# wyhuai/DDNM

Measured on NVIDIA H100. Metric: restored 256x256 images/sec @100 DDIM steps, higher is better.
Workload: dtype fp32

## Files before the change

ddnm_b200/_lib.py:

```python
import ctypes as C
import os

_HERE = os.path.dirname(os.path.abspath(__file__))
LIB_PATH = os.path.join(_HERE, "libddnm_b200.so")


class DDNMError(RuntimeError):
    pass


class SimpleCfg(C.Structure):
    _fields_ = [("ch", C.c_int), ("out_ch", C.c_int), ("n_levels", C.c_int), ("ch_mult", C.c_int * 8),
                ("num_res_blocks", C.c_int), ("n_attn_res", C.c_int), ("attn_res", C.c_int * 4),
                ("in_channels", C.c_int), ("resolution", C.c_int), ("groups", C.c_int), ("eps", C.c_float)]


class OpenAICfg(C.Structure):
    _fields_ = [("image_size", C.c_int), ("model_channels", C.c_int), ("num_res_blocks", C.c_int), ("n_levels", C.c_int),
                ("channel_mult", C.c_int * 8), ("n_attn_ds", C.c_int), ("attn_ds", C.c_int * 4),
                ("num_head_channels", C.c_int), ("out_channels", C.c_int), ("in_channels", C.c_int), ("groups", C.c_int),
                ("eps", C.c_float), ("num_classes", C.c_int), ("low_res", C.c_int), ("num_heads", C.c_int),
                ("num_heads_upsample", C.c_int), ("new_attention_order", C.c_int)]


class ClassifierCfg(C.Structure):
    _fields_ = [("image_size", C.c_int), ("model_channels", C.c_int), ("num_res_blocks", C.c_int), ("n_levels", C.c_int),
                ("channel_mult", C.c_int * 8), ("n_attn_ds", C.c_int), ("attn_ds", C.c_int * 4),
                ("num_head_channels", C.c_int), ("out_channels", C.c_int), ("in_channels", C.c_int), ("groups", C.c_int),
                ("eps", C.c_float), ("pool", C.c_int)]


class ClassifierGuidance(C.Structure):
    _fields_ = [("classifier", C.c_void_p), ("x", C.c_void_p), ("labels", C.c_void_p), ("scale", C.c_float),
                ("grad_buf", C.c_void_p), ("batch", C.c_int), ("labels_checked", C.c_int)]


class OperatorDesc(C.Structure):
    _fields_ = [("kind", C.c_int), ("channels", C.c_int), ("img_dim", C.c_int), ("ratio", C.c_int),
                ("v_small", C.c_void_p), ("u_small", C.c_void_p), ("singulars", C.c_void_p),
                ("singulars_orig", C.c_void_p), ("perm", C.c_void_p), ("mask", C.c_void_p), ("v_small2", C.c_void_p),
                ("u_small2", C.c_void_p)]


class SimpleDeg(C.Structure):
    _fields_ = [("use_mask", C.c_int), ("use_gray", C.c_int), ("scale", C.c_int), ("img_dim", C.c_int), ("channels", C.c_int),
                ("mask", C.c_void_p), ("image_mask", C.c_void_p)]


class HqScalars(C.Structure):
    _fields_ = [("c_recip", C.c_float), ("c_recipm1", C.c_float), ("coef1", C.c_float), ("coef2", C.c_float), ("lambda_t", C.c_float),
                ("gamma_t", C.c_float), ("nonzero", C.c_float), ("clip", C.c_int)]


class Schedule(C.Structure):
    _fields_ = [("n_pairs", C.c_int), ("t_i", C.c_void_p), ("t_j", C.c_void_p), ("abar", C.c_void_p),
                ("num_timesteps", C.c_int), ("eta", C.c_float), ("sigma_y", C.c_float), ("plus", C.c_int)]


class NoiseSeed(C.Structure):
    _fields_ = [("seed", C.c_ulonglong), ("row_offset", C.c_longlong)]


_lib = None

_P, _I, _LL, _F, _D = C.c_void_p, C.c_int, C.c_longlong, C.c_float, C.c_double
GuidanceFn = C.CFUNCTYPE(C.c_int, C.c_void_p, C.c_int, C.c_int, C.c_void_p)

_SIGS = {
    "ddnm_version": (C.c_int, []),
    "ddnm_unet_simple_create": (C.c_int, [C.POINTER(SimpleCfg), _I, C.POINTER(_P)]),
    "ddnm_unet_openai_create": (C.c_int, [C.POINTER(OpenAICfg), _I, C.POINTER(_P)]),
    "ddnm_classifier_create": (C.c_int, [C.POINTER(ClassifierCfg), _I, C.POINTER(_P)]),
    "ddnm_classifier_forward": (C.c_int, [_P, _P, _P, _P, _P]),
    "ddnm_classifier_grad": (C.c_int, [_P, _P, _P, _P, _F, _P, _P, _P]),
    "ddnm_classifier_guidance_fn": (C.c_int, [_P, _I, _I, _P]),
    "ddnm_unet_set_param": (C.c_int, [_P, C.c_char_p, _P, _LL]),
    "ddnm_unet_set_precision": (C.c_int, [_P, _I]),
    "ddnm_unet_finalize": (C.c_int, [_P]),
    "ddnm_unet_forward": (C.c_int, [_P, _P, _P, _P, _P]),
    "ddnm_unet_forward_cond": (C.c_int, [_P, _P, _P, _P, _P, _P]),
    "ddnm_unet_set_graph": (C.c_int, [_P, _I]),
    "ddnm_unet_set_low_res": (C.c_int, [_P, _P, _P]),
    "ddnm_unet_read_tap": (C.c_int, [_P, C.c_char_p, _P, _LL, _P]),
    "ddnm_unet_info": (C.c_int, [_P, C.POINTER(_LL), C.POINTER(_I), C.POINTER(_D)]),
    "ddnm_unet_profile": (C.c_int, [_P, _P, _P, _P, _P, C.c_char_p, _LL]),
    "ddnm_unet_destroy": (C.c_int, [_P]),
    "ddnm_operator_create": (C.c_int, [C.POINTER(OperatorDesc), C.POINTER(_P)]),
    "ddnm_operator_y_dim": (_LL, [_P]),
    "ddnm_operator_A": (C.c_int, [_P, _P, _I, _P, _P]),
    "ddnm_operator_A_pinv": (C.c_int, [_P, _P, _I, _P, _P]),
    "ddnm_operator_project": (C.c_int, [_P, _P, _P, _I, _P, _P]),
    "ddnm_operator_lambda": (C.c_int, [_P, _P, _I, _F, _F, _F, _F, _P, _P]),
    "ddnm_operator_lambda_noise": (C.c_int, [_P, _P, _P, _I, _F, _F, _F, _F, _P, _P]),
    "ddnm_operator_destroy": (C.c_int, [_P]),
    "ddnm_sample": (C.c_int, [_P, _P, C.POINTER(Schedule), _P, _P, _P, _I, _P, _P, _P]),
    "ddnm_sample_guided": (C.c_int, [_P, _P, C.POINTER(Schedule), _P, _P, _P, _I, _P, _P, GuidanceFn, _P, _P, _P, _P]),
    "ddnm_sample_range": (C.c_int, [_P, _P, C.POINTER(Schedule), _I, _I, _P, _P, C.POINTER(C.c_int), _P, _P, _I, _P, _P, _P, _P, _P]),
    "ddnm_noise_fill": (C.c_int, [C.POINTER(NoiseSeed), C.c_uint, C.c_uint, _P, _I, _LL, _P]),
    "ddnm_sample_range_seeded": (C.c_int, [_P, _P, C.POINTER(Schedule), _I, _I, _P, _P, C.POINTER(C.c_int), _P, C.POINTER(NoiseSeed), _I,
                                           _P, _P, _P, _P, _P]),
    "ddnm_sample_seeded": (C.c_int, [_P, _P, C.POINTER(Schedule), _P, _P, C.POINTER(NoiseSeed), _I, _P, _P, _P]),
    "ddnm_sample_simplified_range_seeded": (C.c_int, [_P, C.POINTER(SimpleDeg), C.POINTER(Schedule), _I, _I, _P, _P, C.POINTER(C.c_int),
                                                      _P, C.POINTER(NoiseSeed), _I, _P]),
    "ddnm_hq_step_seeded": (C.c_int, [C.POINTER(SimpleDeg), _P, _P, _I, _P, _P, _I, _I, _P, _P, C.POINTER(NoiseSeed), C.c_uint,
                                      C.POINTER(HqScalars), _I, _P, _P, _P, _P]),
    "ddnm_hq_undo_seeded": (C.c_int, [_P, C.POINTER(NoiseSeed), C.c_uint, _F, _F, _I, _LL, _P]),
    "ddnm_sample_simplified_range": (C.c_int, [_P, C.POINTER(SimpleDeg), C.POINTER(Schedule), _I, _I, _P, _P, C.POINTER(C.c_int), _P, _P,
                                               _I, _P]),
    "ddnm_simplified_A": (C.c_int, [C.POINTER(SimpleDeg), _P, _I, _P, _P]),
    "ddnm_simplified_Ap": (C.c_int, [C.POINTER(SimpleDeg), _P, _I, _P, _P]),
    "ddnm_sample_simplified": (C.c_int, [_P, C.POINTER(SimpleDeg), C.POINTER(Schedule), _P, _P, _P, _I, _P, _P, _P]),
    "ddnm_hq_canvas": (C.c_int, [_P, _I, _I, _I, _I, _I, _P, _P]),
    "ddnm_hq_step": (C.c_int, [C.POINTER(SimpleDeg), _P, _P, _I, _P, _P, _I, _I, _P, _P, _P, C.POINTER(HqScalars), _I, _P, _P, _P, _P]),
    "ddnm_hq_undo": (C.c_int, [_P, _P, _F, _F, _LL, _P]),
    "ddnm_hq_canvas_masked": (C.c_int, [C.POINTER(SimpleDeg), _P, _I, _P, _P, _P]),
    "ddnm_data_transform": (C.c_int, [_P, _LL, _P, _P, _I, _I, _P, _P]),
    "ddnm_inverse_data_transform": (C.c_int, [_P, _LL, _I, _I, _P, _P]),
    "ddnm_finish_images": (C.c_int, [_P, _P, _I, _I, _I, _I, _I, _I, _P, _P, _P, _P]),
    "ddnm_conv_tc": (C.c_int, [_P, _I, _I, _I, _I, _P, _P, _I, _I, _I, _P, _I, _P, _P, _P, _P]),
    "ddnm_conv_tc_ex": (C.c_int, [_P, _I, _I, _I, _I, _P, _P, _I, _I, _I, _I, _P, _I, _P, _P, _I, _P, _I, _I, _I, _I, C.POINTER(_D),
                                  C.POINTER(_I), _P]),
    "ddnm_gemm_tc": (C.c_int, [_P, _LL, _LL, _LL, _LL, _LL, _P, _LL, _LL, _LL, _LL, _LL, _I, _I, _I, _I, _I, _F, _P, _LL, _LL, _LL,
                               _I, _P]),
    "ddnm_conv_direct": (C.c_int, [_P, _I, _I, _I, _I, _P, _P, _I, _I, _I, _P, _P]),
    "ddnm_conv_stem_sr": (C.c_int, [_P, _P, _I, _I, _I, _I, _I, _I, _P, _P, _I, _P, _I, C.POINTER(_F), _P]),
    "ddnm_conv_tc_bench": (C.c_int, [_I, _I, _I, _I, _I, _I, _I, C.POINTER(_F), C.POINTER(_D)]),
    "ddnm_gnconv_chunk_bench": (C.c_int, [_I, _I, _I, _I, _I, _I, _I, C.POINTER(_F)]),
    "ddnm_groupnorm": (C.c_int, [_P, _I, _I, _I, _I, _I, _P, _P, _F, _I, _P, _P]),
    "ddnm_tc_debug_force_bn": (C.c_int, [_I]),
    "ddnm_tc_debug_deal": (C.c_int, [_I]),
    "ddnm_tc_debug_dual_mode": (C.c_int, [_I]),
    "ddnm_tc_debug_halo": (C.c_int, [_I]),
    "ddnm_tc_debug_pingpong": (C.c_int, [_I]),
    "ddnm_tc_debug_pp_pair": (C.c_int, [_I]),
    "ddnm_unet_set_batch_invariant": (C.c_int, [_P, _I]),
    "ddnm_tc_debug_sm_count": (C.c_int, [_I]),
}
EXPORTS = ["ddnm_last_error"] + list(_SIGS)


def lib():
    global _lib
    if _lib is None:
        if not os.path.exists(LIB_PATH):
            raise DDNMError(f"{LIB_PATH} not found: run `python -c 'import __graft_entry__ as g; g.build()'` first")
        L = C.CDLL(LIB_PATH)
        L.ddnm_last_error.restype = C.c_char_p
        L.ddnm_last_error.argtypes = []
        missing = [n for n in _SIGS if not hasattr(L, n)]
        if missing:
            raise DDNMError(f"{LIB_PATH} lacks symbols {missing}: stale build?")
        for name, (res, args) in _SIGS.items():
            fn = getattr(L, name)
            fn.restype, fn.argtypes = res, args
        _lib = L
    return _lib


def check(rc):
    if rc != 0:
        raise DDNMError(lib().ddnm_last_error().decode("utf-8", "replace"))


def noise_seed(seed, row_offset=0):
    seed, row_offset = int(seed), int(row_offset)
    if not 0 <= seed < 1 << 64:
        raise ValueError("seed must fit 64 unsigned bits")
    if row_offset < 0:
        raise ValueError("row_offset must not be negative")
    return NoiseSeed(seed, row_offset)


def ptr(t):
    return None if t is None else C.c_void_p(t.data_ptr())


def cur_stream():
    import torch
    return C.c_void_p(torch.cuda.current_stream().cuda_stream)
```

ddnm_b200/csrc/api.cu:

```cuda
#include "../../include/ddnm_b200.h"

#include <cstring>
#include <vector>

#include "api_util.cuh"
#include "engine.cuh"
#include "kernels.cuh"
#include "tc_gemm.cuh"

using namespace ddnm;

namespace ddnm {
thread_local std::string g_last_error;
}

extern "C" {

const char* ddnm_last_error(void) { return g_last_error.c_str(); }
int ddnm_version(void) { return 100; }

int ddnm_unet_simple_create(const ddnm_simple_cfg* c, int batch, void** handle) {
  DDNM_API_BEGIN
  DDNM_CHECK(c && handle, "null argument");
  SimpleCfg cfg;
  cfg.ch = c->ch; cfg.out_ch = c->out_ch; cfg.n_levels = c->n_levels;
  DDNM_CHECK(c->n_levels >= 1 && c->n_levels <= 8 && c->n_attn_res >= 0 && c->n_attn_res <= 4, "bad config");
  for (int i = 0; i < 8; ++i) cfg.ch_mult[i] = c->ch_mult[i];
  cfg.num_res_blocks = c->num_res_blocks;
  cfg.n_attn_res = c->n_attn_res;
  for (int i = 0; i < 4; ++i) cfg.attn_res[i] = c->attn_res[i];
  cfg.in_channels = c->in_channels; cfg.resolution = c->resolution; cfg.groups = c->groups; cfg.eps = c->eps;
  *handle = static_cast<UNetEngine*>(new UNetSimple(cfg, batch));
  DDNM_API_END
}

int ddnm_unet_openai_create(const ddnm_openai_cfg* c, int batch, void** handle) {
  DDNM_API_BEGIN
  DDNM_CHECK(c && handle, "null argument");
  DDNM_CHECK(c->n_levels >= 1 && c->n_levels <= 8 && c->n_attn_ds >= 0 && c->n_attn_ds <= 4, "bad config");
  OpenAICfg cfg;
  cfg.image_size = c->image_size; cfg.model_channels = c->model_channels; cfg.num_res_blocks = c->num_res_blocks;
  cfg.n_levels = c->n_levels;
  for (int i = 0; i < 8; ++i) cfg.channel_mult[i] = c->channel_mult[i];
  cfg.n_attn_ds = c->n_attn_ds;
  for (int i = 0; i < 4; ++i) cfg.attn_ds[i] = c->attn_ds[i];
  cfg.num_head_channels = c->num_head_channels; cfg.out_channels = c->out_channels; cfg.in_channels = c->in_channels;
  cfg.groups = c->groups; cfg.eps = c->eps; cfg.num_classes = c->num_classes; cfg.low_res = c->low_res;
  cfg.num_heads = c->num_heads; cfg.num_heads_upsample = c->num_heads_upsample; cfg.new_attention_order = c->new_attention_order;
  DDNM_CHECK(c->num_classes >= 0, "bad num_classes");
  DDNM_CHECK(c->new_attention_order == 0 || c->new_attention_order == 1, "new_attention_order must be 0 or 1");
  DDNM_CHECK(c->num_head_channels > 0 || c->num_heads >= 1, "num_head_channels <= 0 needs num_heads >= 1");
  *handle = static_cast<UNetEngine*>(new UNetOpenAI(cfg, batch));
  DDNM_API_END
}

int ddnm_classifier_create(const ddnm_classifier_cfg* c, int batch, void** handle) {
  DDNM_API_BEGIN
  DDNM_CHECK(c && handle, "null argument");
  DDNM_CHECK(c->n_levels >= 1 && c->n_levels <= 8 && c->n_attn_ds >= 0 && c->n_attn_ds <= 4, "bad config");
  EncoderCfg cfg;
  cfg.image_size = c->image_size; cfg.model_channels = c->model_channels; cfg.num_res_blocks = c->num_res_blocks;
  cfg.n_levels = c->n_levels;
  for (int i = 0; i < 8; ++i) cfg.channel_mult[i] = c->channel_mult[i];
  cfg.n_attn_ds = c->n_attn_ds;
  for (int i = 0; i < 4; ++i) cfg.attn_ds[i] = c->attn_ds[i];
  cfg.num_head_channels = c->num_head_channels; cfg.out_channels = c->out_channels; cfg.in_channels = c->in_channels;
  cfg.groups = c->groups; cfg.eps = c->eps; cfg.pool = c->pool;
  *handle = static_cast<UNetEngine*>(new UNetEncoder(cfg, batch));
  DDNM_API_END
}

static UNetEncoder* as_classifier(void* h) {
  UNetEncoder* e = dynamic_cast<UNetEncoder*>(static_cast<UNetEngine*>(h));
  DDNM_CHECK(e != nullptr, "handle is not a classifier");
  return e;
}

int ddnm_classifier_forward(void* h, const float* x, const float* t, float* logits, void* stream) {
  DDNM_API_BEGIN
  DDNM_CHECK(x && t && logits, "null argument");
  as_classifier(h)->forward(x, t, logits, (cudaStream_t)stream);
  DDNM_API_END
}

int ddnm_classifier_grad(void* h, const float* x, const float* t, const int* labels, float scale, float* grad_out, float* logits_out,
                         void* stream) {
  DDNM_API_BEGIN
  as_classifier(h)->grad(x, t, labels, scale, grad_out, logits_out, (cudaStream_t)stream);
  DDNM_API_END
}

int ddnm_classifier_guidance_fn(void* user, int, int t, void* stream) {
  DDNM_API_BEGIN
  ddnm_classifier_guidance* g = static_cast<ddnm_classifier_guidance*>(user);
  DDNM_CHECK(g && g->classifier && g->x && g->labels && g->grad_buf, "incomplete guidance context");
  UNetEncoder* e = as_classifier(g->classifier);
  DDNM_CHECK(g->batch == e->batch(), "classifier was built for batch " + std::to_string(e->batch()) + ", the guided loop runs " +
                                         std::to_string(g->batch));
  cudaStream_t st = (cudaStream_t)stream;
  if (!g->labels_checked) {
    e->check_labels(g->labels, st);
    g->labels_checked = 1;
  }
  e->fill_t((float)t, st);
  e->grad(g->x, e->t_in(), g->labels, g->scale, g->grad_buf, nullptr, st, true);
  DDNM_API_END
}

int ddnm_unet_set_param(void* h, const char* name, const float* data, long long numel) {
  DDNM_API_BEGIN
  static_cast<UNetEngine*>(h)->set_param(name, data, numel);
  DDNM_API_END
}
int ddnm_unet_finalize(void* h) {
  DDNM_API_BEGIN
  static_cast<UNetEngine*>(h)->finalize();
  DDNM_API_END
}
int ddnm_unet_forward(void* h, const float* x, const float* t, float* out, void* stream) {
  DDNM_API_BEGIN
  static_cast<UNetEngine*>(h)->forward(x, t, out, (cudaStream_t)stream);
  DDNM_API_END
}
int ddnm_unet_forward_cond(void* h, const float* x, const float* t, const int* labels, float* out, void* stream) {
  DDNM_API_BEGIN
  UNetEngine* u = static_cast<UNetEngine*>(h);
  u->set_labels(labels, (cudaStream_t)stream);
  u->forward(x, t, out, (cudaStream_t)stream);
  DDNM_API_END
}
int ddnm_unet_set_low_res(void* h, const float* low_res, void* stream) {
  DDNM_API_BEGIN
  static_cast<UNetEngine*>(h)->set_low_res(low_res, (cudaStream_t)stream);
  DDNM_API_END
}
int ddnm_unet_set_precision(void* h, int fp16_terms) {
  DDNM_API_BEGIN
  static_cast<UNetEngine*>(h)->set_terms(fp16_terms);
  DDNM_API_END
}
int ddnm_unet_set_batch_invariant(void* h, int on) {
  DDNM_API_BEGIN
  static_cast<UNetEngine*>(h)->set_batch_invariant(on != 0);
  DDNM_API_END
}
int ddnm_unet_set_graph(void* h, int on) {
  DDNM_API_BEGIN
  static_cast<UNetEngine*>(h)->set_use_graph(on != 0);
  DDNM_API_END
}
int ddnm_unet_read_tap(void* h, const char* name, float* dst, long long cap, void* stream) {
  DDNM_API_BEGIN
  DDNM_CHECK(static_cast<UNetEngine*>(h)->read_tap(name, dst, cap, (cudaStream_t)stream), std::string("unknown tap ") + name);
  DDNM_API_END
}
int ddnm_unet_info(void* h, long long* ws, int* launches, double* flops) {
  DDNM_API_BEGIN
  UNetEngine* u = static_cast<UNetEngine*>(h);
  if (ws) *ws = (long long)u->workspace_bytes();
  if (launches) *launches = u->num_launches();
  if (flops) *flops = u->flops_per_forward();
  DDNM_API_END
}
int ddnm_unet_profile(void* h, const float* x, const float* t, float* out, void* stream, char* json, long long cap) {
  DDNM_API_BEGIN
  std::string s = static_cast<UNetEngine*>(h)->profile(x, t, out, (cudaStream_t)stream);
  DDNM_CHECK((long long)s.size() + 1 <= cap, "json buffer too small");
  std::memcpy(json, s.c_str(), s.size() + 1);
  DDNM_API_END
}
int ddnm_unet_destroy(void* h) {
  DDNM_API_BEGIN
  delete static_cast<UNetEngine*>(h);
  DDNM_API_END
}

}

namespace {
struct Tmp {
  std::vector<void*> ptrs;
  ~Tmp() {
    for (void* p : ptrs) cudaFree(p);
  }
  template <class T>
  T* get(size_t n) {
    void* p = nullptr;
    CUDA_CHECK(cudaMalloc(&p, std::max<size_t>(n, 1) * sizeof(T)));
    ptrs.push_back(p);
    return (T*)p;
  }
};
int sm_count() {
  int dev = 0, n = 0;
  CUDA_CHECK(cudaGetDevice(&dev));
  CUDA_CHECK(cudaDeviceGetAttribute(&n, cudaDevAttrMultiProcessorCount, dev));
  return n;
}
View mkview(float* p, int N, int H, int W, int C) {
  View v;
  v.p = p; v.N = N; v.H = H; v.W = W; v.C = C; v.ld = C;
  return v;
}
int planned_sm_count() {
  int dev = 0;
  CUDA_CHECK(cudaGetDevice(&dev));
  cudaDeviceProp prop;
  CUDA_CHECK(cudaGetDeviceProperties(&prop, dev));
  return engine_sm_count(prop);
}
struct TermsScope {
  int prev;
  explicit TermsScope(int t) : prev(tc_get_terms()) { tc_set_terms(t); }
  ~TermsScope() { tc_set_terms(prev); }
};
}

extern "C" {

int ddnm_conv_tc(const float* x, int N, int H, int W, int Cin, const float* w, const float* bias, int Cout, int mode, int up2,
                 const float* side_x, int CinSide, const float* side_w, const float* residual, float* out, void* stream) {
  DDNM_API_BEGIN
  cudaStream_t s = (cudaStream_t)stream;
  Tmp tmp;
  const int taps = mode == TAPS_1X1 ? 1 : 9;
  int oH = H, oW = W;
  int smode = SPLIT_SAME;
  if (mode == TAPS_3X3_S2) { oH = H / 2; oW = W / 2; smode = SPLIT_S2D; DDNM_CHECK(!up2, "stride 2 with upsample"); }
  if (up2) { oH = 2 * H; oW = 2 * W; DDNM_CHECK(mode == TAPS_3X3 && !side_x && !residual, "upsample path: plain 3x3 only"); }
  const size_t pe = (size_t)N * H * W * Cin;
  SplitView A;
  A.hi = tmp.get<__half>(pe); A.lo = tmp.get<__half>(pe); A.C = Cin;
  if (smode == SPLIT_S2D) { A.N = 4 * N; A.H = oH; A.W = oW; } else { A.N = N; A.H = H; A.W = W; }
  View xv = mkview(const_cast<float*>(x), N, H, W, Cin);
  gn_apply_split(xv, 1, false, nullptr, nullptr, 0.f, false, smode, A.hi, A.lo, s);
  View ov = mkview(out, N, oH, oW, Cout);
  if (up2) {
    const size_t per_phase = (size_t)Cout * 4 * Cin;
    __half* wh = tmp.get<__half>(4 * per_phase);
    __half* wl = tmp.get<__half>(4 * per_phase);
    presum_up2_weights(w, Cout, Cin, wh, wl, s);
    for (int ph = 0; ph < 4; ++ph) {
      TcLaunch L = tc_make_up2_launch(A, wh + ph * per_phase, wl + ph * per_phase, Cout, ov, bias, 0, ph >> 1, ph & 1, sm_count());
      tc_run(L, s);
    }
    CUDA_CHECK(cudaStreamSynchronize(s));
    return 0;
  }
  SplitView S;
  if (side_x) {
    const size_t se = (size_t)N * oH * oW * CinSide;
    S.hi = tmp.get<__half>(se); S.lo = tmp.get<__half>(se); S.N = N; S.H = oH; S.W = oW; S.C = CinSide;
    gn_apply_split(mkview(const_cast<float*>(side_x), N, oH, oW, CinSide), 1, false, nullptr, nullptr, 0.f, false, SPLIT_SAME,
                   S.hi, S.lo, s);
  }
  const int ktot = taps * Cin + (side_x ? CinSide : 0);
  __half* wh = tmp.get<__half>((size_t)Cout * ktot);
  __half* wl = tmp.get<__half>((size_t)Cout * ktot);
  split_conv_weight(w, Cout, Cin, taps, wh, wl, ktot, 0, s);
  if (side_x) split_conv_weight(side_w, Cout, CinSide, 1, wh, wl, ktot, taps * Cin, s);
  TcLaunch L = tc_make_launch(A, mode, side_x ? &S : nullptr, wh, wl, 1, Cout, ov, bias, 0, residual, Cout, 1.0f, sm_count());
  tc_run(L, s);
  CUDA_CHECK(cudaStreamSynchronize(s));
  DDNM_API_END
}

int ddnm_conv_tc_ex(const float* x, int N, int H, int W, int Cin, const float* w, const float* chanadd, int ca_ld, int Cout, int mode,
                    int up2, const float* side_x, int CinSide, const float* side_w, const float* residual, int res_mode, float* out,
                    int out_ld, int split_k, int invariant, int terms, double* stats_out, int* split_used, void* stream) {
  DDNM_API_BEGIN
  DDNM_CHECK(x && w && out, "null argument");
  DDNM_CHECK(mode >= TAPS_3X3 && mode <= TAPS_3X3_S2 && res_mode >= 0 && res_mode <= 2 && out_ld >= Cout && ca_ld >= 0,
             "bad mode, res_mode, out_ld or ca_ld");
  DDNM_CHECK(split_k == -1 || split_k == 1 || split_k == 2 || split_k == 4, "split_k must be -1 (the engine's rule), 1, 2 or 4");
  cudaStream_t s = (cudaStream_t)stream;
  Tmp tmp;
  const TermsScope terms_scope(terms);
  const int sms = planned_sm_count();
  const int taps = mode == TAPS_1X1 ? 1 : 9;
  int oH = H, oW = W;
  int smode = SPLIT_SAME;
  if (mode == TAPS_3X3_S2) { oH = H / 2; oW = W / 2; smode = SPLIT_S2D; DDNM_CHECK(!up2, "stride 2 with upsample"); }
  if (up2) {
    oH = 2 * H; oW = 2 * W;
    DDNM_CHECK(mode == TAPS_3X3 && !side_x && !residual && split_k <= 1, "upsample path: plain unsplit 3x3 only");
  }
  const size_t pe = (size_t)N * H * W * Cin;
  SplitView A;
  A.hi = tmp.get<__half>(pe); A.lo = tmp.get<__half>(pe); A.C = Cin;
  if (smode == SPLIT_S2D) { A.N = 4 * N; A.H = oH; A.W = oW; } else { A.N = N; A.H = H; A.W = W; }
  gn_apply_split(mkview(const_cast<float*>(x), N, H, W, Cin), 1, false, nullptr, nullptr, 0.f, false, smode, A.hi, A.lo, s);
  View ov = mkview(out, N, oH, oW, Cout);
  ov.ld = out_ld;
  if (stats_out) {
    ov.st = tmp.get<StatAcc>((size_t)N * Cout * 2);
    ov.st_ld = Cout;
    CUDA_CHECK(cudaMemsetAsync(ov.st, 0, (size_t)N * Cout * 2 * sizeof(StatAcc), s));
  }
  int S = 1;
  if (up2) {
    const size_t per_phase = (size_t)Cout * 4 * Cin;
    __half* wh = tmp.get<__half>(4 * per_phase);
    __half* wl = tmp.get<__half>(4 * per_phase);
    presum_up2_weights(w, Cout, Cin, wh, wl, s);
    for (int ph = 0; ph < 4; ++ph)
      tc_run(tc_make_up2_launch(A, wh + ph * per_phase, wl + ph * per_phase, Cout, ov, chanadd, ca_ld, ph >> 1, ph & 1, sms, invariant != 0), s);
  } else {
    SplitView Sv;
    if (side_x) {
      const size_t se = (size_t)N * oH * oW * CinSide;
      Sv.hi = tmp.get<__half>(se); Sv.lo = tmp.get<__half>(se); Sv.N = N; Sv.H = oH; Sv.W = oW; Sv.C = CinSide;
      gn_apply_split(mkview(const_cast<float*>(side_x), N, oH, oW, CinSide), 1, false, nullptr, nullptr, 0.f, false, SPLIT_SAME,
                     Sv.hi, Sv.lo, s);
    }
    const int ktot = taps * Cin + (side_x ? CinSide : 0);
    __half* wh = tmp.get<__half>((size_t)Cout * ktot);
    __half* wl = tmp.get<__half>((size_t)Cout * ktot);
    split_conv_weight(w, Cout, Cin, taps, wh, wl, ktot, 0, s);
    if (side_x) split_conv_weight(side_w, Cout, CinSide, 1, wh, wl, ktot, taps * Cin, s);
    TcConvPlan P = tc_plan_conv(A, mode, side_x ? &Sv : nullptr, wh, wl, Cout, ov, chanadd, ca_ld, residual, Cout, res_mode, sms,
                                invariant != 0, split_k);
    if (P.S > 1) tc_set_partials(P, tmp.get<float>((size_t)P.part_elems));
    tc_run_conv(P, s);
    S = P.S;
  }
  CUDA_CHECK(cudaStreamSynchronize(s));
  if (split_used) *split_used = S;
  if (stats_out) {
    std::vector<StatAcc> h((size_t)N * Cout * 2);
    CUDA_CHECK(cudaMemcpy(h.data(), ov.st, h.size() * sizeof(StatAcc), cudaMemcpyDeviceToHost));
    for (size_t i = 0; i < h.size(); ++i) stats_out[i] = stat_value(h[i]);
  }
  DDNM_API_END
}

int ddnm_gemm_tc(const float* a, long long a_numel, long long a_off, long long a_s_row, long long a_s_head, long long a_s_img,
                 const float* b, long long b_numel, long long b_off, long long b_s_row, long long b_s_head, long long b_s_img, int M,
                 int N, int K, int heads, int images, float alpha, float* out, long long out_sn, long long out_sy, long long out_sx,
                 int invariant, void* stream) {
  DDNM_API_BEGIN
  DDNM_CHECK(a && b && out && M > 0 && N > 0 && K > 0 && heads > 0 && images > 0, "null or empty argument");
  cudaStream_t s = (cudaStream_t)stream;
  Tmp tmp;
  auto operand = [&](const float* src, long long numel, long long off, long long rows, long long s_row, long long s_head,
                     long long s_img) {
    DDNM_CHECK(numel % 8 == 0 && off >= 0 && s_row > 0 && s_head > 0 && s_img > 0, "GEMM operand: bad size or strides");
    DDNM_CHECK(off + (K - 1) + (rows - 1) * s_row + (heads - 1) * s_head + (images - 1) * s_img < numel,
               "GEMM operand reaches past its buffer");
    __half* hi = tmp.get<__half>((size_t)numel);
    __half* lo = tmp.get<__half>((size_t)numel);
    gn_apply_split(mkview(const_cast<float*>(src), 1, 1, (int)(numel / 8), 8), 1, false, nullptr, nullptr, 0.f, false, SPLIT_SAME,
                   hi, lo, s);
    return GemmOperand{hi + off, lo + off, s_row, s_head, s_img};
  };
  const GemmOperand A = operand(a, a_numel, a_off, M, a_s_row, a_s_head, a_s_img);
  const GemmOperand B = operand(b, b_numel, b_off, N, b_s_row, b_s_head, b_s_img);
  tc_run(tc_make_gemm_launch(A, B, M, N, K, heads, images, out, out_sn, out_sy, out_sx, alpha, planned_sm_count(), invariant != 0), s);
  CUDA_CHECK(cudaStreamSynchronize(s));
  DDNM_API_END
}

int ddnm_conv_stem_sr(const float* x, const float* low_res, int N, int C, int H, int W, int h, int w, const float* weight,
                      const float* bias, int Cout, float* out, int iters, float* ms_per_iter, void* stream) {
  DDNM_API_BEGIN
  DDNM_CHECK(x && weight && bias && out, "null argument");
  cudaStream_t s = (cudaStream_t)stream;
  View ov = mkview(out, N, H, W, Cout);
  conv3x3_stem_sr(x, low_res, C, h, w, weight, bias, ov, s);
  if (iters > 0 && ms_per_iter) {
    cudaEvent_t e0, e1;
    CUDA_CHECK(cudaEventCreate(&e0));
    CUDA_CHECK(cudaEventCreate(&e1));
    CUDA_CHECK(cudaEventRecord(e0, s));
    for (int i = 0; i < iters; ++i) conv3x3_stem_sr(x, low_res, C, h, w, weight, bias, ov, s);
    CUDA_CHECK(cudaEventRecord(e1, s));
    CUDA_CHECK(cudaEventSynchronize(e1));
    float ms = 0;
    CUDA_CHECK(cudaEventElapsedTime(&ms, e0, e1));
    cudaEventDestroy(e0);
    cudaEventDestroy(e1);
    *ms_per_iter = ms / iters;
  }
  CUDA_CHECK(cudaStreamSynchronize(s));
  DDNM_API_END
}

int ddnm_conv_direct(const float* x, int N, int H, int W, int Cin, const float* w, const float* bias, int Cout, int mode, int up2,
                     float* out, void* stream) {
  DDNM_API_BEGIN
  int oH = H, oW = W;
  if (mode == TAPS_3X3_S2) { oH = H / 2; oW = W / 2; }
  if (up2) { oH = 2 * H; oW = 2 * W; }
  conv_direct_ref(mkview(const_cast<float*>(x), N, H, W, Cin), w, bias, mode, up2 != 0, mkview(out, N, oH, oW, Cout),
                  (cudaStream_t)stream);
  DDNM_API_END
}

namespace {
__device__ __forceinline__ float bench_hash(unsigned long long i, unsigned seed) {
  unsigned x = (unsigned)(i * 2654435761ull) ^ seed;
  x ^= x >> 16; x *= 0x7feb352du; x ^= x >> 15; x *= 0x846ca68bu; x ^= x >> 16;
  return (float)(int)x * (1.0f / 2147483648.0f);
}
__global__ void bench_fill_f32(float* p, long long n, unsigned seed) {
  const long long i = (long long)blockIdx.x * blockDim.x + threadIdx.x;
  if (i < n) p[i] = bench_hash(i, seed);
}
__global__ void bench_fill_split(__half* hi, __half* lo, long long n, unsigned seed, float scale) {
  const long long i = (long long)blockIdx.x * blockDim.x + threadIdx.x;
  if (i < n) split_f16(bench_hash(i, seed) * scale, hi[i], lo[i]);
}
}

int ddnm_conv_tc_bench(int N, int H, int W, int Cin, int Cout, int mode, int iters, float* ms_per_iter, double* flops) {
  DDNM_API_BEGIN
  const bool random = iters < 0;
  if (random) iters = -iters;
  const int feat = mode >> 4;
  mode &= 15;
  const bool up2 = (feat & 8) != 0;
  Tmp tmp;
  const int taps = up2 ? 4 : (mode == TAPS_1X1 ? 1 : 9);
  const size_t pe = (size_t)N * H * W * Cin;
  SplitView A;
  A.hi = tmp.get<__half>(pe); A.lo = tmp.get<__half>(pe); A.N = N; A.H = H; A.W = W; A.C = Cin;
  float* xf = tmp.get<float>(pe);
  CUDA_CHECK(cudaMemset(xf, 0, pe * 4));
  if (random) bench_fill_f32<<<(unsigned)cdivll((long long)pe, 256), 256>>>(xf, (long long)pe, 0x1234u);
  gn_apply_split(mkview(xf, N, H, W, Cin), 1, false, nullptr, nullptr, 0.f, false, SPLIT_SAME, A.hi, A.lo, 0);
  const int ktot = taps * Cin;
  __half* wh = tmp.get<__half>((size_t)Cout * ktot);
  __half* wl = tmp.get<__half>((size_t)Cout * ktot);
  CUDA_CHECK(cudaMemset(wh, 0, (size_t)Cout * ktot * 2));
  CUDA_CHECK(cudaMemset(wl, 0, (size_t)Cout * ktot * 2));
  if (random) {
    const long long wn = (long long)Cout * ktot;
    bench_fill_split<<<(unsigned)cdivll(wn, 256), 256>>>(wh, wl, wn, 0x9876u, 1.0f / sqrtf((float)ktot));
  }
  const int oH = up2 ? 2 * H : H, oW = up2 ? 2 * W : W;
  const size_t oe = (size_t)N * oH * oW * Cout;
  float* o = tmp.get<float>(oe);
  View ov = mkview(o, N, oH, oW, Cout);
  if (feat & 1) {
    ov.st = tmp.get<StatAcc>((size_t)N * Cout * 2);
    ov.st_ld = Cout;
    CUDA_CHECK(cudaMemset(ov.st, 0, (size_t)N * Cout * 2 * sizeof(StatAcc)));
  }
  float* res = nullptr;
  if (feat & 2) {
    res = tmp.get<float>(oe);
    CUDA_CHECK(cudaMemset(res, 0, oe * 4));
    if (random) bench_fill_f32<<<(unsigned)cdivll((long long)oe, 256), 256>>>(res, (long long)oe, 0x777u);
  }
  float* ca = nullptr;
  if (feat & 4) {
    ca = tmp.get<float>((size_t)N * Cout);
    CUDA_CHECK(cudaMemset(ca, 0, (size_t)N * Cout * 4));
  }
  TcLaunch L = up2 ? tc_make_up2_launch(A, wh, wl, Cout, ov, ca, Cout, 0, 0, sm_count())
                   : tc_make_launch(A, mode, nullptr, wh, wl, 1, Cout, ov, ca, Cout, res, Cout, 1.0f, sm_count());
  for (int i = 0; i < 3; ++i) tc_run(L, 0);
  cudaEvent_t e0, e1;
  CUDA_CHECK(cudaEventCreate(&e0));
  CUDA_CHECK(cudaEventCreate(&e1));
  CUDA_CHECK(cudaEventRecord(e0, 0));
  for (int i = 0; i < iters; ++i) tc_run(L, 0);
  CUDA_CHECK(cudaEventRecord(e1, 0));
  CUDA_CHECK(cudaEventSynchronize(e1));
  float ms = 0;
  CUDA_CHECK(cudaEventElapsedTime(&ms, e0, e1));
  cudaEventDestroy(e0);
  cudaEventDestroy(e1);
  *ms_per_iter = ms / iters;
  *flops = L.flops;
  DDNM_API_END
}

int ddnm_gnconv_chunk_bench(int N, int chunk, int H, int W, int Cin, int Cout, int iters, float* ms_per_pass) {
  DDNM_API_BEGIN
  DDNM_CHECK(chunk >= 1 && N % chunk == 0, "chunk must divide N");
  Tmp tmp;
  const size_t pe = (size_t)N * H * W * Cin, ce = (size_t)chunk * H * W * Cin, oe = (size_t)N * H * W * Cout;
  float* x = tmp.get<float>(pe);
  bench_fill_f32<<<(unsigned)cdivll((long long)pe, 256), 256>>>(x, (long long)pe, 0x4321u);
  StatAcc* st = tmp.get<StatAcc>((size_t)N * Cin * 2);
  CUDA_CHECK(cudaMemset(st, 0, (size_t)N * Cin * 2 * sizeof(StatAcc)));
  View xv = mkview(x, N, H, W, Cin);
  xv.st = st; xv.st_ld = Cin;
  gn_stats(xv, 0);
  float* gamma = tmp.get<float>(Cin);
  float* beta = tmp.get<float>(Cin);
  bench_fill_f32<<<cdiv(Cin, 256), 256>>>(gamma, Cin, 0x11u);
  bench_fill_f32<<<cdiv(Cin, 256), 256>>>(beta, Cin, 0x22u);
  SplitView A;
  A.hi = tmp.get<__half>(ce); A.lo = tmp.get<__half>(ce); A.N = chunk; A.H = H; A.W = W; A.C = Cin;
  const int ktot = 9 * Cin;
  __half* wh = tmp.get<__half>((size_t)Cout * ktot);
  __half* wl = tmp.get<__half>((size_t)Cout * ktot);
  bench_fill_split<<<(unsigned)cdivll((long long)Cout * ktot, 256), 256>>>(wh, wl, (long long)Cout * ktot, 0x9876u, 1.0f / sqrtf((float)ktot));
  float* o = tmp.get<float>(oe);
  StatAcc* ost = tmp.get<StatAcc>((size_t)N * Cout * 2);
  CUDA_CHECK(cudaMemset(ost, 0, (size_t)N * Cout * 2 * sizeof(StatAcc)));
  float* ca = tmp.get<float>((size_t)N * Cout);
  CUDA_CHECK(cudaMemset(ca, 0, (size_t)N * Cout * 4));
  const int nch = N / chunk;
  std::vector<View> xs;
  std::vector<TcLaunch> Ls;
  for (int c = 0; c < nch; ++c) {
    View xc = xv;
    xc.p = x + (size_t)c * chunk * H * W * Cin; xc.N = chunk; xc.st = st + (size_t)c * chunk * Cin * 2;
    View oc = mkview(o + (size_t)c * chunk * H * W * Cout, chunk, H, W, Cout);
    oc.st = ost + (size_t)c * chunk * Cout * 2; oc.st_ld = Cout;
    xs.push_back(xc);
    Ls.push_back(tc_make_launch(A, TAPS_3X3, nullptr, wh, wl, 1, Cout, oc, ca + (size_t)c * chunk * Cout, Cout, nullptr, 0, 1.0f, sm_count()));
  }
  auto pass = [&]() {
    for (int c = 0; c < nch; ++c) {
      gn_apply_split(xs[c], 32, true, gamma, beta, 1e-6f, true, SPLIT_SAME, A.hi, A.lo, 0);
      tc_run(Ls[c], 0);
    }
  };
  for (int i = 0; i < 2; ++i) pass();
  cudaEvent_t e0, e1;
  CUDA_CHECK(cudaEventCreate(&e0));
  CUDA_CHECK(cudaEventCreate(&e1));
  CUDA_CHECK(cudaEventRecord(e0, 0));
  for (int i = 0; i < iters; ++i) pass();
  CUDA_CHECK(cudaEventRecord(e1, 0));
  CUDA_CHECK(cudaEventSynchronize(e1));
  float ms = 0;
  CUDA_CHECK(cudaEventElapsedTime(&ms, e0, e1));
  cudaEventDestroy(e0);
  cudaEventDestroy(e1);
  *ms_per_pass = ms / iters;
  DDNM_API_END
}

int ddnm_groupnorm(const float* x, int N, int H, int W, int C, int groups, const float* gamma, const float* beta, float eps,
                   int silu, float* out, void* stream) {
  DDNM_API_BEGIN
  cudaStream_t s = (cudaStream_t)stream;
  Tmp tmp;
  StatAcc* st = tmp.get<StatAcc>((size_t)N * C * 2);
  CUDA_CHECK(cudaMemsetAsync(st, 0, (size_t)N * C * 2 * sizeof(StatAcc), s));
  View xv = mkview(const_cast<float*>(x), N, H, W, C);
  xv.st = st;
  xv.st_ld = C;
  gn_stats(xv, s);
  gn_apply_f32(xv, groups, gamma, beta, eps, silu != 0, out, s);
  CUDA_CHECK(cudaStreamSynchronize(s));
  DDNM_API_END
}

int ddnm_tc_debug_deal(int mode) {
  DDNM_API_BEGIN
  tc_debug_deal(mode);
  DDNM_API_END
}
int ddnm_tc_debug_dual_mode(int mode) {
  DDNM_API_BEGIN
  tc_debug_dual_mode(mode);
  DDNM_API_END
}
int ddnm_tc_debug_halo(int on) {
  DDNM_API_BEGIN
  tc_debug_halo(on);
  DDNM_API_END
}
int ddnm_tc_debug_pingpong(int on) {
  DDNM_API_BEGIN
  tc_debug_pingpong(on);
  DDNM_API_END
}
int ddnm_tc_debug_pp_pair(int on) {
  DDNM_API_BEGIN
  tc_debug_pp_pair(on);
  DDNM_API_END
}
int ddnm_tc_debug_force_bn(int bn) {
  DDNM_API_BEGIN
  tc_debug_force_bn(bn);
  DDNM_API_END
}
int ddnm_tc_debug_sm_count(int n) {
  DDNM_API_BEGIN
  engine_debug_sm_count(n);
  DDNM_API_END
}
}
```

ddnm_b200/csrc/common.cuh:

```cuda
#pragma once
#include <cuda_runtime.h>
#include <cuda_fp16.h>
#include <cuda.h>
#include <cstdint>
#include <cstdio>
#include <stdexcept>
#include <string>

namespace ddnm {

struct Error : std::runtime_error {
  using std::runtime_error::runtime_error;
};

#define DDNM_CHECK(cond, msg)                                                                     \
  do {                                                                                            \
    if (!(cond)) throw ::ddnm::Error(std::string(msg) + " [" #cond "] at " __FILE__ ":" + std::to_string(__LINE__)); \
  } while (0)

#define CUDA_CHECK(expr)                                                                          \
  do {                                                                                            \
    cudaError_t _e = (expr);                                                                      \
    if (_e != cudaSuccess)                                                                        \
      throw ::ddnm::Error(std::string("CUDA error: ") + cudaGetErrorString(_e) + " in " #expr " at " __FILE__ ":" + \
                          std::to_string(__LINE__));                                              \
  } while (0)

inline int cdiv(int a, int b) { return (a + b - 1) / b; }
inline bool first_use_on_device(bool (&flags)[64]) {
  int dev = 0;
  cudaGetDevice(&dev);
  dev &= 63;
  if (flags[dev]) return false;
  flags[dev] = true;
  return true;
}
inline long long cdivll(long long a, long long b) { return (a + b - 1) / b; }

struct StreamBuf {
  float* p = nullptr;
  cudaStream_t st = nullptr;
  StreamBuf(size_t elems, cudaStream_t s) : st(s) {
    cudaError_t e = cudaMallocAsync((void**)&p, elems * sizeof(float), s);
    if (e != cudaSuccess) throw Error(std::string("CUDA error: ") + cudaGetErrorString(e) + " in cudaMallocAsync (sampler scratch)");
  }
  ~StreamBuf() {
    if (p) cudaFreeAsync(p, st);
  }
  StreamBuf(const StreamBuf&) = delete;
  StreamBuf& operator=(const StreamBuf&) = delete;
};

struct StatAcc {
  unsigned long long lo;
  long long hi;
};

bool pdl_enabled();
template <typename... KArgs, typename... Args>
inline void launch_pdl(void (*kernel)(KArgs...), dim3 grid, dim3 block, size_t smem, cudaStream_t st, int cluster, Args... args) {
  cudaLaunchConfig_t cfg = {};
  cfg.gridDim = grid;
  cfg.blockDim = block;
  cfg.dynamicSmemBytes = smem;
  cfg.stream = st;
  cudaLaunchAttribute at[2];
  int na = 0;
  if (pdl_enabled()) {
    at[na].id = cudaLaunchAttributeProgrammaticStreamSerialization;
    at[na].val.programmaticStreamSerializationAllowed = 1;
    ++na;
  }
  if (cluster > 1) {
    at[na].id = cudaLaunchAttributeClusterDimension;
    at[na].val.clusterDim.x = cluster;
    at[na].val.clusterDim.y = 1;
    at[na].val.clusterDim.z = 1;
    ++na;
  }
  cfg.attrs = at;
  cfg.numAttrs = na;
  cudaError_t e = cudaLaunchKernelEx(&cfg, kernel, KArgs(args)...);
  if (e != cudaSuccess) throw Error(std::string("CUDA error: ") + cudaGetErrorString(e) + " in cudaLaunchKernelEx");
}

struct View {
  float* p = nullptr;
  int N = 0, H = 0, W = 0, C = 0, ld = 0;
  StatAcc* st = nullptr;
  int st_ld = 0;
  long long pixels() const { return (long long)N * H * W; }
  View slice(int c0, int c) const {
    View v = *this;
    v.p = p + c0;
    v.C = c;
    if (st) v.st = st + 2 * (size_t)c0;
    return v;
  }
};

struct SplitView {
  __half* hi = nullptr;
  __half* lo = nullptr;
  int N = 0, H = 0, W = 0, C = 0;
};

#ifdef __CUDACC__
__device__ __forceinline__ void pdl_prologue() {
  asm volatile("griddepcontrol.launch_dependents;" ::: "memory");
  asm volatile("griddepcontrol.wait;" ::: "memory");
}
__device__ __forceinline__ uint32_t smem_u32(const void* p) { return (uint32_t)__cvta_generic_to_shared(p); }

__device__ __forceinline__ void mbar_init(uint32_t bar, uint32_t count) {
  asm volatile("mbarrier.init.shared::cta.b64 [%0], %1;" ::"r"(bar), "r"(count));
}
__device__ __forceinline__ void mbar_fence_init() { asm volatile("fence.mbarrier_init.release.cluster;" ::: "memory"); }
__device__ __forceinline__ void mbar_expect_tx(uint32_t bar, uint32_t bytes) {
  asm volatile("mbarrier.arrive.expect_tx.shared::cta.b64 _, [%0], %1;" ::"r"(bar), "r"(bytes) : "memory");
}
__device__ __forceinline__ void mbar_arrive(uint32_t bar) {
  asm volatile("mbarrier.arrive.shared::cta.b64 _, [%0];" ::"r"(bar) : "memory");
}
__device__ __forceinline__ bool mbar_try_wait(uint32_t bar, uint32_t parity) {
  uint32_t ok;
  asm volatile(
      "{\n\t.reg .pred p;\n\t"
      "mbarrier.try_wait.parity.shared::cta.b64 p, [%1], %2;\n\t"
      "selp.u32 %0, 1, 0, p;\n\t}"
      : "=r"(ok)
      : "r"(bar), "r"(parity)
      : "memory");
  return ok != 0;
}
__device__ __forceinline__ void mbar_wait(uint32_t bar, uint32_t parity) {
  if (mbar_try_wait(bar, parity)) return;
  long long t0 = clock64();
  while (!mbar_try_wait(bar, parity)) {
    if (clock64() - t0 > 4000000000LL) __trap();
  }
}

__device__ __forceinline__ void tma_prefetch_desc(const void* tmap) {
  asm volatile("prefetch.tensormap [%0];" ::"l"(tmap) : "memory");
}
__device__ __forceinline__ void tma_load_2d(uint32_t dst, const void* tmap, uint32_t bar, int c0, int c1) {
  asm volatile(
      "cp.async.bulk.tensor.2d.shared::cluster.global.tile.mbarrier::complete_tx::bytes [%0], [%1, {%3, %4}], [%2];" ::"r"(dst),
      "l"(tmap), "r"(bar), "r"(c0), "r"(c1)
      : "memory");
}
__device__ __forceinline__ void tma_load_3d(uint32_t dst, const void* tmap, uint32_t bar, int c0, int c1, int c2) {
  asm volatile(
      "cp.async.bulk.tensor.3d.shared::cluster.global.tile.mbarrier::complete_tx::bytes [%0], [%1, {%3, %4, %5}], [%2];" ::"r"(dst),
      "l"(tmap), "r"(bar), "r"(c0), "r"(c1), "r"(c2)
      : "memory");
}
__device__ __forceinline__ void tma_load_4d(uint32_t dst, const void* tmap, uint32_t bar, int c0, int c1, int c2, int c3) {
  asm volatile(
      "cp.async.bulk.tensor.4d.shared::cluster.global.tile.mbarrier::complete_tx::bytes [%0], [%1, {%3, %4, %5, %6}], [%2];" ::"r"(dst),
      "l"(tmap), "r"(bar), "r"(c0), "r"(c1), "r"(c2), "r"(c3)
      : "memory");
}

__device__ __forceinline__ uint64_t wgmma_desc_sw128(uint32_t saddr) {
  return (uint64_t)((saddr & 0x3FFFFu) >> 4) | ((uint64_t)1 << 16) | ((uint64_t)(1024 >> 4) << 32) | ((uint64_t)1 << 62);
}
__device__ __forceinline__ void wgmma_fence() { asm volatile("wgmma.fence.sync.aligned;" ::: "memory"); }
__device__ __forceinline__ void wgmma_commit() { asm volatile("wgmma.commit_group.sync.aligned;" ::: "memory"); }
template <int N>
__device__ __forceinline__ void wgmma_wait() { asm volatile("wgmma.wait_group.sync.aligned %0;" ::"n"(N) : "memory"); }
__device__ __forceinline__ void wgmma_m64n64k16(float (&d)[32], uint64_t a_desc, uint64_t b_desc, uint32_t accumulate) {
  asm volatile(
      "{\n\t.reg .pred p;\n\t"
      "setp.ne.b32 p, %34, 0;\n\t"
      "wgmma.mma_async.sync.aligned.m64n64k16.f32.f16.f16 "
      "{%0, %1, %2, %3, %4, %5, %6, %7, %8, %9, %10, %11, %12, %13, %14, %15, %16, %17, %18, %19, %20, %21, %22, %23, %24, %25, %26, %27, %28, %29, %30, %31}, "
      "%32, %33, p, 1, 1, 0, 0;\n\t}"
      : "+f"(d[0]), "+f"(d[1]), "+f"(d[2]), "+f"(d[3]), "+f"(d[4]), "+f"(d[5]), "+f"(d[6]), "+f"(d[7]), "+f"(d[8]), "+f"(d[9]), "+f"(d[10]), "+f"(d[11]), "+f"(d[12]), "+f"(d[13]), "+f"(d[14]), "+f"(d[15]), "+f"(d[16]), "+f"(d[17]), "+f"(d[18]), "+f"(d[19]), "+f"(d[20]), "+f"(d[21]), "+f"(d[22]), "+f"(d[23]), "+f"(d[24]), "+f"(d[25]), "+f"(d[26]), "+f"(d[27]), "+f"(d[28]), "+f"(d[29]), "+f"(d[30]), "+f"(d[31])
      : "l"(a_desc), "l"(b_desc), "r"(accumulate));
}
__device__ __forceinline__ void wgmma_m64n128k16(float (&d)[64], uint64_t a_desc, uint64_t b_desc, uint32_t accumulate) {
  asm volatile(
      "{\n\t.reg .pred p;\n\t"
      "setp.ne.b32 p, %66, 0;\n\t"
      "wgmma.mma_async.sync.aligned.m64n128k16.f32.f16.f16 "
      "{%0, %1, %2, %3, %4, %5, %6, %7, %8, %9, %10, %11, %12, %13, %14, %15, %16, %17, %18, %19, %20, %21, %22, %23, %24, %25, %26, %27, %28, %29, %30, %31, %32, %33, %34, %35, %36, %37, %38, %39, %40, %41, %42, %43, %44, %45, %46, %47, %48, %49, %50, %51, %52, %53, %54, %55, %56, %57, %58, %59, %60, %61, %62, %63}, "
      "%64, %65, p, 1, 1, 0, 0;\n\t}"
      : "+f"(d[0]), "+f"(d[1]), "+f"(d[2]), "+f"(d[3]), "+f"(d[4]), "+f"(d[5]), "+f"(d[6]), "+f"(d[7]), "+f"(d[8]), "+f"(d[9]), "+f"(d[10]), "+f"(d[11]), "+f"(d[12]), "+f"(d[13]), "+f"(d[14]), "+f"(d[15]), "+f"(d[16]), "+f"(d[17]), "+f"(d[18]), "+f"(d[19]), "+f"(d[20]), "+f"(d[21]), "+f"(d[22]), "+f"(d[23]), "+f"(d[24]), "+f"(d[25]), "+f"(d[26]), "+f"(d[27]), "+f"(d[28]), "+f"(d[29]), "+f"(d[30]), "+f"(d[31]), "+f"(d[32]), "+f"(d[33]), "+f"(d[34]), "+f"(d[35]), "+f"(d[36]), "+f"(d[37]), "+f"(d[38]), "+f"(d[39]), "+f"(d[40]), "+f"(d[41]), "+f"(d[42]), "+f"(d[43]), "+f"(d[44]), "+f"(d[45]), "+f"(d[46]), "+f"(d[47]), "+f"(d[48]), "+f"(d[49]), "+f"(d[50]), "+f"(d[51]), "+f"(d[52]), "+f"(d[53]), "+f"(d[54]), "+f"(d[55]), "+f"(d[56]), "+f"(d[57]), "+f"(d[58]), "+f"(d[59]), "+f"(d[60]), "+f"(d[61]), "+f"(d[62]), "+f"(d[63])
      : "l"(a_desc), "l"(b_desc), "r"(accumulate));
}
__device__ __forceinline__ void wgmma_m64n256k16(float (&d)[128], uint64_t a_desc, uint64_t b_desc, uint32_t accumulate) {
  asm volatile(
      "{\n\t.reg .pred p;\n\t"
      "setp.ne.b32 p, %130, 0;\n\t"
      "wgmma.mma_async.sync.aligned.m64n256k16.f32.f16.f16 "
      "{%0, %1, %2, %3, %4, %5, %6, %7, %8, %9, %10, %11, %12, %13, %14, %15, %16, %17, %18, %19, %20, %21, %22, %23, %24, %25, %26, %27, %28, %29, %30, %31, %32, %33, %34, %35, %36, %37, %38, %39, %40, %41, %42, %43, %44, %45, %46, %47, %48, %49, %50, %51, %52, %53, %54, %55, %56, %57, %58, %59, %60, %61, %62, %63, %64, %65, %66, %67, %68, %69, %70, %71, %72, %73, %74, %75, %76, %77, %78, %79, %80, %81, %82, %83, %84, %85, %86, %87, %88, %89, %90, %91, %92, %93, %94, %95, %96, %97, %98, %99, %100, %101, %102, %103, %104, %105, %106, %107, %108, %109, %110, %111, %112, %113, %114, %115, %116, %117, %118, %119, %120, %121, %122, %123, %124, %125, %126, %127}, "
      "%128, %129, p, 1, 1, 0, 0;\n\t}"
      : "+f"(d[0]), "+f"(d[1]), "+f"(d[2]), "+f"(d[3]), "+f"(d[4]), "+f"(d[5]), "+f"(d[6]), "+f"(d[7]), "+f"(d[8]), "+f"(d[9]), "+f"(d[10]), "+f"(d[11]), "+f"(d[12]), "+f"(d[13]), "+f"(d[14]), "+f"(d[15]), "+f"(d[16]), "+f"(d[17]), "+f"(d[18]), "+f"(d[19]), "+f"(d[20]), "+f"(d[21]), "+f"(d[22]), "+f"(d[23]), "+f"(d[24]), "+f"(d[25]), "+f"(d[26]), "+f"(d[27]), "+f"(d[28]), "+f"(d[29]), "+f"(d[30]), "+f"(d[31]), "+f"(d[32]), "+f"(d[33]), "+f"(d[34]), "+f"(d[35]), "+f"(d[36]), "+f"(d[37]), "+f"(d[38]), "+f"(d[39]), "+f"(d[40]), "+f"(d[41]), "+f"(d[42]), "+f"(d[43]), "+f"(d[44]), "+f"(d[45]), "+f"(d[46]), "+f"(d[47]), "+f"(d[48]), "+f"(d[49]), "+f"(d[50]), "+f"(d[51]), "+f"(d[52]), "+f"(d[53]), "+f"(d[54]), "+f"(d[55]), "+f"(d[56]), "+f"(d[57]), "+f"(d[58]), "+f"(d[59]), "+f"(d[60]), "+f"(d[61]), "+f"(d[62]), "+f"(d[63]), "+f"(d[64]), "+f"(d[65]), "+f"(d[66]), "+f"(d[67]), "+f"(d[68]), "+f"(d[69]), "+f"(d[70]), "+f"(d[71]), "+f"(d[72]), "+f"(d[73]), "+f"(d[74]), "+f"(d[75]), "+f"(d[76]), "+f"(d[77]), "+f"(d[78]), "+f"(d[79]), "+f"(d[80]), "+f"(d[81]), "+f"(d[82]), "+f"(d[83]), "+f"(d[84]), "+f"(d[85]), "+f"(d[86]), "+f"(d[87]), "+f"(d[88]), "+f"(d[89]), "+f"(d[90]), "+f"(d[91]), "+f"(d[92]), "+f"(d[93]), "+f"(d[94]), "+f"(d[95]), "+f"(d[96]), "+f"(d[97]), "+f"(d[98]), "+f"(d[99]), "+f"(d[100]), "+f"(d[101]), "+f"(d[102]), "+f"(d[103]), "+f"(d[104]), "+f"(d[105]), "+f"(d[106]), "+f"(d[107]), "+f"(d[108]), "+f"(d[109]), "+f"(d[110]), "+f"(d[111]), "+f"(d[112]), "+f"(d[113]), "+f"(d[114]), "+f"(d[115]), "+f"(d[116]), "+f"(d[117]), "+f"(d[118]), "+f"(d[119]), "+f"(d[120]), "+f"(d[121]), "+f"(d[122]), "+f"(d[123]), "+f"(d[124]), "+f"(d[125]), "+f"(d[126]), "+f"(d[127])
      : "l"(a_desc), "l"(b_desc), "r"(accumulate));
}
__device__ __forceinline__ uint32_t cluster_ctarank() {
  uint32_t r;
  asm volatile("mov.u32 %0, %%cluster_ctarank;" : "=r"(r));
  return r;
}
__device__ __forceinline__ void cluster_sync_all() {
  asm volatile("barrier.cluster.arrive.release.aligned;" ::: "memory");
  asm volatile("barrier.cluster.wait.acquire.aligned;" ::: "memory");
}
__device__ __forceinline__ void mbar_arrive_cluster(uint32_t bar, uint32_t cta) {
  uint32_t remote;
  asm volatile("mapa.shared::cluster.u32 %0, %1, %2;" : "=r"(remote) : "r"(bar), "r"(cta));
  asm volatile("mbarrier.arrive.shared::cluster.b64 _, [%0];" ::"r"(remote) : "memory");
}
__device__ __forceinline__ void tma_load_3d_multicast(uint32_t dst, const void* tmap, uint32_t bar, int c0, int c1, int c2, uint16_t mask) {
  asm volatile(
      "cp.async.bulk.tensor.3d.shared::cluster.global.mbarrier::complete_tx::bytes.multicast::cluster [%0], [%1, {%3, %4, %5}], [%2], %6;" ::"r"(dst),
      "l"(tmap), "r"(bar), "r"(c0), "r"(c1), "r"(c2), "h"(mask)
      : "memory");
}
__device__ __forceinline__ void named_bar_sync(int id, int threads) { asm volatile("bar.sync %0, %1;" ::"r"(id), "r"(threads) : "memory"); }
template <int R>
__device__ __forceinline__ void setmaxnreg_dec() { asm volatile("setmaxnreg.dec.sync.aligned.u32 %0;" ::"n"(R)); }
template <int R>
__device__ __forceinline__ void setmaxnreg_inc() { asm volatile("setmaxnreg.inc.sync.aligned.u32 %0;" ::"n"(R)); }

__device__ __forceinline__ void stat_add(StatAcc* acc, float p) {
  const int bits = __float_as_int(p);
  int ex = (bits >> 23) & 0xff;
  unsigned long long m = (unsigned long long)(bits & 0x7fffff);
  if (ex) m |= 0x800000ull; else ex = 1;
  const int sh = ex - 150 + 48;
  unsigned long long lo = 0, hi = 0;
  if (sh >= 64) hi = m << min(sh - 64, 7);
  else if (sh > 0) { lo = m << sh; hi = sh > 40 ? m >> (64 - sh) : 0ull; }
  else if (sh > -24) lo = m >> (-sh);
  if (bits < 0) {
    lo = ~lo + 1ull;
    hi = ~hi + (lo == 0ull ? 1ull : 0ull);
  }
  const unsigned long long w0 = lo & 0xffffffffull;
  const unsigned long long w1 = (hi << 32) | (lo >> 32);
  if (w0) atomicAdd(&acc->lo, w0);
  if (w1) atomicAdd(reinterpret_cast<unsigned long long*>(&acc->hi), w1);
}
__device__ __forceinline__ void two_sum_acc(float& sum, float& comp, float v) {
  const float s = __fadd_rn(sum, v);
  const float bb = __fadd_rn(s, -sum);
  comp = __fadd_rn(comp, __fadd_rn(__fadd_rn(sum, -__fadd_rn(s, -bb)), __fadd_rn(v, -bb)));
  sum = s;
}
__host__ __device__ __forceinline__ double stat_value(const StatAcc& a) {
  return ((double)a.hi * 4294967296.0 + (double)a.lo) * (1.0 / 281474976710656.0);
}

__device__ __forceinline__ float swishf_fast(float x) {
  float e;
  asm("ex2.approx.ftz.f32 %0, %1;" : "=f"(e) : "f"(x * -1.4426950408889634f));
  return __fdividef(x, 1.0f + e);
}
__device__ __forceinline__ void split_f16(float x, __half& hi, __half& lo) {
  unsigned short h;
  asm("cvt.rn.satfinite.f16.f32 %0, %1;" : "=h"(h) : "f"(x));
  hi = __ushort_as_half(h);
  float r = x - __half2float(hi);
  asm("cvt.rn.satfinite.f16.f32 %0, %1;" : "=h"(h) : "f"(r));
  lo = __ushort_as_half(h);
}
__device__ __forceinline__ void split2_f16(float x0, float x1, uint32_t& hi, uint32_t& lo) {
  asm("cvt.rn.satfinite.f16x2.f32 %0, %1, %2;" : "=r"(hi) : "f"(x1), "f"(x0));
  const __half2 h = *reinterpret_cast<const __half2*>(&hi);
  const float2 f = __half22float2(h);
  asm("cvt.rn.satfinite.f16x2.f32 %0, %1, %2;" : "=r"(lo) : "f"(x1 - f.y), "f"(x0 - f.x));
}

#endif

}
```

ddnm_b200/csrc/engine.cu:

```cuda
#include "engine.cuh"

#include <algorithm>
#include <cmath>
#include <cstdlib>
#include <sstream>

#include "kernels.cuh"

namespace ddnm {

Arena::~Arena() {
  for (void* b : blocks_) cudaFree(b);
}
void* Arena::alloc(size_t bytes) {
  bytes = (bytes + 1023) / 1024 * 1024;
  if (bytes == 0) bytes = 1024;
  void* p = nullptr;
  CUDA_CHECK(cudaMalloc(&p, bytes));
  blocks_.push_back(p);
  total_ += bytes;
  return p;
}

static int g_sm_count = 0;
void engine_debug_sm_count(int n) {
  DDNM_CHECK(n >= 0, "SM count must be 0 (the device's) or positive");
  g_sm_count = n;
}
int engine_sm_count(const cudaDeviceProp& prop) {
  return g_sm_count > 0 ? std::min(g_sm_count, prop.multiProcessorCount) : prop.multiProcessorCount;
}

UNetEngine::UNetEngine(int batch, int in_channels, int out_ch, int resolution, int groups, float eps)
    : B_(batch), in_ch_(in_channels), out_ch_(out_ch), R_(resolution), groups_(groups), eps_(eps) {
  DDNM_CHECK(batch >= 1, "batch must be positive");
  int dev = 0;
  CUDA_CHECK(cudaGetDevice(&dev));
  cudaDeviceProp prop;
  CUDA_CHECK(cudaGetDeviceProperties(&prop, dev));
  DDNM_CHECK(prop.major == 9 && prop.minor == 0, "ddnm_b200 kernels are built for sm_90a (H100) only");
  num_sms_ = engine_sm_count(prop);
}

UNetEngine::~UNetEngine() {
  if (graph_exec_) cudaGraphExecDestroy(graph_exec_);
  if (graph_) cudaGraphDestroy(graph_);
  for (auto& kv : params_) cudaFree(kv.second.p);
}

void UNetEngine::set_param(const std::string& name, const float* data, long long numel) {
  DDNM_CHECK(!finalized_, "set_param after finalize");
  DDNM_CHECK(numel > 0 && data != nullptr, "empty parameter " + name);
  float* d = nullptr;
  CUDA_CHECK(cudaMalloc(&d, (size_t)numel * sizeof(float)));
  CUDA_CHECK(cudaMemcpy(d, data, (size_t)numel * sizeof(float), cudaMemcpyDefault));
  auto it = params_.find(name);
  if (it != params_.end()) cudaFree(it->second.p);
  params_[name] = Param{d, numel};
}

const float* UNetEngine::P(const std::string& name, long long expect) const {
  auto it = params_.find(name);
  DDNM_CHECK(it != params_.end(), "missing parameter '" + name + "'");
  if (expect >= 0)
    DDNM_CHECK(it->second.n == expect, "parameter '" + name + "' has " + std::to_string(it->second.n) + " elements, expected " +
                                           std::to_string(expect));
  return it->second.p;
}

View UNetEngine::new_view(int H, int W, int C) {
  View v = view_of((float*)arena_.alloc((size_t)B_ * H * W * C * sizeof(float)), H, W, C);
  v.st = new_stats(C);
  v.st_ld = C;
  return v;
}

View UNetEngine::view_of(float* p, int H, int W, int C) const {
  View v;
  v.p = p; v.N = B_; v.H = H; v.W = W; v.C = C; v.ld = C;
  return v;
}

StatAcc* UNetEngine::new_stats(int C) {
  const size_t need = (size_t)B_ * C * 2;
  if (stats_chunks_.empty() || stats_chunks_.back().used + need > stats_chunks_.back().cap) {
    StatsChunk c;
    c.cap = std::max<size_t>(need, (size_t)1 << 20);
    c.used = 0;
    c.p = (StatAcc*)arena_.alloc(c.cap * sizeof(StatAcc));
    stats_chunks_.push_back(c);
  }
  StatsChunk& c = stats_chunks_.back();
  StatAcc* p = c.p + c.used;
  c.used += need;
  return p;
}

UNetEngine::TcWeights UNetEngine::prep_weights(const std::string& main, int Cout, int Cin, int taps, const std::string& side,
                                               int CinSide) {
  TcWeights w;
  w.ktot = taps * Cin + CinSide;
  const size_t n = (size_t)Cout * w.ktot;
  w.hi = (__half*)arena_.alloc(n * sizeof(__half));
  w.lo = (__half*)arena_.alloc(n * sizeof(__half));
  split_conv_weight(P(main, (long long)Cout * Cin * taps), Cout, Cin, taps, w.hi, w.lo, w.ktot, 0, 0);
  if (CinSide) split_conv_weight(P(side, (long long)Cout * CinSide), Cout, CinSide, 1, w.hi, w.lo, w.ktot, taps * Cin, 0);
  return w;
}

const float* UNetEngine::bias_sum(const std::string& a, const std::string& b, int C) {
  std::vector<float> ha(C), hb(C, 0.f);
  CUDA_CHECK(cudaMemcpy(ha.data(), P(a, C), C * sizeof(float), cudaMemcpyDeviceToHost));
  if (!b.empty()) CUDA_CHECK(cudaMemcpy(hb.data(), P(b, C), C * sizeof(float), cudaMemcpyDeviceToHost));
  for (int i = 0; i < C; ++i) ha[i] += hb[i];
  float* d = (float*)arena_.alloc(C * sizeof(float));
  CUDA_CHECK(cudaMemcpy(d, ha.data(), C * sizeof(float), cudaMemcpyHostToDevice));
  return d;
}

float* UNetEngine::dev_copy(const std::vector<float>& v) {
  float* d = (float*)arena_.alloc(v.size() * sizeof(float));
  CUDA_CHECK(cudaMemcpy(d, v.data(), v.size() * sizeof(float), cudaMemcpyHostToDevice));
  return d;
}

void UNetEngine::add_op(const std::string& name, const std::string& kind, double flops, double bytes,
                        std::function<void(cudaStream_t)> f) {
  ops_.push_back(OpRecord{name, kind, flops, bytes, std::move(f)});
}

void UNetEngine::emit_gn_split(const std::string& name, const View& x, const std::string& norm, bool silu, int mode,
                               SplitView& dst, const float* ss, int ss_ld, SplitView* raw) {
  const long long out_elems = mode == SPLIT_AVG2 ? x.pixels() * x.C / 4 : x.pixels() * x.C;
  DDNM_CHECK((size_t)out_elems <= split_elems_, "split scratch too small");
  dst.C = x.C;
  if (mode == SPLIT_SAME) { dst.N = x.N; dst.H = x.H; dst.W = x.W; }
  else if (mode == SPLIT_AVG2) { dst.N = x.N; dst.H = x.H / 2; dst.W = x.W / 2; }
  else { dst.N = 4 * x.N; dst.H = x.H / 2; dst.W = x.W / 2; }
  const double in_bytes = (double)x.pixels() * x.C * 4;
  if (!norm.empty()) {
    DDNM_CHECK(x.st != nullptr, "GroupNorm input without producer-side statistics: " + name);
    const float* g = P(norm + ".weight", x.C);
    const float* b = P(norm + ".bias", x.C);
    const int groups = groups_;
    const float eps = eps_;
    __half *hi = dst.hi, *lo = dst.lo, *rhi = nullptr, *rlo = nullptr;
    if (raw) {
      DDNM_CHECK(mode == SPLIT_SAME, "raw side output only with the plain split");
      raw->N = x.N; raw->H = x.H; raw->W = x.W; raw->C = x.C;
      rhi = raw->hi; rlo = raw->lo;
    }
    add_op(name + ".gn_split", "gn_split", 0, in_bytes + out_elems * 4.0 * (raw ? 2 : 1),
           [=](cudaStream_t s) { gn_apply_split(x, groups, true, g, b, eps, silu, mode, hi, lo, s, ss, ss_ld, rhi, rlo); });
  } else {
    __half *hi = dst.hi, *lo = dst.lo;
    add_op(name + ".split", "gn_split", 0, in_bytes + out_elems * 4.0,
           [=](cudaStream_t s) { gn_apply_split(x, 1, false, nullptr, nullptr, 0.f, silu, mode, hi, lo, s); });
  }
}

void UNetEngine::emit_tc(const std::string& name, const SplitView& a, int mode, const SplitView* side, const TcWeights& w,
                         int Cout, const View& out, const float* chanadd, int ca_ld, const float* residual, int ldr, int res_mode) {
  TcConvPlan P = tc_plan_conv(a, mode, side, w.hi, w.lo, Cout, out, chanadd, ca_ld, residual, ldr, res_mode, num_sms_, invariant_);
  const TcLaunch& L = P.L;
  const double bytes = (double)a.N * a.H * a.W * a.C * 4 + (side ? (double)side->N * side->H * side->W * side->C * 4 : 0) +
                       (double)Cout * w.ktot * 4 + (double)out.pixels() * Cout * 4 * (residual ? 2 : 1);
  if (P.S > 1) {
    tc_set_partials(P, (float*)arena_.alloc((size_t)P.part_elems * sizeof(float)));
    add_op(name, "tc", L.flops, bytes, [L](cudaStream_t s) { tc_run(L, s); });
    add_op(name + ".splitk_reduce", "reduce", 0, (double)(P.S + 1 + (residual ? 1 : 0)) * (P.part_elems / P.S) * 4,
           [P](cudaStream_t s) { tc_run_split_reduce(P, s); });
    return;
  }
  add_op(name, "tc", L.flops, bytes, [L](cudaStream_t s) { tc_run(L, s); });
}

void UNetEngine::alloc_common(size_t split_elems, size_t hbuf_elems) {
  split_elems_ = split_elems;
  hbuf_elems_ = hbuf_elems;
  splitA_hi_ = (__half*)arena_.alloc(split_elems * 2);
  splitA_lo_ = (__half*)arena_.alloc(split_elems * 2);
  splitB_hi_ = (__half*)arena_.alloc(split_elems * 2);
  splitB_lo_ = (__half*)arena_.alloc(split_elems * 2);
  if (hbuf_elems) hbuf_ = (float*)arena_.alloc(hbuf_elems * 4);
  x_in_ = (float*)arena_.alloc((size_t)B_ * in_ch_ * R_ * R_ * 4);
  t_in_ = (float*)arena_.alloc((size_t)B_ * 4);
  labels_in_ = (int*)arena_.alloc((size_t)B_ * 4);
  CUDA_CHECK(cudaMemset(labels_in_, 0, (size_t)B_ * 4));
  out_ = (float*)arena_.alloc(out_elems() * 4);
  if (lowres_ > 0) lowres_in_ = (float*)arena_.alloc((size_t)B_ * in_ch_ * lowres_ * lowres_ * 4);
}

void UNetEngine::emit_up2_conv(const std::string& name, const SplitView& a, const std::string& wname, int Cout, const View& out,
                               const float* chanadd, int ca_ld) {
  const int Cin = a.C;
  const size_t per_phase = (size_t)Cout * 4 * Cin;
  __half* wh = (__half*)arena_.alloc(4 * per_phase * sizeof(__half));
  __half* wl = (__half*)arena_.alloc(4 * per_phase * sizeof(__half));
  presum_up2_weights(P(wname, (long long)Cout * Cin * 9), Cout, Cin, wh, wl, 0);
  for (int ph = 0; ph < 4; ++ph) {
    TcLaunch L = tc_make_up2_launch(a, wh + ph * per_phase, wl + ph * per_phase, Cout, out, chanadd, ca_ld, ph >> 1, ph & 1, num_sms_,
                                     invariant_);
    const double bytes = (double)a.N * a.H * a.W * Cin * 4 + (double)per_phase * 4 + (double)a.N * a.H * a.W * Cout * 4;
    add_op(name + ".ph" + std::to_string(ph), "tc", L.flops, bytes, [L](cudaStream_t s) { tc_run(L, s); });
  }
}

void UNetEngine::alloc_attention(size_t qkv_elems, size_t s_elems, size_t o_elems) {
  qkv_ = (float*)arena_.alloc(qkv_elems * 4);
  attS_ = (float*)arena_.alloc(s_elems * 4);
  attO_ = (float*)arena_.alloc(o_elems * 4);
  qkvh_ = (__half*)arena_.alloc(qkv_elems * 2);
  qkvl_ = (__half*)arena_.alloc(qkv_elems * 2);
  ph_ = (__half*)arena_.alloc(s_elems * 2);
  pl_ = (__half*)arena_.alloc(s_elems * 2);
  vth_ = (__half*)arena_.alloc(o_elems * 2);
  vtl_ = (__half*)arena_.alloc(o_elems * 2);
}

void UNetEngine::emit_attention_core(const std::string& name, float* qkv, int T, int heads, int ch, int qkv_ld, int head_stride,
                                     int q_off, int k_off, int v_off, float alpha) {
  float *q = qkv, *S = attS_, *O = attO_;
  const int Bn = B_, C = heads * ch;
  const long long img = (long long)T * qkv_ld;
  const double fl = 2.0 * Bn * heads * (double)T * T * ch;
  const double sbytes = (double)Bn * heads * T * T * 4;
  if (T % 128 == 0 && ch % 8 == 0) {
    __half *qh = qkvh_, *ql = qkvl_, *ph = ph_, *pl = pl_, *vh = vth_, *vl = vtl_;
    DDNM_CHECK(qkv_ld % C == 0, "qkv row is not a multiple of the attention width");
    const View qv = view_of(qkv, 1, T * (qkv_ld / C), C);
    add_op(name + ".qkv_split", "gn_split", 0, (double)Bn * T * qkv_ld * 8,
           [=](cudaStream_t s) { gn_apply_split(qv, 1, false, nullptr, nullptr, 0.f, false, SPLIT_SAME, qh, ql, s); });
    const long long hs = head_stride ? head_stride : qkv_ld;
    GemmOperand A{qh + q_off, ql + q_off, qkv_ld, hs, img};
    GemmOperand Bk{qh + k_off, ql + k_off, qkv_ld, hs, img};
    TcLaunch L1 = tc_make_gemm_launch(A, Bk, T, T, ch, heads, Bn, S, (long long)heads * T * T, (long long)T * T, T, alpha, num_sms_, invariant_);
    add_op(name + ".qk", "tc", L1.flops, (double)Bn * T * qkv_ld * 4 + sbytes, [L1](cudaStream_t s) { tc_run(L1, s); });
    add_op(name + ".softmax", "softmax", 0, sbytes * 2, [=](cudaStream_t s) { softmax_split(S, (long long)Bn * heads * T, T, ph, pl, s); });
    add_op(name + ".v_transpose", "gn_split", 0, (double)Bn * T * C * 8,
           [=](cudaStream_t s) { transpose_split(q, qkv_ld, head_stride, v_off, Bn, T, heads, ch, vh, vl, s); });
    GemmOperand P{ph, pl, T, (long long)T * T, (long long)heads * T * T};
    GemmOperand Vt{vh, vl, T, (long long)ch * T, (long long)heads * ch * T};
    TcLaunch L2 = tc_make_gemm_launch(P, Vt, T, ch, T, heads, Bn, O, (long long)T * C, ch, C, 1.0f, num_sms_, invariant_);
    add_op(name + ".pv", "tc", L2.flops, sbytes + (double)Bn * T * C * 8, [L2](cudaStream_t s) { tc_run(L2, s); });
  } else {
    add_op(name + ".qk", "sgemm", fl, (double)Bn * heads * T * (2.0 * ch + T) * 4, [=](cudaStream_t s) {
      sgemm_batched(true, Bn, heads, T, T, ch, alpha, q + q_off, qkv_ld, img, head_stride, q + k_off, qkv_ld, img, head_stride, S, T,
                    (long long)heads * T * T, (long long)T * T, s);
    });
    add_op(name + ".softmax", "softmax", 0, sbytes * 2, [=](cudaStream_t s) { softmax_rows(S, (long long)Bn * heads * T, T, s); });
    add_op(name + ".pv", "sgemm", fl, (double)Bn * heads * T * (2.0 * ch + T) * 4, [=](cudaStream_t s) {
      sgemm_batched(false, Bn, heads, T, ch, T, 1.0f, S, T, (long long)heads * T * T, (long long)T * T, q + v_off, qkv_ld, img, head_stride, O,
                    C, (long long)T * C, ch, s);
    });
  }
}

void UNetEngine::emit_stem(const std::string& wname, const View& out) {
  const float* xin = x_in_;
  if (lowres_ > 0) {
    const float *w = P(wname + ".weight", (long long)out.C * 2 * in_ch_ * 9), *b = P(wname + ".bias", out.C);
    const float* lr = lowres_in_;
    const int cin = in_ch_, s = lowres_;
    add_op("stem.sr", "stem", 2.0 * B_ * R_ * R_ * (double)out.C * 2 * cin * 9,
           (double)B_ * (R_ * R_ * (cin + out.C) + (double)s * s * cin) * 4,
           [=](cudaStream_t st) { conv3x3_stem_sr(xin, lr, cin, s, s, w, b, out, st); });
    return;
  }
  const float *w = P(wname + ".weight", (long long)out.C * in_ch_ * 9), *b = P(wname + ".bias", out.C);
  const int cin = in_ch_;
  add_op("stem", "stem", 2.0 * B_ * R_ * R_ * (double)out.C * cin * 9, (double)B_ * R_ * R_ * (cin + out.C) * 4,
         [=](cudaStream_t s) { conv3x3_small_cin(xin, cin, w, b, out, s); });
}

void UNetEngine::emit_head(const std::string& norm, const std::string& conv, const View& fh) {
  DDNM_CHECK(fh.st != nullptr, "head input without statistics");
  DDNM_CHECK(out_ch_ <= 64, "head convolution: out_ch <= 64");
  if (head_conv_supported(fh, out_ch_) && std::getenv("DDNM_HEAD_TC") == nullptr) {
    const float *g = P(norm + ".weight", fh.C), *b = P(norm + ".bias", fh.C);
    const float *w = P(conv + ".weight", (long long)out_ch_ * fh.C * 9), *cb = P(conv + ".bias", out_ch_);
    const int groups = groups_, oc = out_ch_;
    const float eps = eps_;
    float* o = out_;
    add_op("head.conv", "head", 2.0 * fh.pixels() * (double)oc * fh.C * 9, (double)fh.pixels() * (fh.C + oc) * 4,
           [=](cudaStream_t s) { head_conv(fh, groups, g, b, eps, w, cb, oc, o, s); });
    return;
  }
  SplitView A{splitA_hi_, splitA_lo_};
  emit_gn_split("head", fh, norm, true, SPLIT_SAME, A);
  const int ktot = 9 * fh.C;
  TcWeights w;
  w.ktot = ktot;
  w.hi = (__half*)arena_.alloc((size_t)64 * ktot * sizeof(__half));
  w.lo = (__half*)arena_.alloc((size_t)64 * ktot * sizeof(__half));
  CUDA_CHECK(cudaMemset(w.hi, 0, (size_t)64 * ktot * sizeof(__half)));
  CUDA_CHECK(cudaMemset(w.lo, 0, (size_t)64 * ktot * sizeof(__half)));
  split_conv_weight(P(conv + ".weight", (long long)out_ch_ * fh.C * 9), out_ch_, fh.C, 9, w.hi, w.lo, ktot, 0, 0);
  std::vector<float> hb(64, 0.f);
  CUDA_CHECK(cudaMemcpy(hb.data(), P(conv + ".bias", out_ch_), out_ch_ * sizeof(float), cudaMemcpyDeviceToHost));
  float* bias64 = dev_copy(hb);
  const View o64 = view_of((float*)arena_.alloc((size_t)B_ * fh.H * fh.W * 64 * sizeof(float)), fh.H, fh.W, 64);
  emit_tc("head.conv", A, TAPS_3X3, nullptr, w, 64, o64, bias64, 0, nullptr, 0);
  float* o = out_;
  const View real = o64.slice(0, out_ch_);
  add_op("head.to_nchw", "head", 0, (double)fh.pixels() * (64 + out_ch_) * 4, [=](cudaStream_t s) { nhwc_to_nchw(real, o, s); });
}

void UNetEngine::emit_time_embed(const std::string& name, const std::string& layer0, const std::string& layer1, int ch,
                                 bool sin_first, const float* label_emb, int num_classes, const std::vector<EmbProj>& projs) {
  const int tdim = ch * 4;
  float* emb = (float*)arena_.alloc((size_t)B_ * ch * 4);
  float* t0 = (float*)arena_.alloc((size_t)B_ * tdim * 4);
  float* t1 = (float*)arena_.alloc((size_t)B_ * tdim * 4);
  float* fr = (float*)arena_.alloc((size_t)(ch / 2) * 4);
  CUDA_CHECK(cudaMemcpy(fr, P("__freq", ch / 2), (ch / 2) * 4, cudaMemcpyDeviceToDevice));
  emb_ld_ = 0;
  for (const EmbProj& pr : projs) {
    emb_off_[pr.block] = emb_ld_;
    emb_ld_ += pr.rows;
  }
  float* W = (float*)arena_.alloc((size_t)emb_ld_ * tdim * 4);
  float* Bv = (float*)arena_.alloc((size_t)emb_ld_ * 4);
  emb_all_ = (float*)arena_.alloc((size_t)B_ * emb_ld_ * 4);
  for (const EmbProj& pr : projs) {
    const int off = emb_off_[pr.block];
    CUDA_CHECK(cudaMemcpy(W + (size_t)off * tdim, P(pr.weight, (long long)pr.rows * tdim), (size_t)pr.rows * tdim * 4,
                          cudaMemcpyDeviceToDevice));
    CUDA_CHECK(cudaMemcpy(Bv + off, pr.bias, (size_t)pr.rows * 4, cudaMemcpyDeviceToDevice));
  }
  const float *w0 = P(layer0 + ".weight", (long long)tdim * ch), *b0 = P(layer0 + ".bias", tdim);
  const float *w1 = P(layer1 + ".weight", (long long)tdim * tdim), *b1 = P(layer1 + ".bias", tdim);
  const float* t = t_in_;
  const int* labels = labels_in_;
  float* rows = emb_all_;
  const int Bn = B_, tot = emb_ld_;
  add_op(name, "temb", 0, 0, [=](cudaStream_t s) {
    sinusoid(t, Bn, fr, ch, sin_first, emb, s);
    linear(emb, Bn, ch, w0, b0, tdim, t0, tdim, 0, 1, s);
    if (label_emb) {
      linear(t0, Bn, tdim, w1, b1, tdim, t1, tdim, 0, 0, s);
      add_label_swish(t1, label_emb, labels, Bn, tdim, num_classes, s);
    } else {
      linear(t0, Bn, tdim, w1, b1, tdim, t1, tdim, 0, 1, s);
    }
    linear(t1, Bn, tdim, W, Bv, tot, rows, tot, 0, 0, s);
  });
}

UNetEngine::Torso UNetEngine::plan_torso(int image_size, int in_channels, int model_channels, const int* channel_mult, int n_levels,
                                         int num_res_blocks, const int* attn_ds, int n_attn_ds) {
  auto attn_at = [&](int ds) { return std::find(attn_ds, attn_ds + n_attn_ds, ds) != attn_ds + n_attn_ds; };
  Torso t;
  int ch = channel_mult[0] * model_channels, ds = 1, res = image_size;
  t.input.push_back({{{LAYER_CONV, in_channels, ch}}, res, res, ch});
  for (int lv = 0; lv < n_levels; ++lv) {
    const int co = channel_mult[lv] * model_channels;
    for (int i = 0; i < num_res_blocks; ++i) {
      Block b{{{LAYER_RES, ch, co}}, res, res, co};
      ch = co;
      if (attn_at(ds)) b.layers.push_back({LAYER_ATTN, ch, ch});
      t.input.push_back(b);
    }
    if (lv != n_levels - 1) {
      t.input.push_back({{{LAYER_RES_DOWN, ch, ch}}, res, res / 2, ch});
      res /= 2;
      ds *= 2;
    }
  }
  t.middle = {{{LAYER_RES, ch, ch}, {LAYER_ATTN, ch, ch}, {LAYER_RES, ch, ch}}, res, res, ch};
  return t;
}

void UNetEngine::emit_res_block(const std::string& p, const View& x, const View& h, const View& out, int kind) {
  const int Cin = x.C, Cout = out.C;
  if (kind != LAYER_RES) DDNM_CHECK(Cin == Cout, "up/down ResBlocks keep the channel count");
  SplitView A{splitA_hi_, splitA_lo_}, Bs{splitB_hi_, splitB_lo_};
  const int mode1 = kind == LAYER_RES_DOWN ? SPLIT_AVG2 : SPLIT_SAME;
  const bool has_skip_conv = has_param(p + ".skip_connection.weight");
  emit_gn_split(p + ".in", x, p + ".in_layers.0", true, mode1, A, nullptr, 0, has_skip_conv ? &Bs : nullptr);
  if (kind == LAYER_RES_UP) {
    emit_up2_conv(p + ".conv1", A, p + ".in_layers.2.weight", Cout, h, P(p + ".in_layers.2.bias", Cout), 0);
  } else {
    TcWeights w1 = prep_weights(p + ".in_layers.2.weight", Cout, Cin, 9, "", 0);
    emit_tc(p + ".conv1", A, TAPS_3X3, nullptr, w1, Cout, h, P(p + ".in_layers.2.bias", Cout), 0, nullptr, 0);
  }
  emit_gn_split(p + ".out", h, p + ".out_layers.0", true, SPLIT_SAME, A, emb_rows(p), emb_ld_);
  if (has_skip_conv) {
    DDNM_CHECK(kind == LAYER_RES, "skip convolution on an up/down block");
    TcWeights w2 = prep_weights(p + ".out_layers.3.weight", Cout, Cout, 9, p + ".skip_connection.weight", Cin);
    emit_tc(p + ".conv2+skip", A, TAPS_3X3, &Bs, w2, Cout, out, bias_sum(p + ".out_layers.3.bias", p + ".skip_connection.bias", Cout), 0,
            nullptr, 0);
  } else {
    DDNM_CHECK(Cin == Cout, "identity skip needs equal channels");
    TcWeights w2 = prep_weights(p + ".out_layers.3.weight", Cout, Cout, 9, "", 0);
    emit_tc(p + ".conv2", A, TAPS_3X3, nullptr, w2, Cout, out, P(p + ".out_layers.3.bias", Cout), 0, x.p, x.ld,
            kind == LAYER_RES_UP ? 1 : (kind == LAYER_RES_DOWN ? 2 : 0));
  }
}

void UNetEngine::emit_attention_block(const std::string& p, const View& x, const View& out, int heads, bool new_order, float* qkv) {
  const int C = x.C, T = x.H * x.W, ch = C / heads;
  SplitView A{splitA_hi_, splitA_lo_};
  emit_gn_split(p + ".norm", x, p + ".norm", false, SPLIT_SAME, A);
  TcWeights wqkv = prep_weights(p + ".qkv.weight", 3 * C, C, 1, "", 0);
  emit_tc(p + ".qkv", A, TAPS_1X1, nullptr, wqkv, 3 * C, view_of(qkv, x.H, x.W, 3 * C), P(p + ".qkv.bias", 3 * C), 0, nullptr, 0);
  const float alpha = 1.0f / std::sqrt((float)ch);
  if (new_order) emit_attention_core(p, qkv, T, heads, ch, 3 * C, ch, 0, C, 2 * C, alpha);
  else emit_attention_core(p, qkv, T, heads, ch, 3 * C, 3 * ch, 0, ch, 2 * ch, alpha);
  emit_gn_split(p + ".proj_in", view_of(attO_, x.H, x.W, C), "", false, SPLIT_SAME, A);
  TcWeights wp = prep_weights(p + ".proj_out.weight", C, C, 1, "", 0);
  emit_tc(p + ".proj_out", A, TAPS_1X1, nullptr, wp, C, out, P(p + ".proj_out.bias", C), 0, x.p, x.ld);
}

void UNetEngine::set_terms(int t) {
  DDNM_CHECK(!finalized_, "precision must be chosen before finalize");
  DDNM_CHECK(t == 1 || t == 3, "terms must be 1 (fast fp16) or 3 (fp32-grade)");
  terms_ = t;
}

void UNetEngine::set_batch_invariant(bool on) {
  DDNM_CHECK(!finalized_, "batch-invariant mode must be chosen before finalize");
  invariant_ = on;
}

void UNetEngine::finalize() {
  DDNM_CHECK(!finalized_, "finalize called twice");
  const int prev = tc_get_terms();
  tc_set_terms(terms_);
  try {
    build_program();
  } catch (...) {
    tc_set_terms(prev);
    throw;
  }
  tc_set_terms(prev);
  std::vector<OpRecord> zero;
  for (const StatsChunk& c : stats_chunks_) {
    StatAcc* sb = c.p;
    const size_t sbytes = c.used * sizeof(StatAcc);
    zero.push_back(OpRecord{"stats.zero", "memset", 0, (double)sbytes,
                            [=](cudaStream_t s) { CUDA_CHECK(cudaMemsetAsync(sb, 0, sbytes, s)); }});
  }
  ops_.insert(ops_.begin(), zero.begin(), zero.end());
  CUDA_CHECK(cudaDeviceSynchronize());
  finalized_ = true;
}

void UNetEngine::run_ops(cudaStream_t s, size_t n) {
  for (size_t i = 0; i < n && i < ops_.size(); ++i) ops_[i].run(s);
}

void UNetEngine::fill_t(float t, cudaStream_t stream) { fill(t_in_, B_, t, stream); }

void UNetEngine::set_labels(const int* labels_dev, cudaStream_t stream) {
  DDNM_CHECK(class_cond_, "set_labels on a network without a label embedding");
  DDNM_CHECK(labels_dev != nullptr, "null labels");
  if (labels_dev != labels_in_) CUDA_CHECK(cudaMemcpyAsync(labels_in_, labels_dev, (size_t)B_ * sizeof(int), cudaMemcpyDeviceToDevice, stream));
}

void UNetEngine::set_low_res(const float* low_res_dev, cudaStream_t stream) {
  DDNM_CHECK(lowres_ > 0, "set_low_res on a network without a low-resolution input");
  DDNM_CHECK(low_res_dev != nullptr, "null low_res");
  if (low_res_dev != lowres_in_)
    CUDA_CHECK(cudaMemcpyAsync(lowres_in_, low_res_dev, (size_t)B_ * in_ch_ * lowres_ * lowres_ * 4, cudaMemcpyDeviceToDevice, stream));
  lowres_set_ = true;
}

void UNetEngine::forward(const float* x, const float* t, float* out, cudaStream_t stream) {
  DDNM_CHECK(finalized_, "forward before finalize");
  DDNM_CHECK(lowres_ == 0 || lowres_set_, "super-resolution network: no low_res conditioning image was given");
  const size_t xin = (size_t)B_ * in_ch_ * R_ * R_ * 4;
  if (x != x_in_) CUDA_CHECK(cudaMemcpyAsync(x_in_, x, xin, cudaMemcpyDeviceToDevice, stream));
  if (t != t_in_) CUDA_CHECK(cudaMemcpyAsync(t_in_, t, (size_t)B_ * 4, cudaMemcpyDeviceToDevice, stream));
  replay(stream, ops_.size() - n_tail_ops_, graph_, graph_exec_);
  if (out != out_) CUDA_CHECK(cudaMemcpyAsync(out, out_, out_elems() * 4, cudaMemcpyDeviceToDevice, stream));
}

void UNetEngine::replay(cudaStream_t stream, size_t n, cudaGraph_t& g, cudaGraphExec_t& exec) {
  if (!use_graph_) {
    run_ops(stream, n);
    return;
  }
  if (!exec) {
    cudaStream_t cs = nullptr;
    CUDA_CHECK(cudaStreamCreateWithFlags(&cs, cudaStreamNonBlocking));
    CUDA_CHECK(cudaStreamSynchronize(stream));
    run_ops(cs, n);
    CUDA_CHECK(cudaStreamSynchronize(cs));
    CUDA_CHECK(cudaStreamBeginCapture(cs, cudaStreamCaptureModeThreadLocal));
    try {
      run_ops(cs, n);
    } catch (...) {
      cudaGraph_t gg = nullptr;
      cudaStreamEndCapture(cs, &gg);
      if (gg) cudaGraphDestroy(gg);
      cudaStreamDestroy(cs);
      throw;
    }
    CUDA_CHECK(cudaStreamEndCapture(cs, &g));
    CUDA_CHECK(cudaGraphInstantiate(&exec, g, 0));
    CUDA_CHECK(cudaStreamDestroy(cs));
  }
  CUDA_CHECK(cudaGraphLaunch(exec, stream));
}

bool UNetEngine::read_tap(const std::string& name, float* dst, long long capacity, cudaStream_t stream) {
  auto it = taps_.find(name);
  if (it == taps_.end()) return false;
  const View& v = it->second;
  DDNM_CHECK(capacity >= v.pixels() * v.C, "tap buffer too small");
  nhwc_to_nchw(v, dst, stream);
  return true;
}

double UNetEngine::flops_per_forward() const {
  double f = 0;
  for (auto& op : ops_) f += op.flops;
  return f;
}

std::string UNetEngine::profile(const float* x, const float* t, float* out, cudaStream_t stream) {
  const bool g = use_graph_;
  use_graph_ = false;
  forward(x, t, out, stream);
  CUDA_CHECK(cudaStreamSynchronize(stream));
  std::vector<cudaEvent_t> ev(ops_.size() + 1);
  for (auto& e : ev) CUDA_CHECK(cudaEventCreate(&e));
  CUDA_CHECK(cudaEventRecord(ev[0], stream));
  for (size_t i = 0; i < ops_.size(); ++i) {
    ops_[i].run(stream);
    CUDA_CHECK(cudaEventRecord(ev[i + 1], stream));
  }
  CUDA_CHECK(cudaStreamSynchronize(stream));
  std::ostringstream js;
  js << "[";
  for (size_t i = 0; i < ops_.size(); ++i) {
    float ms = 0;
    CUDA_CHECK(cudaEventElapsedTime(&ms, ev[i], ev[i + 1]));
    if (i) js << ",";
    js << "{\"name\":\"" << ops_[i].name << "\",\"kind\":\"" << ops_[i].kind << "\",\"ms\":" << ms << ",\"flops\":" << ops_[i].flops
       << ",\"bytes\":" << ops_[i].bytes << "}";
  }
  js << "]";
  for (auto& e : ev) cudaEventDestroy(e);
  use_graph_ = g;
  return js.str();
}

}
```

ddnm_b200/csrc/engine.cuh:

```cuda
#pragma once
#include <functional>
#include <map>
#include <memory>
#include <string>
#include <vector>

#include "common.cuh"
#include "tc_gemm.cuh"

namespace ddnm {

struct SimpleCfg {
  int ch = 128, out_ch = 3, n_levels = 6;
  int ch_mult[8] = {1, 1, 2, 2, 4, 4, 0, 0};
  int num_res_blocks = 2;
  int n_attn_res = 1;
  int attn_res[4] = {16, 0, 0, 0};
  int in_channels = 3, resolution = 256, groups = 32;
  float eps = 1e-6f;
};

class Arena {
 public:
  ~Arena();
  void* alloc(size_t bytes);
  size_t used() const { return total_; }

 private:
  std::vector<void*> blocks_;
  size_t total_ = 0;
};

struct OpRecord {
  std::string name;
  std::string kind;
  double flops = 0;
  double bytes = 0;
  std::function<void(cudaStream_t)> run;
};

struct OpenAICfg {
  int image_size = 256, model_channels = 256, num_res_blocks = 2, n_levels = 6;
  int channel_mult[8] = {1, 1, 2, 2, 4, 4, 0, 0};
  int n_attn_ds = 3;
  int attn_ds[4] = {8, 16, 32, 0};
  int num_head_channels = 64;
  int out_channels = 6, in_channels = 3, groups = 32;
  float eps = 1e-5f;
  int num_classes = 0;
  int low_res = 0;
  int num_heads = 1, num_heads_upsample = -1;
  int new_attention_order = 0;
};

void engine_debug_sm_count(int n);
int engine_sm_count(const cudaDeviceProp& prop);

class UNetEngine {
 public:
  UNetEngine(int batch, int in_channels, int out_ch, int resolution, int groups, float eps);
  virtual ~UNetEngine();
  void set_param(const std::string& name, const float* data, long long numel);
  void finalize();
  void forward(const float* x, const float* t, float* out, cudaStream_t stream);
  bool read_tap(const std::string& name, float* dst_nchw, long long capacity, cudaStream_t stream);
  std::string profile(const float* x, const float* t, float* out, cudaStream_t stream);
  int batch() const { return B_; }
  int out_ch() const { return out_ch_; }
  int in_channels() const { return in_ch_; }
  int resolution() const { return R_; }
  float* x_in() const { return x_in_; }
  float* t_in() const { return t_in_; }
  void fill_t(float t, cudaStream_t stream);
  int* labels_in() const { return labels_in_; }
  bool class_conditional() const { return class_cond_; }
  void set_labels(const int* labels_dev, cudaStream_t stream);
  int low_res_size() const { return lowres_; }
  void set_low_res(const float* low_res_dev, cudaStream_t stream);
  float* out_buf() const { return out_; }
  void set_use_graph(bool on) { use_graph_ = on; }
  void set_terms(int t);
  void set_batch_invariant(bool on);
  size_t workspace_bytes() const { return arena_.used(); }
  int num_launches() const { return (int)ops_.size(); }
  double flops_per_forward() const;

 protected:
  struct Param { float* p; long long n; };
  const float* P(const std::string& name, long long expect = -1) const;
  View new_view(int H, int W, int C);
  View view_of(float* p, int H, int W, int C) const;
  StatAcc* new_stats(int C);
  struct TcWeights { __half *hi, *lo; int ktot; };
  TcWeights prep_weights(const std::string& main, int Cout, int Cin, int taps, const std::string& side, int CinSide);
  const float* bias_sum(const std::string& a, const std::string& b, int C);
  float* dev_copy(const std::vector<float>& v);
  bool has_param(const std::string& name) const { return params_.count(name) != 0; }

  void add_op(const std::string& name, const std::string& kind, double flops, double bytes, std::function<void(cudaStream_t)> f);
  void emit_gn_split(const std::string& name, const View& x, const std::string& norm, bool silu, int mode, SplitView& dst,
                     const float* ss = nullptr, int ss_ld = 0, SplitView* raw = nullptr);
  void emit_tc(const std::string& name, const SplitView& a, int mode, const SplitView* side, const TcWeights& w, int Cout,
               const View& out, const float* chanadd, int ca_ld, const float* residual, int ldr, int res_mode = 0);
  void emit_attention_core(const std::string& name, float* qkv, int T, int heads, int ch, int qkv_ld, int head_stride, int q_off,
                           int k_off, int v_off, float alpha);
  void alloc_attention(size_t qkv_elems, size_t s_elems, size_t o_elems);
  void emit_up2_conv(const std::string& name, const SplitView& a, const std::string& wname, int Cout, const View& out,
                     const float* chanadd, int ca_ld);
  void emit_stem(const std::string& wname, const View& out);
  void emit_head(const std::string& norm, const std::string& conv, const View& h);

  struct EmbProj { std::string block, weight; const float* bias; int rows; };
  void emit_time_embed(const std::string& name, const std::string& layer0, const std::string& layer1, int ch, bool sin_first,
                       const float* label_emb, int num_classes, const std::vector<EmbProj>& projs);
  const float* emb_rows(const std::string& block) const { return emb_all_ + emb_off_.at(block); }

  enum LayerKind { LAYER_CONV, LAYER_RES, LAYER_RES_DOWN, LAYER_RES_UP, LAYER_ATTN };
  struct Block {
    struct Layer { int kind, cin, cout; };
    std::vector<Layer> layers;
    int res_in, res_out, cout;
  };
  struct Torso { std::vector<Block> input; Block middle; };
  static Torso plan_torso(int image_size, int in_channels, int model_channels, const int* channel_mult, int n_levels,
                          int num_res_blocks, const int* attn_ds, int n_attn_ds);
  void emit_res_block(const std::string& p, const View& x, const View& h, const View& out, int kind);
  void emit_attention_block(const std::string& p, const View& x, const View& out, int heads, bool new_order, float* qkv);

  void alloc_common(size_t split_elems, size_t hbuf_elems);
  virtual void build_program() = 0;
  virtual size_t out_elems() const { return (size_t)B_ * out_ch_ * R_ * R_; }
  void run_ops(cudaStream_t s, size_t n = (size_t)-1);
  void replay(cudaStream_t stream, size_t n, cudaGraph_t& g, cudaGraphExec_t& exec);

  int B_, in_ch_, out_ch_, R_, groups_;
  float eps_;
  int num_sms_ = 132;
  bool finalized_ = false, use_graph_ = true;
  int terms_ = 3;
  bool invariant_ = false;
  Arena arena_;
  std::map<std::string, Param> params_;
  std::vector<OpRecord> ops_;
  size_t n_tail_ops_ = 0;
  std::map<std::string, View> taps_;
  float *x_in_ = nullptr, *t_in_ = nullptr, *out_ = nullptr;
  int* labels_in_ = nullptr;
  bool class_cond_ = false;
  float* lowres_in_ = nullptr;
  int lowres_ = 0;
  bool lowres_set_ = false;
  __half *splitA_hi_ = nullptr, *splitA_lo_ = nullptr, *splitB_hi_ = nullptr, *splitB_lo_ = nullptr;
  size_t split_elems_ = 0;
  float* hbuf_ = nullptr;
  size_t hbuf_elems_ = 0;
  float *qkv_ = nullptr, *attS_ = nullptr, *attO_ = nullptr;
  __half *qkvh_ = nullptr, *qkvl_ = nullptr, *ph_ = nullptr, *pl_ = nullptr, *vth_ = nullptr, *vtl_ = nullptr;
  struct StatsChunk { StatAcc* p; size_t cap, used; };
  std::vector<StatsChunk> stats_chunks_;
  float* emb_all_ = nullptr;
  int emb_ld_ = 0;
  std::map<std::string, int> emb_off_;
  cudaGraph_t graph_ = nullptr;
  cudaGraphExec_t graph_exec_ = nullptr;
};

class UNetSimple : public UNetEngine {
 public:
  UNetSimple(const SimpleCfg& cfg, int batch);

 private:
  void build_program() override;
  void emit_resblock(const std::string& p, const View& x, const View& out);
  void emit_attn(const std::string& p, const View& x, const View& out);
  void emit_downsample(const std::string& p, const View& x, const View& out);
  void emit_upsample(const std::string& p, const View& x, const View& out);
  SimpleCfg cfg_;
};

class UNetOpenAI : public UNetEngine {
 public:
  UNetOpenAI(const OpenAICfg& cfg, int batch);

 private:
  void build_program() override;
  int attn_heads(int C, bool upsample) const;
  OpenAICfg cfg_;
};

struct EncoderCfg {
  int image_size = 256, model_channels = 128, num_res_blocks = 2, n_levels = 6;
  int channel_mult[8] = {1, 1, 2, 2, 4, 4, 0, 0};
  int n_attn_ds = 3;
  int attn_ds[4] = {8, 16, 32, 0};
  int num_head_channels = 64;
  int out_channels = 1000, in_channels = 3, groups = 32;
  float eps = 1e-5f;
  int pool = 1;
};

class UNetEncoder : public UNetEngine {
 public:
  UNetEncoder(const EncoderCfg& cfg, int batch);
  ~UNetEncoder() override;
  void grad(const float* x, const float* t, const int* labels, float scale, float* grad_out, float* logits, cudaStream_t stream,
            bool labels_checked = false);
  void check_labels(const int* labels, cudaStream_t stream) const;
  int num_classes() const { return cfg_.out_channels; }

 private:
  void build_program() override;
  size_t out_elems() const override { return (size_t)B_ * cfg_.out_channels; }
  struct Res { std::string p; View x, h, out; bool down, skip_conv; };
  struct Attn { std::string p; View x, out; float* qkv; };
  struct Layer { int kind; Res r; Attn a; };
  void emit_head(const View& h);
  void emit_backward(const View& stem_out, const std::vector<Layer>& layers, const View& top);
  void emit_gn_backward(const std::string& name, const float* g, const View& x, const std::string& norm, const float* ss, int ss_ld,
                        bool silu, bool pool, const float* add, bool add_pool, float* dx32, const SplitView& dst);
  TcWeights prep_weights_t(const std::string& w, int Cout, int Cin, int taps);
  EncoderCfg cfg_;
  int headT_ = 0;
  float *hf_ = nullptr, *tok_ = nullptr, *hqkv_ = nullptr, *hp_ = nullptr, *ha0_ = nullptr;
  float *scale_in_ = nullptr, *grad_ = nullptr, *gx_[2] = {nullptr, nullptr}, *g1_ = nullptr, *g2_ = nullptr, *gqkv_ = nullptr;
  float *sP_ = nullptr, *sdP_ = nullptr, *gnb_part_ = nullptr;
  size_t gnb_part_elems_ = 0;
  cudaGraph_t ggraph_ = nullptr;
  cudaGraphExec_t ggraph_exec_ = nullptr;
};

}
```

ddnm_b200/csrc/tc_gemm.cu:

```cuda
#include "tc_gemm.cuh"

#include <cstdlib>

#include "kernels.cuh"

namespace ddnm {

static constexpr int BM = 128;
static constexpr int kConsumerThreads = 256;
static constexpr int kTcThreads = kConsumerThreads + 32;
static constexpr int BK = 64;
static constexpr int A_PLANE_BYTES = BM * BK * 2;

static constexpr int HALO_PLANE_BYTES = 17 * 1024;
static constexpr int HALO_UNITS = 2;

template <int BN, bool DUAL, bool HALO = false>
struct TcCfg {
  static constexpr int B_PLANE_BYTES = BN * BK * 2;
  static constexpr int A_UNIT_BYTES = 2 * HALO_PLANE_BYTES;
  static constexpr int A_RING_BYTES = HALO ? HALO_UNITS * A_UNIT_BYTES : 0;
  static constexpr int STAGE_BYTES = (HALO ? 0 : 2 * A_PLANE_BYTES) + 2 * B_PLANE_BYTES;
  static constexpr int STAGES = (HALO || BN == 64) ? 4 : 3;
  static constexpr int RING_BYTES = A_RING_BYTES + STAGES * STAGE_BYTES;
  static constexpr int PART_BYTES = 8 * BN * 8;
  static constexpr int RUN_BYTES = 4 * 2 * BN * 8;
  static constexpr int SMEM_BYTES = RING_BYTES + 1024  + 256  + PART_BYTES + RUN_BYTES;
  static constexpr int ACC = DUAL ? BN : BN / 2;
  static_assert(SMEM_BYTES <= 227 * 1024, "shared memory capacity");
};

template <int N, int R>
__device__ __forceinline__ void wgmma_tile(float (&d)[R], uint64_t a, uint64_t b, uint32_t accumulate) {
  static_assert(N / 2 <= R, "accumulator too small");
  if constexpr (N == 64) wgmma_m64n64k16(*reinterpret_cast<float(*)[32]>(&d[0]), a, b, accumulate);
  else if constexpr (N == 128) wgmma_m64n128k16(*reinterpret_cast<float(*)[64]>(&d[0]), a, b, accumulate);
  else wgmma_m64n256k16(*reinterpret_cast<float(*)[128]>(&d[0]), a, b, accumulate);
}

__device__ __forceinline__ void tc_decode(const TcParams& p, int tile, int& n_idx, int& x0, int& y0, int& n0) {
  n_idx = tile % p.n_tiles;
  const int m = tile / p.n_tiles;
  const int tx = m % p.tiles_x;
  const int t2 = m / p.tiles_x;
  const int ty = t2 % p.tiles_y;
  const int tn = t2 / p.tiles_y;
  x0 = tx * p.bw;
  y0 = ty * p.bh;
  n0 = tn * p.bn;
}

template <int STAGES>
struct TcBars {
  uint32_t base;
  __device__ uint32_t full(int s) const { return base + 8u * s; }
  __device__ uint32_t empty(int s) const { return base + 8u * (STAGES + s); }
  __device__ uint32_t a_full(int u) const { return base + 8u * (2 * STAGES + u); }
  __device__ uint32_t a_empty(int u) const { return base + 8u * (2 * STAGES + HALO_UNITS + u); }
  __device__ uint32_t turn(int w) const { return base + 8u * (2 * STAGES + 2 * HALO_UNITS + w); }
};

struct TcRing {
  uint32_t stage = 0, phase = 0;
  uint32_t aunit = 0, aphase = 0;
};

template <class Cfg, bool PAIR, bool HALO>
__device__ __forceinline__ void tc_produce_tile(const CUtensorMap* tm_a0h, const CUtensorMap* tm_a0l, const CUtensorMap* tm_a1h,
                                                const CUtensorMap* tm_a1l, const CUtensorMap* tm_bh, const CUtensorMap* tm_bl,
                                                const TcParams& p, uint32_t smem_base, TcBars<Cfg::STAGES> bars, int tile, int kb_lo,
                                                int kb_hi, uint32_t rank, TcRing& r, bool load_a = true) {
  const int halo_r = p.mode0 == TAPS_UP2X2 ? 2 : 3;
  const int halo_w = p.bw + halo_r - 1;
  const bool lo = p.terms != 1;
  const uint32_t planes = lo ? 2u : 1u;
  const uint32_t stage_tx = (HALO || !load_a) ? planes * Cfg::B_PLANE_BYTES : (uint32_t)(lo ? Cfg::STAGE_BYTES : Cfg::STAGE_BYTES / 2);
  int n_idx, x0, y0, n0;
  tc_decode(p, tile, n_idx, x0, y0, n0);
  const int bz = p.b_batched == 1 ? n0 : 0;
  for (int kb = kb_lo; kb < kb_hi; ++kb) {
    int bkb = kb;
    if constexpr (HALO) {
      const int ua = kb / halo_r, dx = kb - ua * halo_r, dy = ua / p.cb0, cs = ua - dy * p.cb0;
      bkb = (dy * halo_r + dx) * p.cb0 + cs;
      if (dx == 0 && load_a) {
        mbar_wait(bars.a_empty(r.aunit), r.aphase ^ 1u);
        const uint32_t ua_s = smem_base + r.aunit * Cfg::A_UNIT_BYTES;
        const uint32_t fa = bars.a_full(r.aunit);
        const int cy = y0 + dy - 1 + p.up_py, cx = x0 - 1 + p.up_px;
        mbar_expect_tx(fa, planes * (uint32_t)(halo_w * p.bh * 128));
        tma_load_4d(ua_s, tm_a0h, fa, cs * BK, cx, cy, n0);
        if (lo) tma_load_4d(ua_s + HALO_PLANE_BYTES, tm_a0l, fa, cs * BK, cx, cy, n0);
      }
      if (dx == halo_r - 1) {
        if (++r.aunit == HALO_UNITS) {
          r.aunit = 0;
          r.aphase ^= 1u;
        }
      }
    }
    mbar_wait(bars.empty(r.stage), r.phase ^ 1u);
    const uint32_t sa = smem_base + Cfg::A_RING_BYTES + r.stage * Cfg::STAGE_BYTES;
    const uint32_t sb = HALO ? sa : sa + 2 * A_PLANE_BYTES;
    const uint32_t fb = bars.full(r.stage);
    mbar_expect_tx(fb, stage_tx);
    if (HALO || !load_a) {
    } else if (kb < p.kb0) {
      const int tap = kb / p.cb0;
      const int c = (kb - tap * p.cb0) * BK;
      int cx = x0, cy = y0, cn = n0;
      if (p.mode0 == TAPS_3X3) {
        cy += tap / 3 - 1;
        cx += tap % 3 - 1;
      } else if (p.mode0 == TAPS_UP2X2) {
        cy += tap / 2 + p.up_py - 1;
        cx += tap % 2 + p.up_px - 1;
      } else if (p.mode0 == TAPS_3X3_S2) {
        const int dy = tap / 3, dx = tap % 3;
        cy += dy >> 1;
        cx += dx >> 1;
        cn += ((dy & 1) * 2 + (dx & 1)) * p.phase_stride;
      }
      tma_load_4d(sa, tm_a0h, fb, c, cx, cy, cn);
      if (lo) tma_load_4d(sa + A_PLANE_BYTES, tm_a0l, fb, c, cx, cy, cn);
    } else {
      const int c = (kb - p.kb0) * BK;
      tma_load_4d(sa, tm_a1h, fb, c, x0, y0, n0);
      if (lo) tma_load_4d(sa + A_PLANE_BYTES, tm_a1l, fb, c, x0, y0, n0);
    }
    if (PAIR) {
      constexpr int BN = Cfg::B_PLANE_BYTES / (BK * 2);
      const uint32_t half = rank * (BN / 2) * 128u;
      const int brow = n_idx * BN + (int)rank * (BN / 2);
      tma_load_3d_multicast(sb + half, tm_bh, fb, bkb * BK, brow, 0, (uint16_t)3);
      if (lo) tma_load_3d_multicast(sb + Cfg::B_PLANE_BYTES + half, tm_bl, fb, bkb * BK, brow, 0, (uint16_t)3);
    } else if (p.b_batched == 2) {
      constexpr int BN = Cfg::B_PLANE_BYTES / (BK * 2);
      tma_load_4d(sb, tm_bh, fb, kb * BK, n_idx * BN, y0, n0);
      if (lo) tma_load_4d(sb + Cfg::B_PLANE_BYTES, tm_bl, fb, kb * BK, n_idx * BN, y0, n0);
    } else {
      constexpr int BN = Cfg::B_PLANE_BYTES / (BK * 2);
      tma_load_3d(sb, tm_bh, fb, bkb * BK, n_idx * BN, bz);
      if (lo) tma_load_3d(sb + Cfg::B_PLANE_BYTES, tm_bl, fb, bkb * BK, n_idx * BN, bz);
    }
    if (++r.stage == Cfg::STAGES) {
      r.stage = 0;
      r.phase ^= 1u;
    }
  }
}

template <int BN, bool DUAL, bool NTAIL, int R>
__device__ __forceinline__ void tc_epilogue_rows(const TcParams& p, float (&d)[R], bool dual, int r0, int cq, int n_idx, int x0,
                                                 int y0, int n0, int split_off) {
  const int ppi = p.bw * p.bh;
  float* orow[2];
  const float* rrow[2];
  const float* crow[2];
  bool valid[2];
#pragma unroll
  for (int h = 0; h < 2; ++h) {
    const int r = r0 + 8 * h;
    const int xi = r % p.bw, yi = (r / p.bw) % p.bh, ni = r / ppi;
    const int n = n0 + ni;
    valid[h] = n < p.N;
    orow[h] = p.out + (long long)n * p.out_sn + (long long)(y0 + yi) * p.out_sy + (long long)(x0 + xi) * p.out_sx + n_idx * BN +
              (long long)split_off * p.split_stride;
    rrow[h] = nullptr;
    if (p.residual) {
      long long rp;
      if (p.res_mode == 0) rp = ((long long)n * p.H + (y0 + yi)) * p.W + (x0 + xi);
      else if (p.res_mode == 1) rp = ((long long)n * (p.H >> 1) + ((y0 + yi) >> 1)) * (p.W >> 1) + ((x0 + xi) >> 1);
      else rp = ((long long)n * (2 * p.H) + 2 * (y0 + yi)) * (2 * p.W) + 2 * (x0 + xi);
      rrow[h] = p.residual + rp * p.ldr + n_idx * BN;
    }
    crow[h] = p.chanadd ? p.chanadd + (long long)n * p.ca_ld + n_idx * BN : nullptr;
  }
#pragma unroll
  for (int j = 0; j < BN / 8; ++j) {
    const int c = 8 * j + cq;
#pragma unroll
    for (int h = 0; h < 2; ++h) {
      float a0 = d[4 * j + 2 * h], a1 = d[4 * j + 2 * h + 1];
      if constexpr (DUAL) {
        if (dual) {
          a0 += d[4 * (j + BN / 8) + 2 * h];
          a1 += d[4 * (j + BN / 8) + 2 * h + 1];
        }
      }
      float v0 = p.alpha * a0, v1 = p.alpha * a1;
      if (crow[h] && valid[h]) {
        const float2 cv = __ldg(reinterpret_cast<const float2*>(crow[h] + c));
        v0 += cv.x;
        v1 += cv.y;
      }
      if (rrow[h] && valid[h]) {
        float2 rv = __ldg(reinterpret_cast<const float2*>(rrow[h] + c));
        if (p.res_mode == 2) {
          const long long r_dx = p.ldr, r_dy = (long long)2 * p.W * p.ldr;
          const float2 q1 = __ldg(reinterpret_cast<const float2*>(rrow[h] + r_dx + c));
          const float2 q2 = __ldg(reinterpret_cast<const float2*>(rrow[h] + r_dy + c));
          const float2 q3 = __ldg(reinterpret_cast<const float2*>(rrow[h] + r_dy + r_dx + c));
          rv.x = ((rv.x + q1.x) + (q2.x + q3.x)) * 0.25f;
          rv.y = ((rv.y + q1.y) + (q2.y + q3.y)) * 0.25f;
        }
        v0 += rv.x;
        v1 += rv.y;
      }
      if (!valid[h]) v0 = v1 = 0.f;
      d[4 * j + 2 * h] = v0;
      d[4 * j + 2 * h + 1] = v1;
      if (valid[h] && (!NTAIL || n_idx * BN + c < p.Cout)) *reinterpret_cast<float2*>(orow[h] + c) = make_float2(v0, v1);
    }
  }
}

template <int BN, int R>
__device__ __forceinline__ void tc_stats_rows(const float (&d)[R], float2* part, int lane, int cq) {
#pragma unroll
  for (int j = 0; j < BN / 8; ++j) {
#pragma unroll
    for (int e = 0; e < 2; ++e) {
      const float a = d[4 * j + e], b = d[4 * j + 2 + e];
      float s = a + b, q = a * a + b * b;
#pragma unroll
      for (int k = 4; k <= 16; k <<= 1) {
        s += __shfl_xor_sync(0xffffffffu, s, k);
        q += __shfl_xor_sync(0xffffffffu, q, k);
      }
      if (lane < 4) part[8 * j + cq + e] = make_float2(s, q);
    }
  }
}

template <int BN, bool DUAL, bool HALO, bool NTAIL>
__global__ void __launch_bounds__(kTcThreads, 1)
conv_tc_kernel(const __grid_constant__ CUtensorMap tm_a0h, const __grid_constant__ CUtensorMap tm_a0l,
               const __grid_constant__ CUtensorMap tm_a1h, const __grid_constant__ CUtensorMap tm_a1l,
               const __grid_constant__ CUtensorMap tm_bh, const __grid_constant__ CUtensorMap tm_bl, const TcParams p) {
  using Cfg = TcCfg<BN, DUAL, HALO>;
  constexpr int STAGES = Cfg::STAGES;
  extern __shared__ uint8_t smem_raw[];
  const uint32_t smem_base = (smem_u32(smem_raw) + 1023u) & ~1023u;
  const uint32_t bar_base = smem_base + Cfg::RING_BYTES;
  const TcBars<STAGES> bars{bar_base};
  auto full_bar = [&](int s) { return bars.full(s); };
  auto empty_bar = [&](int s) { return bars.empty(s); };
  auto a_full_bar = [&](int u) { return bars.a_full(u); };
  auto a_empty_bar = [&](int u) { return bars.a_empty(u); };
  const int halo_r = p.mode0 == TAPS_UP2X2 ? 2 : 3;
  const int halo_w = p.bw + halo_r - 1;
  uint8_t* stat_smem = smem_raw + (bar_base + 256u - smem_u32(smem_raw));
  float2* part = reinterpret_cast<float2*>(stat_smem);
  float2* run = reinterpret_cast<float2*>(stat_smem + Cfg::PART_BYTES);

  pdl_prologue();
  const int warp = threadIdx.x >> 5;
  const int lane = threadIdx.x & 31;
  const int KB = p.kb0 + p.kb1;
  const int m_tiles = p.tiles_x * p.tiles_y * p.tiles_n;
  const int total_tiles = m_tiles * p.n_tiles;
  const int n_units = total_tiles * p.split_k;
  const int n_workers = (int)gridDim.x;
  const int worker = (int)blockIdx.x;
  const int unit_begin = p.deal ? (int)((long long)worker * n_units / n_workers) : worker;
  const int unit_end = p.deal ? (int)((long long)(worker + 1) * n_units / n_workers) : n_units;
  const int unit_step = p.deal ? 1 : n_workers;
  auto k_lo = [&](int u) { return (int)((long long)(u % p.split_k) * KB / p.split_k); };
  auto k_hi = [&](int u) { return (int)((long long)(u % p.split_k + 1) * KB / p.split_k); };

  if (warp == 8 && lane == 0) {
    tma_prefetch_desc(&tm_a0h);
    tma_prefetch_desc(&tm_a0l);
    tma_prefetch_desc(&tm_bh);
    tma_prefetch_desc(&tm_bl);
    if (p.kb1) {
      tma_prefetch_desc(&tm_a1h);
      tma_prefetch_desc(&tm_a1l);
    }
    for (int s = 0; s < STAGES; ++s) {
      mbar_init(full_bar(s), 1);
      mbar_init(empty_bar(s), 8);
    }
    if (HALO) {
      for (int u = 0; u < HALO_UNITS; ++u) {
        mbar_init(a_full_bar(u), 1);
        mbar_init(a_empty_bar(u), 8);
      }
    }
    mbar_fence_init();
  }
  __syncthreads();

  auto decode = [&](int tile, int& n_idx, int& x0, int& y0, int& n0) { tc_decode(p, tile, n_idx, x0, y0, n0); };

  if (warp == 8) {
    if (lane == 0) {
      TcRing ring;
      for (int u = unit_begin; u < unit_end; u += unit_step)
        tc_produce_tile<Cfg, false, HALO>(&tm_a0h, &tm_a0l, &tm_a1h, &tm_a1l, &tm_bh, &tm_bl, p, smem_base, bars, u / p.split_k, k_lo(u),
                                          k_hi(u), 0u, ring);
    }
  } else {
  const int wg = warp >> 2;
  const uint32_t a_row_off = (uint32_t)wg * 64u * 128u;
  const uint32_t halo_row_off = (uint32_t)(((wg * 64) / p.bw) * halo_w + (wg * 64) % p.bw) * 128u;
  const int r0 = warp * 16 + (lane >> 2);
  const int cq = (lane & 3) * 2;
  const int tid = threadIdx.x;
  const int ppi = p.bw * p.bh;
  const int wpi = ppi >= 128 ? 8 : ppi / 16;
  uint32_t stage = 0, phase = 0;
  uint32_t a_done = 0;
  if (p.stats) {
    for (int i = tid; i < 4 * 2 * BN; i += kConsumerThreads) run[i] = make_float2(0.f, 0.f);
  }
  float d[Cfg::ACC];
  const bool dual = DUAL && p.terms != 1;
  auto release = [&](int s) {
    if (lane == 0) mbar_arrive(empty_bar(s));
  };
  auto release_a = [&](int a) {
    if (lane == 0) mbar_arrive(a_empty_bar(a));
  };
  for (int u = unit_begin; u < unit_end; u += unit_step) {
    const int kb_lo = k_lo(u), kb_hi = k_hi(u);
    int prev = -1;
    for (int kb = kb_lo; kb < kb_hi; ++kb) {
      uint32_t a_base = smem_base + stage * Cfg::STAGE_BYTES + a_row_off;
      uint32_t a_plane = A_PLANE_BYTES;
      uint32_t a_unit = 0;
      bool a_first = false;
      if constexpr (HALO) {
        int ua = 0, dx = 0;
        if (kb < p.kb0) {
          ua = halo_r == 3 ? (int)(__umulhi((uint32_t)kb, 0xAAAAAAABu) >> 1) : kb >> 1;
          dx = kb - ua * halo_r;
        }
        a_unit = a_done + (uint32_t)ua;
        a_first = dx == 0;
        if (a_first) mbar_wait(a_full_bar(a_unit % HALO_UNITS), (a_unit / HALO_UNITS) & 1u);
        a_base = smem_base + (a_unit % HALO_UNITS) * Cfg::A_UNIT_BYTES + (kb < p.kb0 ? halo_row_off + 128u * dx : a_row_off);
        a_plane = HALO_PLANE_BYTES;
      }
      mbar_wait(full_bar(stage), phase);
      const uint32_t sa = smem_base + Cfg::A_RING_BYTES + stage * Cfg::STAGE_BYTES;
      const uint32_t sb = HALO ? sa : sa + 2 * A_PLANE_BYTES;
      const uint64_t ah = wgmma_desc_sw128(a_base);
      const uint64_t al = wgmma_desc_sw128(a_base + a_plane);
      const uint64_t bh = wgmma_desc_sw128(sb);
      const uint64_t bl = wgmma_desc_sw128(sb + Cfg::B_PLANE_BYTES);
      wgmma_fence();
#pragma unroll
      for (int k = 0; k < BK / 16; ++k) {
        const uint64_t adv = 2u * k;
        const uint32_t acc = (uint32_t)(kb != kb_lo || k != 0);
        if (dual) {
          wgmma_tile<DUAL ? 2 * BN : BN>(d, ah + adv, bh + adv, acc);
          wgmma_tile<BN>(d, al + adv, bh + adv, 1u);
        } else {
          wgmma_tile<BN>(d, ah + adv, bh + adv, acc);
          if (p.terms != 1) {
            wgmma_tile<BN>(d, ah + adv, bl + adv, 1u);
            wgmma_tile<BN>(d, al + adv, bh + adv, 1u);
          }
        }
      }
      wgmma_commit();
      wgmma_wait<1>();
      if (prev >= 0) release(prev);
      prev = (int)stage;
      if (++stage == STAGES) {
        stage = 0;
        phase ^= 1u;
      }
      if (HALO && a_first && kb != kb_lo) release_a((a_unit - 1) % HALO_UNITS);
    }
    wgmma_wait<0>();
    if (prev >= 0) release(prev);
    if constexpr (HALO) {
      a_done += p.cb0 * halo_r;
      release_a((a_done - 1) % HALO_UNITS);
    }

    int n_idx, x0, y0, n0;
    decode(u / p.split_k, n_idx, x0, y0, n0);
    tc_epilogue_rows<BN, DUAL, NTAIL>(p, d, dual, r0, cq, n_idx, x0, y0, n0, u % p.split_k);
    if (p.stats) {
      tc_stats_rows<BN>(d, part + warp * BN, lane, cq);
      named_bar_sync(1, kConsumerThreads);
      const int nslots = 8 / wpi;
      bool flush = true;
      if (u + unit_step < unit_end) {
        int nn_idx, nx0, ny0, nn0;
        decode((u + unit_step) / p.split_k, nn_idx, nx0, ny0, nn0);
        flush = p.stat_per_tile || nslots > 1 || nn0 != n0 || nn_idx != n_idx;
      }
      for (int i = tid; i < 2 * BN; i += kConsumerThreads) {
        const int which = i / BN, col = i - which * BN;
        for (int g = 0; g < nslots; ++g) {
          float2& acc = run[(g * 2 + which) * BN + col];
          for (int w = g * wpi; w < (g + 1) * wpi; ++w) {
            const float2 pv = part[w * BN + col];
            two_sum_acc(acc.x, acc.y, which ? pv.y : pv.x);
          }
          if (flush) {
            const int n = n0 + g;
            if (n < p.N) {
              StatAcc* dst = p.stats + ((size_t)n * p.st_ld + n_idx * BN + col) * 2 + which;
              stat_add(dst, acc.x);
              stat_add(dst, acc.y);
            }
            acc = make_float2(0.f, 0.f);
          }
        }
      }
      named_bar_sync(1, kConsumerThreads);
    }
  }
  }
}

static constexpr int kPpThreads = 384;

__device__ __forceinline__ int pp_worker(int cta, int T) {
  const int k = cta >> 1;
  return (k / T) * 2 * T + k % T + (cta & 1) * T;
}

template <int BN, bool HALO>
struct PpCfg {
  using Ring = TcCfg<BN, false, HALO>;
  static constexpr int PART_BYTES = 8 * BN * 8;
  static constexpr int RUN_BYTES = 2 * BN * 8;
  static constexpr int STAT_BYTES = PART_BYTES + RUN_BYTES;
  static constexpr int SMEM_BYTES = Ring::RING_BYTES + 1024  + 256  + 2 * STAT_BYTES;
  static_assert(SMEM_BYTES <= 227 * 1024, "shared memory capacity");
};

template <int BN, int TERMS, bool HALO, bool NTAIL, bool PAIR>
__global__ void __launch_bounds__(kPpThreads, 1)
conv_tc_pingpong_kernel(const __grid_constant__ CUtensorMap tm_a0h, const __grid_constant__ CUtensorMap tm_a0l,
                        const __grid_constant__ CUtensorMap tm_a1h, const __grid_constant__ CUtensorMap tm_a1l,
                        const __grid_constant__ CUtensorMap tm_bh, const __grid_constant__ CUtensorMap tm_bl, const TcParams p) {
  static_assert(TERMS == 1 || TERMS == 3, "1 or 3 fp16 products per MAC");
  static_assert(!PAIR || !NTAIL, "CTA pairs share one weight matrix (no batched GEMMs)");
  using Cfg = PpCfg<BN, HALO>;
  using Ring = typename Cfg::Ring;
  constexpr int STAGES = Ring::STAGES;
  extern __shared__ uint8_t smem_raw[];
  const uint32_t smem_base = (smem_u32(smem_raw) + 1023u) & ~1023u;
  const TcBars<STAGES> bars{smem_base + Ring::RING_BYTES};

  pdl_prologue();
  const int warp = threadIdx.x >> 5;
  const int lane = threadIdx.x & 31;
  const int KB = p.kb0 + p.kb1;
  const int n_units = p.tiles_x * p.tiles_y * p.tiles_n * p.n_tiles * p.split_k;
  const int n_workers = (int)gridDim.x, worker = PAIR ? pp_worker((int)blockIdx.x, p.n_tiles) : (int)blockIdx.x;
  const int unit_begin = p.deal ? (int)((long long)worker * n_units / n_workers) : worker;
  const int unit_end = p.deal ? (int)((long long)(worker + 1) * n_units / n_workers) : n_units;
  const int unit_step = p.deal ? 1 : n_workers;
  auto k_lo = [&](int u) { return (int)((long long)(u % p.split_k) * KB / p.split_k); };
  auto k_hi = [&](int u) { return (int)((long long)(u % p.split_k + 1) * KB / p.split_k); };
  auto units_of = [&](int w) {
    return p.deal ? (int)((long long)(w + 1) * n_units / n_workers) - (int)((long long)w * n_units / n_workers)
                  : (n_units - w + n_workers - 1) / n_workers;
  };
  const int peer = worker + ((blockIdx.x & 1) ? -p.n_tiles : p.n_tiles);

  if (threadIdx.x == 0) {
    tma_prefetch_desc(&tm_a0h);
    tma_prefetch_desc(&tm_a0l);
    tma_prefetch_desc(&tm_bh);
    tma_prefetch_desc(&tm_bl);
    if (p.kb1) {
      tma_prefetch_desc(&tm_a1h);
      tma_prefetch_desc(&tm_a1l);
    }
    for (int s = 0; s < STAGES; ++s) {
      mbar_init(bars.full(s), 1);
      mbar_init(bars.empty(s), PAIR ? 8 : 4);
    }
    if (HALO) {
      for (int u = 0; u < HALO_UNITS; ++u) {
        mbar_init(bars.a_full(u), 1);
        mbar_init(bars.a_empty(u), 4);
      }
    }
    mbar_init(bars.turn(0), 4);
    mbar_init(bars.turn(1), 4);
    mbar_fence_init();
  }
  if (PAIR) cluster_sync_all();
  else __syncthreads();

  if (warp < 4) {
    setmaxnreg_dec<40>();
    if (threadIdx.x == 0) {
      TcRing ring;
      for (int u = unit_begin; u < unit_end; u += unit_step)
        tc_produce_tile<Ring, PAIR, HALO>(&tm_a0h, &tm_a0l, &tm_a1h, &tm_a1l, &tm_bh, &tm_bl, p, smem_base, bars, u / p.split_k,
                                          k_lo(u), k_hi(u), PAIR ? cluster_ctarank() : 0u, ring);
      if constexpr (PAIR) {
        const int peer_begin = p.deal ? (int)((long long)peer * n_units / n_workers) : peer;
        const uint32_t g0 = (uint32_t)(units_of(worker) * KB);
        uint32_t q = g0;
        auto ghost_release = [&](uint32_t g) {
          mbar_wait(bars.full(g % STAGES), (g / STAGES) & 1u);
          for (int w = 0; w < 4; ++w) {
            mbar_arrive(bars.empty(g % STAGES));
            mbar_arrive_cluster(bars.empty(g % STAGES), cluster_ctarank() ^ 1u);
          }
        };
        for (int j = units_of(worker); j < units_of(peer); ++j) {
          for (int kb = 0; kb < KB; ++kb, ++q) {
            if (q >= g0 + STAGES) ghost_release(q - STAGES);
            tc_produce_tile<Ring, true, HALO>(&tm_a0h, &tm_a0l, &tm_a1h, &tm_a1l, &tm_bh, &tm_bl, p, smem_base, bars,
                                              peer_begin + j * unit_step, kb, kb + 1, cluster_ctarank(), ring, false);
          }
        }
        for (uint32_t g = q >= g0 + STAGES ? q - STAGES : g0; g < q; ++g) ghost_release(g);
        for (int s = 0; s < STAGES; ++s) {
          mbar_wait(bars.empty(ring.stage), ring.phase ^ 1u);
          if (++ring.stage == STAGES) {
            ring.stage = 0;
            ring.phase ^= 1u;
          }
        }
      }
    }
    return;
  }
  setmaxnreg_inc<232>();
  const int c = (warp >> 2) - 1;
  const int wq = warp & 3;
  const int tid = threadIdx.x - 128 * (c + 1);
  const int r0 = wq * 16 + (lane >> 2);
  const int cq = (lane & 3) * 2;
  const int halo_r = p.mode0 == TAPS_UP2X2 ? 2 : 3;
  const int halo_w = p.bw + halo_r - 1;
  const int units_per_tile = p.cb0 * halo_r;
  uint32_t halo_row_off[2];
#pragma unroll
  for (int f = 0; f < 2; ++f) halo_row_off[f] = (uint32_t)(((f * 64) / p.bw) * halo_w + (f * 64) % p.bw) * 128u;
  const int wpi = p.bw * p.bh >= 128 ? 8 : p.bw * p.bh / 16;
  uint8_t* stat_smem = smem_raw + (bars.base + 256u - smem_u32(smem_raw)) + c * Cfg::STAT_BYTES;
  float2* part = reinterpret_cast<float2*>(stat_smem);
  float2* run = reinterpret_cast<float2*>(stat_smem + Cfg::PART_BYTES);
  if (p.stats) {
    for (int i = tid; i < 2 * BN; i += 128) run[i] = make_float2(0.f, 0.f);
  }
  auto release = [&](int s) {
    if (lane == 0) {
      mbar_arrive(bars.empty(s));
      if (PAIR) mbar_arrive_cluster(bars.empty(s), cluster_ctarank() ^ 1u);
    }
  };
  auto release_a = [&](uint32_t a) {
    if (lane == 0) mbar_arrive(bars.a_empty(a % HALO_UNITS));
  };
  uint32_t kpos = c ? (uint32_t)(k_hi(unit_begin) - k_lo(unit_begin)) : 0u;
  float d[2][BN / 2];
  int turn = 0;
  for (int u = unit_begin + c * unit_step; u < unit_end; u += 2 * unit_step, ++turn) {
    const int kb_lo = k_lo(u), kb_hi = k_hi(u);
    if (c == 1 || turn > 0) mbar_wait(bars.turn(c), (uint32_t)(c ? turn : turn - 1) & 1u);
    uint32_t stage = kpos % STAGES, phase = (kpos / STAGES) & 1u;
    const uint32_t a_done = (uint32_t)((2 * turn + c) * units_per_tile);
    int prev = -1;
    for (int kb = kb_lo; kb < kb_hi; ++kb) {
      const uint32_t sb = smem_base + Ring::A_RING_BYTES + stage * Ring::STAGE_BYTES;
      uint32_t a_base = sb;
      uint32_t a_frag1 = 64u * 128u;
      uint32_t a_plane = A_PLANE_BYTES;
      uint32_t a_unit = 0;
      bool a_first = false;
      if constexpr (HALO) {
        const int ua = halo_r == 3 ? (int)(__umulhi((uint32_t)kb, 0xAAAAAAABu) >> 1) : kb >> 1;
        const int dx = kb - ua * halo_r;
        a_unit = a_done + (uint32_t)ua;
        a_first = dx == 0;
        if (a_first) mbar_wait(bars.a_full(a_unit % HALO_UNITS), (a_unit / HALO_UNITS) & 1u);
        a_base = smem_base + (a_unit % HALO_UNITS) * Ring::A_UNIT_BYTES + halo_row_off[0] + 128u * dx;
        a_frag1 = halo_row_off[1] - halo_row_off[0];
        a_plane = HALO_PLANE_BYTES;
      }
      mbar_wait(bars.full(stage), phase);
      const uint32_t sbb = HALO ? sb : sb + 2 * A_PLANE_BYTES;
      const uint64_t ah0 = wgmma_desc_sw128(a_base), ah1 = wgmma_desc_sw128(a_base + a_frag1);
      const uint64_t al0 = wgmma_desc_sw128(a_base + a_plane), al1 = wgmma_desc_sw128(a_base + a_frag1 + a_plane);
      const uint64_t bh = wgmma_desc_sw128(sbb);
      const uint64_t bl = wgmma_desc_sw128(sbb + Ring::B_PLANE_BYTES);
      wgmma_fence();
#pragma unroll
      for (int k = 0; k < BK / 16; ++k) {
        const uint64_t adv = 2u * k;
        const uint32_t acc = (uint32_t)(kb != kb_lo || k != 0);
        wgmma_tile<BN>(d[0], ah0 + adv, bh + adv, acc);
        wgmma_tile<BN>(d[1], ah1 + adv, bh + adv, acc);
        if constexpr (TERMS == 3) {
          wgmma_tile<BN>(d[0], ah0 + adv, bl + adv, 1u);
          wgmma_tile<BN>(d[1], ah1 + adv, bl + adv, 1u);
          wgmma_tile<BN>(d[0], al0 + adv, bh + adv, 1u);
          wgmma_tile<BN>(d[1], al1 + adv, bh + adv, 1u);
        }
      }
      wgmma_commit();
      wgmma_wait<1>();
      if (prev >= 0) release(prev);
      prev = (int)stage;
      if (++stage == STAGES) {
        stage = 0;
        phase ^= 1u;
      }
      if (HALO && a_first && kb != kb_lo) release_a(a_unit - 1);
    }
    __syncwarp();
    if (lane == 0) mbar_arrive(bars.turn(c ^ 1));
    wgmma_wait<0>();
    if (prev >= 0) release(prev);
    if (HALO) release_a(a_done + units_per_tile - 1);
    kpos += (uint32_t)(kb_hi - kb_lo) + (uint32_t)(k_hi(u + unit_step) - k_lo(u + unit_step));

    int n_idx, x0, y0, n0;
    tc_decode(p, u / p.split_k, n_idx, x0, y0, n0);
#pragma unroll
    for (int f = 0; f < 2; ++f) tc_epilogue_rows<BN, false, NTAIL>(p, d[f], false, 64 * f + r0, cq, n_idx, x0, y0, n0, u % p.split_k);
    if (p.stats) {
#pragma unroll
      for (int f = 0; f < 2; ++f) tc_stats_rows<BN>(d[f], part + (4 * f + wq) * BN, lane, cq);
      named_bar_sync(1 + c, 128);
      const int nslots = 8 / wpi;
      bool flush = true;
      const int un = u + 2 * unit_step;
      if (!p.stat_per_tile && un < unit_end) {
        int nn_idx, nx0, ny0, nn0;
        tc_decode(p, un / p.split_k, nn_idx, nx0, ny0, nn0);
        flush = nslots > 1 || nn0 != n0 || nn_idx != n_idx;
      }
      for (int i = tid; i < 2 * BN; i += 128) {
        const int which = i / BN, col = i - which * BN;
        for (int g = 0; g < nslots; ++g) {
          float2 acc = nslots == 1 ? run[i] : make_float2(0.f, 0.f);
          for (int w = g * wpi; w < (g + 1) * wpi; ++w) {
            const float2 pv = part[w * BN + col];
            two_sum_acc(acc.x, acc.y, which ? pv.y : pv.x);
          }
          if (flush) {
            const int n = n0 + g;
            if (n < p.N) {
              StatAcc* dst = p.stats + ((size_t)n * p.st_ld + n_idx * BN + col) * 2 + which;
              stat_add(dst, acc.x);
              stat_add(dst, acc.y);
            }
            acc = make_float2(0.f, 0.f);
          }
          if (nslots == 1) run[i] = acc;
        }
      }
      named_bar_sync(1 + c, 128);
    }
  }
}

typedef CUresult (*EncodeTiledFn)(CUtensorMap*, CUtensorMapDataType, cuuint32_t, void*, const cuuint64_t*, const cuuint64_t*,
                                  const cuuint32_t*, const cuuint32_t*, CUtensorMapInterleave, CUtensorMapSwizzle,
                                  CUtensorMapL2promotion, CUtensorMapFloatOOBfill);

static EncodeTiledFn encode_fn() {
  static EncodeTiledFn fn = nullptr;
  if (!fn) {
    void* f = nullptr;
    cudaDriverEntryPointQueryResult q;
    CUDA_CHECK(cudaGetDriverEntryPoint("cuTensorMapEncodeTiled", &f, cudaEnableDefault, &q));
    DDNM_CHECK(f != nullptr && q == cudaDriverEntryPointSuccess, "cuTensorMapEncodeTiled not available");
    fn = reinterpret_cast<EncodeTiledFn>(f);
  }
  return fn;
}

static CUtensorMap make_map_f16(const void* base, int rank, const uint64_t* dims, const uint32_t* box,
                                const uint64_t* strides_elems = nullptr) {
  CUtensorMap m;
  cuuint64_t gdim[5], gstr[4];
  cuuint32_t b[5], es[5];
  uint64_t stride = 2;
  for (int i = 0; i < rank; ++i) {
    gdim[i] = dims[i];
    b[i] = box[i];
    es[i] = 1;
    stride *= dims[i];
    if (i < rank - 1) gstr[i] = strides_elems ? strides_elems[i] * 2 : stride;
  }
  CUresult r = encode_fn()(&m, CU_TENSOR_MAP_DATA_TYPE_FLOAT16, rank, const_cast<void*>(base), gdim, gstr, b, es,
                           CU_TENSOR_MAP_INTERLEAVE_NONE, CU_TENSOR_MAP_SWIZZLE_128B, CU_TENSOR_MAP_L2_PROMOTION_L2_256B,
                           CU_TENSOR_MAP_FLOAT_OOB_FILL_NONE);
  DDNM_CHECK(r == CUDA_SUCCESS, "cuTensorMapEncodeTiled failed (" + std::to_string((int)r) + ")");
  return m;
}

static int g_terms = 3;
void tc_set_terms(int terms) {
  DDNM_CHECK(terms == 1 || terms == 3, "terms must be 1 or 3");
  g_terms = terms;
}
int tc_get_terms() { return g_terms; }
static int g_force_bn = 0;
void tc_debug_force_bn(int bn) {
  DDNM_CHECK(bn == 0 || bn == 64 || bn == 128, "BN must be 0 (heuristic), 64 or 128");
  g_force_bn = bn;
}
static int g_dual_mode = 1;
void tc_debug_dual_mode(int mode) { g_dual_mode = mode; }
static int g_halo_enable = [] { const char* v = std::getenv("DDNM_HALO"); return v && *v ? std::atoi(v) : 1; }();
void tc_debug_halo(int on) { g_halo_enable = on; }
static int g_pingpong_enable = [] { const char* v = std::getenv("DDNM_PINGPONG"); return v && *v ? std::atoi(v) : 1; }();
void tc_debug_pingpong(int on) { g_pingpong_enable = on; }
static int g_pp_pair_enable = [] { const char* v = std::getenv("DDNM_PP_PAIR"); return v && *v ? std::atoi(v) : 1; }();
void tc_debug_pp_pair(int on) { g_pp_pair_enable = on; }
static int g_deal = -1;
void tc_debug_deal(int mode) {
  DDNM_CHECK(mode >= -1 && mode <= 1, "deal mode must be -1 (default rule), 0 (round-robin) or 1 (contiguous ranges)");
  g_deal = mode;
}

TcLaunch tc_make_launch(const SplitView& src0, int mode0, const SplitView* src1, const __half* w_hi, const __half* w_lo,
                        int w_batches, int Cout, const View& out, const float* chanadd, int ca_ld, const float* residual,
                        int ldr, float alpha, int num_sms, int res_mode, bool invariant) {
  TcLaunch L;
  TcParams& p = L.p;
  const int taps = (mode0 == TAPS_1X1) ? 1 : (mode0 == TAPS_UP2X2 ? 4 : 9);
  DDNM_CHECK(src0.C % BK == 0, "tensor-core conv needs Cin % 64 == 0");
  DDNM_CHECK(Cout % 64 == 0, "tensor-core conv needs Cout % 64 == 0");
  p.H = out.H; p.W = out.W; p.N = out.N;
  p.bw = out.W >= 128 ? 128 : out.W;
  DDNM_CHECK(128 % p.bw == 0 && out.W % p.bw == 0, "unsupported width for the 128-pixel tile");
  p.bh = std::min(out.H, 128 / p.bw);
  DDNM_CHECK(out.H % p.bh == 0 && 128 % (p.bw * p.bh) == 0, "unsupported height for the 128-pixel tile");
  p.bn = 128 / (p.bw * p.bh);
  p.tiles_x = out.W / p.bw;
  p.tiles_y = out.H / p.bh;
  p.tiles_n = cdiv(out.N, p.bn);
  {
    const int m_tiles = p.tiles_x * p.tiles_y * p.tiles_n;
    L.BN = 64;
    if (Cout % 128 == 0 && (long long)m_tiles * (Cout / 128) >= num_sms / 2) L.BN = 128;
    if (g_force_bn && Cout % g_force_bn == 0) L.BN = g_force_bn;
  }
  p.n_tiles = Cout / L.BN;
  L.dual = !invariant && g_dual_mode != 0;
  L.pingpong = g_pingpong_enable != 0;
  p.mode0 = mode0;
  p.cb0 = src0.C / BK;
  p.kb0 = taps * p.cb0;
  p.kb1 = src1 ? src1->C / BK : 0;
  if (src1) DDNM_CHECK(src1->C % BK == 0 && src1->H == out.H && src1->W == out.W && src1->N == out.N, "bad 1x1 side input");
  p.phase_stride = 0;
  p.up_py = p.up_px = 0;
  p.b_batched = w_batches > 1 ? 1 : 0;
  if (p.b_batched) DDNM_CHECK(p.bn == 1 && w_batches == out.N, "batched B operand needs one image per tile");
  if (mode0 == TAPS_3X3_S2) {
    DDNM_CHECK(src0.H == out.H && src0.W == out.W && src0.N == 4 * out.N, "stride-2 source must be 4 parity phases");
    p.phase_stride = out.N;
  } else {
    DDNM_CHECK(src0.H == out.H && src0.W == out.W && src0.N == out.N, "source/output shape mismatch");
  }
  p.Cout = Cout; p.ldc = out.ld; p.out = out.p;
  p.out_sx = out.ld; p.out_sy = (long long)out.W * out.ld; p.out_sn = (long long)out.H * out.W * out.ld;
  DDNM_CHECK(out.C == Cout && out.ld % 2 == 0 && ((uintptr_t)out.p & 7) == 0, "output view misaligned (rows move as float2)");
  p.chanadd = chanadd; p.ca_ld = ca_ld; p.residual = residual; p.ldr = ldr; p.alpha = alpha; p.res_mode = res_mode;
  p.stats = out.st; p.st_ld = out.st_ld;
  p.terms = g_terms;
  p.stat_per_tile = invariant ? 1 : 0;
  if (out.st) DDNM_CHECK(p.bw * p.bh >= 32, "GroupNorm statistics need >= 32 pixels per image");
  if (residual) DDNM_CHECK(ldr % 2 == 0 && ((uintptr_t)residual & 7) == 0, "residual misaligned (rows move as float2)");
  if (chanadd) DDNM_CHECK(ca_ld % 2 == 0 && ((uintptr_t)chanadd & 7) == 0, "channel-add rows misaligned");

  const uint64_t ad[4] = {(uint64_t)src0.C, (uint64_t)src0.W, (uint64_t)src0.H, (uint64_t)src0.N};
  const uint32_t abox[4] = {(uint32_t)BK, (uint32_t)p.bw, (uint32_t)p.bh, (uint32_t)p.bn};
  L.a0h = make_map_f16(src0.hi, 4, ad, abox);
  L.a0l = make_map_f16(src0.lo, 4, ad, abox);
  L.halo = g_halo_enable != 0 && (mode0 == TAPS_3X3 || mode0 == TAPS_UP2X2) && p.bw % 64 == 0 && p.bn == 1 && !src1;
  if (L.halo) {
    const uint32_t hbox[4] = {(uint32_t)BK, (uint32_t)(p.bw + (mode0 == TAPS_UP2X2 ? 1 : 2)), (uint32_t)p.bh, 1u};
    L.hh = make_map_f16(src0.hi, 4, ad, hbox);
    L.hl = make_map_f16(src0.lo, 4, ad, hbox);
  }
  if (src1) {
    const uint64_t ad1[4] = {(uint64_t)src1->C, (uint64_t)src1->W, (uint64_t)src1->H, (uint64_t)src1->N};
    L.a1h = make_map_f16(src1->hi, 4, ad1, abox);
    L.a1l = make_map_f16(src1->lo, 4, ad1, abox);
  } else {
    L.a1h = L.a0h;
    L.a1l = L.a0l;
  }
  const int Ktot = (p.kb0 + p.kb1) * BK;
  const uint64_t bd[3] = {(uint64_t)Ktot, (uint64_t)Cout, (uint64_t)w_batches};
  const uint32_t bbox[3] = {(uint32_t)BK, (uint32_t)L.BN, 1u};
  L.bh = make_map_f16(w_hi, 3, bd, bbox);
  L.bl = make_map_f16(w_lo, 3, bd, bbox);
  L.pp_pair = g_pp_pair_enable != 0 && w_batches == 1 && mode0 != TAPS_UP2X2;
  if (L.pp_pair) {
    const uint32_t hbox[3] = {(uint32_t)BK, (uint32_t)(L.BN / 2), 1u};
    L.bh2 = make_map_f16(w_hi, 3, bd, hbox);
    L.bl2 = make_map_f16(w_lo, 3, bd, hbox);
  }
  const int total = p.tiles_x * p.tiles_y * p.tiles_n * p.n_tiles;
  L.grid = std::min(total, num_sms);
  p.deal = g_deal >= 0 ? g_deal : (out.st != nullptr && p.n_tiles == 1 && total >= 2 * L.grid ? 1 : 0);
  if (p.n_tiles != 1) p.deal = 0;
  L.flops = 2.0 * (double)out.pixels() * Cout * Ktot;
  return L;
}

TcLaunch tc_make_up2_launch(const SplitView& src, const __half* w_hi, const __half* w_lo, int Cout, const View& out, const float* chanadd,
                            int ca_ld, int py, int px, int num_sms, bool invariant) {
  DDNM_CHECK(out.H == 2 * src.H && out.W == 2 * src.W && out.N == src.N, "upsample phase: output must be twice the source size");
  View lr = out;
  lr.H = src.H;
  lr.W = src.W;
  TcLaunch L = tc_make_launch(src, TAPS_UP2X2, nullptr, w_hi, w_lo, 1, Cout, lr, chanadd, ca_ld, nullptr, 0, 1.0f, num_sms, 0, invariant);
  TcParams& p = L.p;
  p.up_py = py;
  p.up_px = px;
  p.out = out.p + ((size_t)py * out.W + px) * out.ld;
  p.out_sx = 2LL * out.ld;
  p.out_sy = 2LL * out.W * out.ld;
  p.out_sn = (long long)out.H * out.W * out.ld;
  return L;
}

TcConvPlan tc_plan_conv(const SplitView& src0, int mode0, const SplitView* src1, const __half* w_hi, const __half* w_lo, int Cout,
                        const View& out, const float* chanadd, int ca_ld, const float* residual, int ldr, int res_mode, int num_sms,
                        bool invariant, int split_k) {
  TcConvPlan P;
  P.out = out; P.chanadd = chanadd; P.ca_ld = ca_ld; P.residual = residual; P.ldr = ldr;
  P.L = tc_make_launch(src0, mode0, src1, w_hi, w_lo, 1, Cout, out, chanadd, ca_ld, residual, ldr, 1.0f, num_sms, res_mode, invariant);
  const TcParams& p = P.L.p;
  const int tiles = p.tiles_x * p.tiles_y * p.tiles_n * p.n_tiles, kblocks = p.kb0 + p.kb1;
  static const bool split_on = std::getenv("DDNM_SPLITK") == nullptr || std::atoi(std::getenv("DDNM_SPLITK")) != 0;
  int S = 1;
  if (split_k > 0) {
    DDNM_CHECK(split_k == 1 || split_k == 2 || split_k == 4, "split_k must be 1, 2 or 4");
    DDNM_CHECK(split_k == 1 || (res_mode == 0 && kblocks >= split_k), "split-K needs res_mode 0 and a k-block per split");
    S = split_k;
  } else if (split_on && res_mode == 0 && kblocks >= 32) {
    if (invariant) S = out.H * out.W <= 64 ? 2 : 1;
    else if (2 * tiles <= num_sms) S = 4 * tiles <= num_sms ? 4 : 2;
  }
  if (S == 1) return P;
  P.S = S;
  const long long stride = out.pixels() * Cout;
  P.part_elems = S * stride;
  View pv = out;
  pv.p = nullptr; pv.ld = Cout; pv.st = nullptr; pv.st_ld = 0;
  TcLaunch Ls = tc_make_launch(src0, mode0, src1, w_hi, w_lo, 1, Cout, pv, nullptr, 0, nullptr, 0, 1.0f, num_sms, 0, invariant);
  DDNM_CHECK(Ls.BN == P.L.BN, "split-K: tile shape changed");
  Ls.p.split_k = S;
  Ls.p.split_stride = stride;
  Ls.halo = false;
  Ls.grid = std::min(tiles * S, num_sms);
  P.L = Ls;
  return P;
}

void tc_set_partials(TcConvPlan& P, float* part) {
  DDNM_CHECK(P.S > 1 && part != nullptr, "partial buffer for an unsplit plan");
  P.part = part;
  P.L.p.out = part;
}

void tc_run_split_reduce(const TcConvPlan& P, cudaStream_t stream) {
  DDNM_CHECK(P.S > 1 && P.part != nullptr, "split-K reduce without partial buffers");
  splitk_reduce(P.part, P.S, P.part_elems / P.S, P.out, P.chanadd, P.ca_ld, P.residual, P.ldr, stream);
}

void tc_run_conv(const TcConvPlan& P, cudaStream_t stream) {
  tc_run(P.L, stream);
  if (P.S > 1) tc_run_split_reduce(P, stream);
}

TcLaunch tc_make_gemm_launch(const GemmOperand& A, const GemmOperand& B, int M, int N, int K, int heads, int images, float* out,
                             long long out_sn, long long out_sy, long long out_sx, float alpha, int num_sms, bool invariant) {
  TcLaunch L;
  TcParams& p = L.p;
  DDNM_CHECK(M % 128 == 0 && N % 8 == 0 && K % 8 == 0, "attention GEMM: M % 128, N % 8, K % 8");
  p.H = heads; p.W = M; p.N = images;
  p.bw = 128; p.bh = 1; p.bn = 1;
  p.tiles_x = M / 128; p.tiles_y = heads; p.tiles_n = images;
  const int m_tiles = p.tiles_x * p.tiles_y * p.tiles_n;
  L.BN = 64;
  if (N % 128 == 0 && (long long)m_tiles * (N / 128) >= num_sms / 2) L.BN = 128;
  if (g_force_bn && N % g_force_bn == 0) L.BN = g_force_bn;
  L.dual = !invariant && g_dual_mode != 0;
  L.pingpong = g_pingpong_enable != 0;
  p.n_tiles = cdiv(N, L.BN);
  L.ntail = N % L.BN != 0;
  p.mode0 = TAPS_1X1;
  p.cb0 = cdiv(K, BK); p.kb0 = p.cb0; p.kb1 = 0;
  p.phase_stride = 0;
  p.up_py = p.up_px = 0;
  p.b_batched = 2;
  p.Cout = N; p.ldc = (int)out_sx; p.out = out;
  p.out_sn = out_sn; p.out_sy = out_sy; p.out_sx = out_sx;
  DDNM_CHECK(out_sx % 2 == 0 && out_sy % 2 == 0 && out_sn % 2 == 0 && ((uintptr_t)out & 7) == 0, "attention GEMM output misaligned");
  p.chanadd = nullptr; p.ca_ld = 0; p.residual = nullptr; p.ldr = 0; p.res_mode = 0; p.alpha = alpha;
  p.stats = nullptr; p.st_ld = 0;
  p.terms = g_terms;
  const uint64_t ad[4] = {(uint64_t)K, (uint64_t)M, (uint64_t)heads, (uint64_t)images};
  const uint64_t as[3] = {(uint64_t)A.s_row, (uint64_t)A.s_head, (uint64_t)A.s_img};
  const uint32_t abox[4] = {(uint32_t)BK, 128u, 1u, 1u};
  L.a0h = make_map_f16(A.hi, 4, ad, abox, as);
  L.a0l = make_map_f16(A.lo, 4, ad, abox, as);
  L.a1h = L.a0h;
  L.a1l = L.a0l;
  const uint64_t bd[4] = {(uint64_t)K, (uint64_t)N, (uint64_t)heads, (uint64_t)images};
  const uint64_t bs[3] = {(uint64_t)B.s_row, (uint64_t)B.s_head, (uint64_t)B.s_img};
  const uint32_t bbox[4] = {(uint32_t)BK, (uint32_t)L.BN, 1u, 1u};
  L.bh = make_map_f16(B.hi, 4, bd, bbox, bs);
  L.bl = make_map_f16(B.lo, 4, bd, bbox, bs);
  L.grid = std::min(m_tiles * p.n_tiles, num_sms);
  L.flops = 2.0 * (double)images * heads * M * (double)N * K;
  return L;
}

template <int BN, bool DUAL, bool HALO = false, bool NTAIL = false>
static void launch_bn(const TcLaunch& L, cudaStream_t stream) {
  using Cfg = TcCfg<BN, DUAL, HALO>;
  static bool attr_set[64] = {};
  if (first_use_on_device(attr_set))
    CUDA_CHECK(cudaFuncSetAttribute(conv_tc_kernel<BN, DUAL, HALO, NTAIL>, cudaFuncAttributeMaxDynamicSharedMemorySize, Cfg::SMEM_BYTES));
  launch_pdl(conv_tc_kernel<BN, DUAL, HALO, NTAIL>, dim3(L.grid), dim3(kTcThreads), (size_t)Cfg::SMEM_BYTES, stream, 1,
             HALO ? L.hh : L.a0h, HALO ? L.hl : L.a0l, L.a1h, L.a1l, L.bh, L.bl, L.p);
  CUDA_CHECK(cudaGetLastError());
}

template <int BN>
static void launch_forms(const TcLaunch& L, cudaStream_t stream) {
  if (L.ntail) {
    if constexpr (BN == 64) {
      if (L.dual) launch_bn<BN, true, false, true>(L, stream);
      else launch_bn<BN, false, false, true>(L, stream);
      return;
    }
    throw Error("partial N tiles need BN = 64");
  }
  if (L.halo && L.dual) launch_bn<BN, true, true>(L, stream);
  else if (L.halo) launch_bn<BN, false, true>(L, stream);
  else if (L.dual) launch_bn<BN, true>(L, stream);
  else launch_bn<BN, false>(L, stream);
}

template <int BN, int TERMS, bool HALO, bool NTAIL = false, bool PAIR = false>
static void launch_pingpong(const TcLaunch& L, cudaStream_t stream) {
  using Cfg = PpCfg<BN, HALO>;
  const auto kernel = conv_tc_pingpong_kernel<BN, TERMS, HALO, NTAIL, PAIR>;
  static bool attr_set[64] = {};
  static int max_clusters[64] = {};
  if (first_use_on_device(attr_set)) {
    CUDA_CHECK(cudaFuncSetAttribute(kernel, cudaFuncAttributeMaxDynamicSharedMemorySize, Cfg::SMEM_BYTES));
    if (PAIR) {
      cudaLaunchConfig_t cfg = {};
      cudaLaunchAttribute at;
      at.id = cudaLaunchAttributeClusterDimension;
      at.val.clusterDim.x = 2;
      at.val.clusterDim.y = 1;
      at.val.clusterDim.z = 1;
      cfg.gridDim = dim3(2);
      cfg.blockDim = dim3(kPpThreads);
      cfg.dynamicSmemBytes = Cfg::SMEM_BYTES;
      cfg.attrs = &at;
      cfg.numAttrs = 1;
      int dev = 0;
      CUDA_CHECK(cudaGetDevice(&dev));
      CUDA_CHECK(cudaOccupancyMaxActiveClusters(&max_clusters[dev & 63], kernel, &cfg));
    }
  }
  if (PAIR) {
    int dev = 0;
    CUDA_CHECK(cudaGetDevice(&dev));
    if (L.grid / 2 > max_clusters[dev & 63]) {
      launch_pingpong<BN, TERMS, HALO, NTAIL, false>(L, stream);
      return;
    }
  }
  launch_pdl(kernel, dim3(L.grid), dim3(kPpThreads), (size_t)Cfg::SMEM_BYTES, stream, PAIR ? 2 : 1, HALO ? L.hh : L.a0h,
             HALO ? L.hl : L.a0l, L.a1h, L.a1l, PAIR ? L.bh2 : L.bh, PAIR ? L.bl2 : L.bl, L.p);
  CUDA_CHECK(cudaGetLastError());
}

template <int BN, bool PAIR>
static void launch_pingpong_terms(const TcLaunch& L, cudaStream_t stream) {
  if (L.p.terms == 1) {
    if (L.halo) launch_pingpong<BN, 1, true, false, PAIR>(L, stream);
    else launch_pingpong<BN, 1, false, false, PAIR>(L, stream);
  } else {
    if (L.halo) launch_pingpong<BN, 3, true, false, PAIR>(L, stream);
    else launch_pingpong<BN, 3, false, false, PAIR>(L, stream);
  }
}

template <int BN>
static void launch_pingpong_forms(const TcLaunch& L, cudaStream_t stream) {
  if (L.ntail) {
    if constexpr (BN == 64) {
      if (L.p.terms == 1) launch_pingpong<BN, 1, false, true>(L, stream);
      else launch_pingpong<BN, 3, false, true>(L, stream);
      return;
    }
    throw Error("partial N tiles need BN = 64");
  }
  if (L.pp_pair && L.p.split_k == 1 && L.grid % (2 * L.p.n_tiles) == 0 && (L.p.n_tiles == 1 || L.p.deal == 0))
    launch_pingpong_terms<BN, true>(L, stream);
  else launch_pingpong_terms<BN, false>(L, stream);
}

void tc_run(const TcLaunch& L, cudaStream_t stream) {
  DDNM_CHECK(!L.halo || (L.p.split_k == 1 && L.p.kb1 == 0), "the HALO form runs unsplit launches without a 1x1 side input");
  const int units = L.p.tiles_x * L.p.tiles_y * L.p.tiles_n * L.p.n_tiles * L.p.split_k;
  if (L.pingpong && units > L.grid) {
    switch (L.BN) {
      case 128: launch_pingpong_forms<128>(L, stream); return;
      case 64: launch_pingpong_forms<64>(L, stream); return;
      default: throw Error("bad BN");
    }
  }
  switch (L.BN) {
    case 128: launch_forms<128>(L, stream); break;
    case 64: launch_forms<64>(L, stream); break;
    default: throw Error("bad BN");
  }
}

}
```

ddnm_b200/csrc/tc_gemm.cuh:

```cuda
#pragma once
#include "common.cuh"

namespace ddnm {

enum TcTapMode : int {
  TAPS_3X3 = 0,
  TAPS_1X1 = 1,
  TAPS_3X3_S2 = 2,
  TAPS_UP2X2 = 3,
};

struct TcParams {
  int H, W, N;
  int bw, bh, bn;
  int tiles_x, tiles_y, tiles_n;
  int n_tiles;
  int mode0;
  int cb0, kb0;
  int kb1;
  int phase_stride;
  int up_py, up_px;
  int b_batched;
  long long out_sn, out_sy, out_sx;
  int Cout, ldc;
  float* out;
  const float* chanadd;
  int ca_ld;
  const float* residual;
  int ldr;
  int res_mode;
  float alpha;
  StatAcc* stats;
  int st_ld;
  int split_k = 1;
  long long split_stride = 0;
  int deal = 0;
  int terms;
  int stat_per_tile = 0;
};

struct TcLaunch {
  CUtensorMap a0h, a0l, a1h, a1l, bh, bl;
  CUtensorMap hh, hl;
  TcParams p;
  int BN = 128;
  bool dual = false;
  bool halo = false;
  bool pingpong = false;
  bool pp_pair = false;
  CUtensorMap bh2, bl2;
  bool ntail = false;
  int grid = 0;
  double flops = 0;
};

TcLaunch tc_make_launch(const SplitView& src0, int mode0, const SplitView* src1, const __half* w_hi, const __half* w_lo,
                        int w_batches, int Cout, const View& out, const float* chanadd, int ca_ld, const float* residual,
                        int ldr, float alpha, int num_sms, int res_mode = 0, bool invariant = false);
void tc_run(const TcLaunch& L, cudaStream_t stream);
TcLaunch tc_make_up2_launch(const SplitView& src, const __half* w_hi, const __half* w_lo, int Cout, const View& out, const float* chanadd,
                            int ca_ld, int py, int px, int num_sms, bool invariant = false);

struct TcConvPlan {
  TcLaunch L;
  int S = 1;
  long long part_elems = 0;
  float* part = nullptr;
  View out;
  const float* chanadd = nullptr;
  int ca_ld = 0;
  const float* residual = nullptr;
  int ldr = 0;
};
TcConvPlan tc_plan_conv(const SplitView& src0, int mode0, const SplitView* src1, const __half* w_hi, const __half* w_lo, int Cout,
                        const View& out, const float* chanadd, int ca_ld, const float* residual, int ldr, int res_mode, int num_sms,
                        bool invariant, int split_k = -1);
void tc_set_partials(TcConvPlan& plan, float* part);
void tc_run_split_reduce(const TcConvPlan& plan, cudaStream_t stream);
void tc_run_conv(const TcConvPlan& plan, cudaStream_t stream);

struct GemmOperand {
  const __half* hi;
  const __half* lo;
  long long s_row, s_head, s_img;
};
TcLaunch tc_make_gemm_launch(const GemmOperand& A, const GemmOperand& B, int M, int N, int K, int heads, int images, float* out,
                             long long out_sn, long long out_sy, long long out_sx, float alpha, int num_sms, bool invariant = false);

void tc_debug_force_bn(int bn);
void tc_debug_deal(int mode);
void tc_debug_dual_mode(int mode);
void tc_debug_halo(int on);
void tc_debug_pingpong(int on);
void tc_debug_pp_pair(int on);
void tc_set_terms(int terms);
int tc_get_terms();

}
```

ddnm_b200/csrc/unet_simple.cu:

```cuda
#include <algorithm>
#include <cmath>

#include "engine.cuh"
#include "kernels.cuh"

namespace ddnm {

UNetSimple::UNetSimple(const SimpleCfg& cfg, int batch)
    : UNetEngine(batch, cfg.in_channels, cfg.out_ch, cfg.resolution, cfg.groups, cfg.eps), cfg_(cfg) {}

void UNetSimple::emit_resblock(const std::string& p, const View& x, const View& out) {
  const int Cin = x.C, Cout = out.C;
  DDNM_CHECK((size_t)(x.pixels() * Cout) <= hbuf_elems_, "hbuf too small");
  SplitView A{splitA_hi_, splitA_lo_}, Bs{splitB_hi_, splitB_lo_};
  View h = view_of(hbuf_, x.H, x.W, Cout);
  h.st = new_stats(Cout); h.st_ld = Cout;
  emit_gn_split(p + ".norm1", x, p + ".norm1", true, SPLIT_SAME, A, nullptr, 0, Cin != Cout ? &Bs : nullptr);
  TcWeights w1 = prep_weights(p + ".conv1.weight", Cout, Cin, 9, "", 0);
  emit_tc(p + ".conv1", A, TAPS_3X3, nullptr, w1, Cout, h, emb_rows(p), emb_ld_, nullptr, 0);
  emit_gn_split(p + ".norm2", h, p + ".norm2", true, SPLIT_SAME, A);
  if (Cin != Cout) {
    TcWeights w2 = prep_weights(p + ".conv2.weight", Cout, Cout, 9, p + ".nin_shortcut.weight", Cin);
    emit_tc(p + ".conv2+nin", A, TAPS_3X3, &Bs, w2, Cout, out, bias_sum(p + ".conv2.bias", p + ".nin_shortcut.bias", Cout), 0,
            nullptr, 0);
  } else {
    TcWeights w2 = prep_weights(p + ".conv2.weight", Cout, Cout, 9, "", 0);
    emit_tc(p + ".conv2", A, TAPS_3X3, nullptr, w2, Cout, out, P(p + ".conv2.bias", Cout), 0, x.p, x.ld);
  }
}

void UNetSimple::emit_attn(const std::string& p, const View& x, const View& out) {
  const int C = x.C, T = x.H * x.W;
  SplitView A{splitA_hi_, splitA_lo_};
  emit_gn_split(p + ".norm", x, p + ".norm", false, SPLIT_SAME, A);
  TcWeights wqkv;
  wqkv.ktot = C;
  wqkv.hi = (__half*)arena_.alloc((size_t)3 * C * C * sizeof(__half));
  wqkv.lo = (__half*)arena_.alloc((size_t)3 * C * C * sizeof(__half));
  std::vector<float> hb(3 * C);
  const char* nm[3] = {".q", ".k", ".v"};
  for (int i = 0; i < 3; ++i) {
    split_conv_weight(P(p + nm[i] + ".weight", (long long)C * C), C, C, 1, wqkv.hi + (size_t)i * C * C, wqkv.lo + (size_t)i * C * C, C, 0, 0);
    CUDA_CHECK(cudaMemcpy(hb.data() + i * C, P(p + nm[i] + ".bias", C), C * sizeof(float), cudaMemcpyDeviceToHost));
  }
  float* bqkv = dev_copy(hb);
  emit_tc(p + ".qkv", A, TAPS_1X1, nullptr, wqkv, 3 * C, view_of(qkv_, x.H, x.W, 3 * C), bqkv, 0, nullptr, 0);
  emit_attention_core(p, qkv_, T, 1, C, 3 * C, 0, 0, C, 2 * C, 1.0f / sqrtf((float)C));
  emit_gn_split(p + ".proj_in", view_of(attO_, x.H, x.W, C), "", false, SPLIT_SAME, A);
  TcWeights wp = prep_weights(p + ".proj_out.weight", C, C, 1, "", 0);
  emit_tc(p + ".proj_out", A, TAPS_1X1, nullptr, wp, C, out, P(p + ".proj_out.bias", C), 0, x.p, x.ld);
}

void UNetSimple::emit_downsample(const std::string& p, const View& x, const View& out) {
  SplitView A{splitA_hi_, splitA_lo_};
  emit_gn_split(p + ".s2d", x, "", false, SPLIT_S2D, A);
  TcWeights w = prep_weights(p + ".conv.weight", x.C, x.C, 9, "", 0);
  emit_tc(p + ".conv", A, TAPS_3X3_S2, nullptr, w, x.C, out, P(p + ".conv.bias", x.C), 0, nullptr, 0);
}

void UNetSimple::emit_upsample(const std::string& p, const View& x, const View& out) {
  SplitView A{splitA_hi_, splitA_lo_};
  emit_gn_split(p + ".split", x, "", false, SPLIT_SAME, A);
  emit_up2_conv(p + ".conv", A, p + ".conv.weight", x.C, out, P(p + ".conv.bias", x.C), 0);
}

void UNetSimple::build_program() {
  const SimpleCfg& c = cfg_;
  const int L = c.n_levels, R = c.resolution, nrb = c.num_res_blocks;
  DDNM_CHECK(c.ch % 64 == 0, "base channel count must be a multiple of 64 (tensor-core K blocks)");
  auto has_attn = [&](int res) {
    for (int i = 0; i < c.n_attn_res; ++i)
      if (c.attn_res[i] == res) return true;
    return false;
  };
  auto mult = [&](int lv) { return c.ch * c.ch_mult[lv]; };
  auto in_mult = [&](int lv) { return lv == 0 ? c.ch : c.ch * c.ch_mult[lv - 1]; };

  struct HS { int res, C; };
  std::vector<HS> hs_shape;
  hs_shape.push_back({R, c.ch});
  {
    int res = R;
    for (int lv = 0; lv < L; ++lv) {
      for (int ib = 0; ib < nrb; ++ib) hs_shape.push_back({res, mult(lv)});
      if (lv != L - 1) {
        res /= 2;
        hs_shape.push_back({res, mult(lv)});
      }
    }
  }
  const int n_up = L * (nrb + 1);
  DDNM_CHECK((int)hs_shape.size() == n_up, "skip stack / up-block count mismatch");
  struct UpB { int lv, ib, res, Ch, Cs, Cout; };
  std::vector<UpB> upb;
  {
    int res = R >> (L - 1);
    int block_in = mult(L - 1);
    for (int lv = L - 1; lv >= 0; --lv) {
      for (int ib = 0; ib <= nrb; ++ib) {
        const int skip = (ib == nrb) ? in_mult(lv) : mult(lv);
        upb.push_back({lv, ib, res, block_in, skip, mult(lv)});
        block_in = mult(lv);
      }
      if (lv != 0) res *= 2;
    }
    for (int u = 0; u < n_up; ++u) {
      const HS& h = hs_shape[n_up - 1 - u];
      DDNM_CHECK(h.res == upb[u].res && h.C == upb[u].Cs, "skip shape does not match its up block");
    }
  }

  size_t split_max = 0, hbuf_max = 0, att_tok = 0, att_c = 0, att_T = 0;
  int n_gn = 0;
  std::vector<EmbProj> projs;
  auto plan_conv_in = [&](int res, int Cin, bool up2) {
    split_max = std::max(split_max, (size_t)B_ * res * res * Cin * (up2 ? 4 : 1));
  };
  auto plan_rb = [&](const std::string& p, int res, int Cin, int Cout) {
    plan_conv_in(res, Cin, false);
    plan_conv_in(res, Cout, false);
    hbuf_max = std::max(hbuf_max, (size_t)B_ * res * res * Cout);
    n_gn += 2;
    projs.push_back({p, p + ".temb_proj.weight", bias_sum(p + ".temb_proj.bias", p + ".conv1.bias", Cout), Cout});
  };
  auto plan_attn = [&](int res, int C) {
    plan_conv_in(res, C, false);
    att_tok = std::max(att_tok, (size_t)res * res);
    att_c = std::max(att_c, (size_t)C);
    att_T = std::max(att_T, (size_t)res * res);
    n_gn += 1;
  };
  {
    int res = R;
    for (int lv = 0; lv < L; ++lv) {
      int cin = in_mult(lv);
      for (int ib = 0; ib < nrb; ++ib) {
        plan_rb("down." + std::to_string(lv) + ".block." + std::to_string(ib), res, cin, mult(lv));
        cin = mult(lv);
        if (has_attn(res)) plan_attn(res, cin);
      }
      if (lv != L - 1) {
        plan_conv_in(res, cin, false);
        res /= 2;
      }
    }
    plan_rb("mid.block_1", res, mult(L - 1), mult(L - 1));
    plan_attn(res, mult(L - 1));
    plan_rb("mid.block_2", res, mult(L - 1), mult(L - 1));
    for (const UpB& u : upb) {
      plan_rb("up." + std::to_string(u.lv) + ".block." + std::to_string(u.ib), u.res, u.Ch + u.Cs, u.Cout);
      if (has_attn(u.res)) plan_attn(u.res, u.Cout);
      if (u.ib == nrb && u.lv != 0) plan_conv_in(u.res, u.Cout, true);
    }
    n_gn += 1;
  }
  alloc_common(split_max, hbuf_max);
  alloc_attention((size_t)B_ * att_tok * 3 * att_c, (size_t)B_ * att_T * att_T, (size_t)B_ * att_tok * att_c);

  emit_time_embed("temb", "temb.dense.0", "temb.dense.1", c.ch, true, nullptr, 0, projs);
  std::vector<View> cat(n_up);
  for (int u = 0; u < n_up; ++u) cat[u] = new_view(upb[u].res, upb[u].res, upb[u].Ch + upb[u].Cs);
  auto hs_slot = [&](int i) {
    const int u = n_up - 1 - i;
    return cat[u].slice(upb[u].Ch, upb[u].Cs);
  };
  std::vector<View> hs;
  {
    View v0 = hs_slot(0);
    emit_stem("conv_in", v0);
    hs.push_back(v0);
    taps_["conv_in"] = v0;
  }
  int res = R;
  for (int lv = 0; lv < L; ++lv) {
    for (int ib = 0; ib < nrb; ++ib) {
      const std::string p = "down." + std::to_string(lv) + ".block." + std::to_string(ib);
      View slot = hs_slot((int)hs.size());
      if (has_attn(res)) {
        View tmp = new_view(res, res, mult(lv));
        emit_resblock(p, hs.back(), tmp);
        emit_attn("down." + std::to_string(lv) + ".attn." + std::to_string(ib), tmp, slot);
      } else {
        emit_resblock(p, hs.back(), slot);
      }
      hs.push_back(slot);
      taps_["down." + std::to_string(lv) + "." + std::to_string(ib)] = slot;
    }
    if (lv != L - 1) {
      View slot = hs_slot((int)hs.size());
      emit_downsample("down." + std::to_string(lv) + ".downsample", hs.back(), slot);
      hs.push_back(slot);
      taps_["down." + std::to_string(lv) + ".ds"] = slot;
      res /= 2;
    }
  }
  {
    const int C = mult(L - 1);
    View m1 = new_view(res, res, C), m2 = new_view(res, res, C);
    emit_resblock("mid.block_1", hs.back(), m1);
    taps_["mid.block_1"] = m1;
    emit_attn("mid.attn_1", m1, m2);
    taps_["mid.attn_1"] = m2;
    View dst = cat[0].slice(0, upb[0].Ch);
    emit_resblock("mid.block_2", m2, dst);
    taps_["mid.block_2"] = dst;
  }
  View final_h;
  for (int u = 0; u < n_up; ++u) {
    const UpB& ub = upb[u];
    const std::string p = "up." + std::to_string(ub.lv) + ".block." + std::to_string(ub.ib);
    const bool attn = has_attn(ub.res);
    const bool last_in_level = ub.ib == nrb;
    const bool upsample_next = last_in_level && ub.lv != 0;
    View dest;
    if (u == n_up - 1) dest = new_view(ub.res, ub.res, ub.Cout);
    else if (upsample_next) dest = new_view(ub.res, ub.res, ub.Cout);
    else dest = cat[u + 1].slice(0, upb[u + 1].Ch);
    if (attn) {
      View tmp = new_view(ub.res, ub.res, ub.Cout);
      emit_resblock(p, cat[u], tmp);
      emit_attn("up." + std::to_string(ub.lv) + ".attn." + std::to_string(ub.ib), tmp, dest);
    } else {
      emit_resblock(p, cat[u], dest);
    }
    taps_["up." + std::to_string(ub.lv) + "." + std::to_string(ub.ib)] = dest;
    if (upsample_next) {
      View d2 = cat[u + 1].slice(0, upb[u + 1].Ch);
      emit_upsample("up." + std::to_string(ub.lv) + ".upsample", dest, d2);
      taps_["up." + std::to_string(ub.lv) + ".us"] = d2;
    }
    if (u == n_up - 1) final_h = dest;
  }
  emit_head("norm_out", "conv_out", final_h);
}

}
```

include/ddnm_b200.h:

```cpp
#ifndef DDNM_B200_H
#define DDNM_B200_H

#ifdef __cplusplus
extern "C" {
#endif

const char* ddnm_last_error(void);
int ddnm_version(void);

typedef struct {
  int ch, out_ch, n_levels;
  int ch_mult[8];
  int num_res_blocks;
  int n_attn_res;
  int attn_res[4];
  int in_channels, resolution, groups;
  float eps;
} ddnm_simple_cfg;

int ddnm_unet_simple_create(const ddnm_simple_cfg* cfg, int batch, void** handle);

typedef struct {
  int image_size, model_channels, num_res_blocks, n_levels;
  int channel_mult[8];
  int n_attn_ds;
  int attn_ds[4];
  int num_head_channels, out_channels, in_channels, groups;
  float eps;
  int num_classes;
  int low_res;
  int num_heads;
  int num_heads_upsample;
  int new_attention_order;
} ddnm_openai_cfg;
int ddnm_unet_openai_create(const ddnm_openai_cfg* cfg, int batch, void** handle);
int ddnm_unet_set_param(void* handle, const char* name, const float* data, long long numel);
int ddnm_unet_set_precision(void* handle, int fp16_terms);
int ddnm_unet_finalize(void* handle);
int ddnm_unet_forward(void* handle, const float* x, const float* t, float* out, void* stream);
int ddnm_unet_forward_cond(void* handle, const float* x, const float* t, const int* labels, float* out, void* stream);
int ddnm_unet_set_low_res(void* handle, const float* low_res, void* stream);
int ddnm_unet_set_graph(void* handle, int use_cuda_graph);
int ddnm_unet_read_tap(void* handle, const char* name, float* dst_nchw, long long capacity, void* stream);
int ddnm_unet_info(void* handle, long long* workspace_bytes, int* launches, double* flops_per_forward);
int ddnm_unet_profile(void* handle, const float* x, const float* t, float* out, void* stream, char* json, long long capacity);
int ddnm_unet_destroy(void* handle);

typedef struct {
  int kind, channels, img_dim, ratio;
  const float* v_small;
  const float* u_small;
  const float* singulars;
  const float* singulars_orig;
  const long long* perm;
  const long long* mask;
  const float* v_small2;
  const float* u_small2;
} ddnm_operator_desc;

int ddnm_operator_create(const ddnm_operator_desc* desc, void** handle);
long long ddnm_operator_y_dim(void* handle);
int ddnm_operator_A(void* handle, const float* x, int B, float* y, void* stream);
int ddnm_operator_A_pinv(void* handle, const float* y, int B, float* x, void* stream);
int ddnm_operator_project(void* handle, const float* x0, const float* y, int B, float* x0_hat, void* stream);
int ddnm_operator_lambda(void* handle, const float* v, int B, float a, float sigma_y, float sigma_t, float eta, float* out,
                         void* stream);
int ddnm_operator_lambda_noise(void* handle, const float* v, const float* eps, int B, float a, float sigma_y, float sigma_t,
                               float eta, float* out, void* stream);
int ddnm_operator_destroy(void* handle);

typedef struct {
  int n_pairs;
  const int* t_i;
  const int* t_j;
  const float* abar;
  int num_timesteps;
  float eta;
  float sigma_y;
  int plus;
} ddnm_schedule;

int ddnm_sample(void* unet, void* op, const ddnm_schedule* sched, const float* x_T, const float* y, const float* noise, int B,
                float* out_x0, float* out_x0_pred, void* stream);

typedef int (*ddnm_guidance_fn)(void* user, int pair_index, int t, void* stream);
int ddnm_sample_guided(void* unet, void* op, const ddnm_schedule* sched, const float* x_T, const float* y, const float* noise, int B,
                       const int* labels, const float* grad_buf, ddnm_guidance_fn fn, void* user, float* out_x0, float* out_x0_pred,
                       void* stream);

int ddnm_sample_range(void* unet, void* op, const ddnm_schedule* sched, int k_begin, int k_end, float* xt, float* x0_pred,
                      int* have_x0, const float* y, const float* noise, int B, const int* labels, const float* grad_buf,
                      ddnm_guidance_fn fn, void* user, void* stream);

typedef struct {
  unsigned long long seed;
  long long row_offset;
} ddnm_noise_seed;
int ddnm_noise_fill(const ddnm_noise_seed* seed, unsigned tag, unsigned draw, float* out, int B, long long per_image, void* stream);
int ddnm_sample_range_seeded(void* unet, void* op, const ddnm_schedule* sched, int k_begin, int k_end, float* xt, float* x0_pred,
                             int* have_x0, const float* y, const ddnm_noise_seed* seed, int B, const int* labels,
                             const float* grad_buf, ddnm_guidance_fn fn, void* user, void* stream);
int ddnm_sample_seeded(void* unet, void* op, const ddnm_schedule* sched, const float* x_T, const float* y, const ddnm_noise_seed* seed,
                       int B, float* out_x0, float* out_x0_pred, void* stream);

typedef struct {
  int image_size, model_channels, num_res_blocks, n_levels;
  int channel_mult[8];
  int n_attn_ds;
  int attn_ds[4];
  int num_head_channels, out_channels, in_channels, groups;
  float eps;
  int pool;
} ddnm_classifier_cfg;
int ddnm_classifier_create(const ddnm_classifier_cfg* cfg, int batch, void** handle);
int ddnm_classifier_forward(void* h, const float* x, const float* t, float* logits, void* stream);
int ddnm_classifier_grad(void* h, const float* x, const float* t, const int* labels, float scale, float* grad_out, float* logits_out,
                         void* stream);
typedef struct {
  void* classifier;
  const float* x;
  const int* labels;
  float scale;
  float* grad_buf;
  int batch;
  int labels_checked;
} ddnm_classifier_guidance;
int ddnm_classifier_guidance_fn(void* user, int pair_index, int t, void* stream);

typedef struct {
  int use_mask, use_gray, scale, img_dim, channels;
  const float* mask;
  const float* image_mask;
} ddnm_simple_deg;
int ddnm_simplified_A(const ddnm_simple_deg* deg, const float* x, int B, float* y, void* stream);
int ddnm_simplified_Ap(const ddnm_simple_deg* deg, const float* y, int B, float* x, void* stream);
int ddnm_sample_simplified(void* unet, const ddnm_simple_deg* deg, const ddnm_schedule* sched, const float* x_T, const float* y,
                           const float* noise, int B, float* out_x0, float* out_x0_pred, void* stream);

int ddnm_sample_simplified_range(void* unet, const ddnm_simple_deg* deg, const ddnm_schedule* sched, int k_begin, int k_end, float* xt,
                                 float* x0_pred, int* have_x0, const float* y, const float* noise, int B, void* stream);
int ddnm_sample_simplified_range_seeded(void* unet, const ddnm_simple_deg* deg, const ddnm_schedule* sched, int k_begin, int k_end,
                                        float* xt, float* x0_pred, int* have_x0, const float* y, const ddnm_noise_seed* seed, int B,
                                        void* stream);

typedef struct {
  float c_recip, c_recipm1;
  float coef1, coef2;
  float lambda_t, gamma_t;
  float nonzero;
  int clip;
} ddnm_hq_scalars;
int ddnm_hq_canvas(const float* gt, int B, int H, int W, int scale, int use_gray, float* apy_canvas, void* stream);
int ddnm_hq_step(const ddnm_simple_deg* deg, const float* x, const float* model_out, int out_ch, const float* apy, const float* canvas,
                 int canvas_h, int canvas_w, const int* rects, const float* grad, const float* noise, const ddnm_hq_scalars* sc, int B,
                 float* x0_hat, float* x_next, float* scratch, void* stream);
int ddnm_hq_undo(float* x, const float* noise, float sqrt_one_minus_beta, float sqrt_beta, long long n, void* stream);
int ddnm_hq_step_seeded(const ddnm_simple_deg* deg, const float* x, const float* model_out, int out_ch, const float* apy,
                        const float* canvas, int canvas_h, int canvas_w, const int* rects, const float* grad,
                        const ddnm_noise_seed* seed, unsigned draw, const ddnm_hq_scalars* sc, int B, float* x0_hat, float* x_next,
                        float* scratch, void* stream);
int ddnm_hq_undo_seeded(float* x, const ddnm_noise_seed* seed, unsigned draw, float sqrt_one_minus_beta, float sqrt_beta, int B,
                        long long per_image, void* stream);
int ddnm_hq_canvas_masked(const ddnm_simple_deg* deg, const float* gt, int B, float* apy, float* scratch, void* stream);

int ddnm_data_transform(const float* x, long long n, const float* uniform_noise, const float* gauss_noise, int rescaled, int logit,
                        float* out, void* stream);
int ddnm_inverse_data_transform(const float* x, long long n, int rescaled, int logit, float* out, void* stream);
int ddnm_finish_images(const float* x, const float* orig, int B, int C, int H, int W, int rescaled, int logit, float* out01,
                       unsigned char* out_u8_hwc, float* psnr, void* stream);

int ddnm_conv_tc(const float* x, int N, int H, int W, int Cin, const float* w, const float* bias, int Cout, int mode, int up2,
                 const float* side_x, int CinSide, const float* side_w, const float* residual, float* out, void* stream);
int ddnm_conv_tc_ex(const float* x, int N, int H, int W, int Cin, const float* w, const float* chanadd, int ca_ld, int Cout, int mode,
                    int up2, const float* side_x, int CinSide, const float* side_w, const float* residual, int res_mode, float* out,
                    int out_ld, int split_k, int invariant, int terms, double* stats_out, int* split_used, void* stream);
int ddnm_gemm_tc(const float* a, long long a_numel, long long a_off, long long a_s_row, long long a_s_head, long long a_s_img,
                 const float* b, long long b_numel, long long b_off, long long b_s_row, long long b_s_head, long long b_s_img, int M,
                 int N, int K, int heads, int images, float alpha, float* out, long long out_sn, long long out_sy, long long out_sx,
                 int invariant, void* stream);
int ddnm_conv_direct(const float* x, int N, int H, int W, int Cin, const float* w, const float* bias, int Cout, int mode, int up2,
                     float* out, void* stream);
int ddnm_conv_stem_sr(const float* x, const float* low_res, int N, int C, int H, int W, int h, int w, const float* weight,
                      const float* bias, int Cout, float* out, int iters, float* ms_per_iter, void* stream);
int ddnm_conv_tc_bench(int N, int H, int W, int Cin, int Cout, int mode, int iters, float* ms_per_iter, double* flops);
int ddnm_gnconv_chunk_bench(int N, int chunk, int H, int W, int Cin, int Cout, int iters, float* ms_per_pass);
int ddnm_groupnorm(const float* x, int N, int H, int W, int C, int groups, const float* gamma, const float* beta, float eps,
                   int silu, float* out, void* stream);
int ddnm_tc_debug_force_bn(int bn);
int ddnm_tc_debug_deal(int mode);
int ddnm_tc_debug_dual_mode(int mode);
int ddnm_tc_debug_halo(int on);
int ddnm_tc_debug_pingpong(int on);
int ddnm_tc_debug_pp_pair(int on);
int ddnm_unet_set_batch_invariant(void* handle, int on);
int ddnm_tc_debug_sm_count(int n);

#ifdef __cplusplus
}
#endif
#endif
```

Before: 3.185.

## Load fp32 activations via TMA and split to fp16 hi/lo inside ping-pong conv kernel

Adds an A32 variant of the ping-pong tensor-core conv kernel. It TMA-loads fp32 activations directly, and idle producer warps split each k-block into fp16 hi/lo planes in shared memory before the consumer warps run wgmma. This removes the separate split passes for the stride-2 downsample input and the 1x1 shortcut side input, saving a global write and read of two half planes per conv. In exchange the kernel gains extra shared-memory traffic, a new barrier stage per ring slot and proxy fences, and the path is limited to unsplit, non-halo, 3-term persistent launches.

```diff
diff --git a/ddnm_b200/_lib.py b/ddnm_b200/_lib.py
--- a/ddnm_b200/_lib.py
+++ b/ddnm_b200/_lib.py
@@ -133,6 +133,8 @@
     "ddnm_tc_debug_halo": (C.c_int, [_I]),
     "ddnm_tc_debug_pingpong": (C.c_int, [_I]),
     "ddnm_tc_debug_pp_pair": (C.c_int, [_I]),
+    "ddnm_tc_debug_a32": (C.c_int, [_I]),
+    "ddnm_tc_a32_launches": (C.c_int, [C.POINTER(_LL)]),
     "ddnm_unet_set_batch_invariant": (C.c_int, [_P, _I]),
     "ddnm_tc_debug_sm_count": (C.c_int, [_I]),
 }
diff --git a/ddnm_b200/csrc/api.cu b/ddnm_b200/csrc/api.cu
--- a/ddnm_b200/csrc/api.cu
+++ b/ddnm_b200/csrc/api.cu
@@ -289,7 +289,7 @@
   SplitView A;
   A.hi = tmp.get<__half>(pe); A.lo = tmp.get<__half>(pe); A.C = Cin;
   if (smode == SPLIT_S2D) { A.N = 4 * N; A.H = oH; A.W = oW; } else { A.N = N; A.H = H; A.W = W; }
-  gn_apply_split(mkview(const_cast<float*>(x), N, H, W, Cin), 1, false, nullptr, nullptr, 0.f, false, smode, A.hi, A.lo, s);
+  auto split_x = [&] { gn_apply_split(mkview(const_cast<float*>(x), N, H, W, Cin), 1, false, nullptr, nullptr, 0.f, false, smode, A.hi, A.lo, s); };
   View ov = mkview(out, N, oH, oW, Cout);
   ov.ld = out_ld;
   if (stats_out) {
@@ -303,15 +303,18 @@
     __half* wh = tmp.get<__half>(4 * per_phase);
     __half* wl = tmp.get<__half>(4 * per_phase);
     presum_up2_weights(w, Cout, Cin, wh, wl, s);
+    split_x();
     for (int ph = 0; ph < 4; ++ph)
       tc_run(tc_make_up2_launch(A, wh + ph * per_phase, wl + ph * per_phase, Cout, ov, chanadd, ca_ld, ph >> 1, ph & 1, sms, invariant != 0), s);
   } else {
+    A.f32 = x;
+    A.ld = Cin;
     SplitView Sv;
     if (side_x) {
       const size_t se = (size_t)N * oH * oW * CinSide;
       Sv.hi = tmp.get<__half>(se); Sv.lo = tmp.get<__half>(se); Sv.N = N; Sv.H = oH; Sv.W = oW; Sv.C = CinSide;
-      gn_apply_split(mkview(const_cast<float*>(side_x), N, oH, oW, CinSide), 1, false, nullptr, nullptr, 0.f, false, SPLIT_SAME,
-                     Sv.hi, Sv.lo, s);
+      Sv.f32 = side_x;
+      Sv.ld = CinSide;
     }
     const int ktot = taps * Cin + (side_x ? CinSide : 0);
     __half* wh = tmp.get<__half>((size_t)Cout * ktot);
@@ -320,6 +323,10 @@
     if (side_x) split_conv_weight(side_w, Cout, CinSide, 1, wh, wl, ktot, taps * Cin, s);
     TcConvPlan P = tc_plan_conv(A, mode, side_x ? &Sv : nullptr, wh, wl, Cout, ov, chanadd, ca_ld, residual, Cout, res_mode, sms,
                                 invariant != 0, split_k);
+    if (!(P.L.p.a32 & 1)) split_x();
+    if (side_x && !(P.L.p.a32 & 2))
+      gn_apply_split(mkview(const_cast<float*>(side_x), N, oH, oW, CinSide), 1, false, nullptr, nullptr, 0.f, false, SPLIT_SAME,
+                     Sv.hi, Sv.lo, s);
     if (P.S > 1) tc_set_partials(P, tmp.get<float>((size_t)P.part_elems));
     tc_run_conv(P, s);
     S = P.S;
@@ -577,6 +584,17 @@
   tc_debug_pp_pair(on);
   DDNM_API_END
 }
+int ddnm_tc_debug_a32(int on) {
+  DDNM_API_BEGIN
+  tc_debug_a32(on);
+  DDNM_API_END
+}
+int ddnm_tc_a32_launches(long long* n) {
+  DDNM_API_BEGIN
+  DDNM_CHECK(n, "null argument");
+  *n = tc_a32_launches();
+  DDNM_API_END
+}
 int ddnm_tc_debug_force_bn(int bn) {
   DDNM_API_BEGIN
   tc_debug_force_bn(bn);
diff --git a/ddnm_b200/csrc/common.cuh b/ddnm_b200/csrc/common.cuh
--- a/ddnm_b200/csrc/common.cuh
+++ b/ddnm_b200/csrc/common.cuh
@@ -103,6 +103,8 @@
   __half* hi = nullptr;
   __half* lo = nullptr;
   int N = 0, H = 0, W = 0, C = 0;
+  const float* f32 = nullptr;
+  int ld = 0;
 };
 
 #ifdef __CUDACC__
@@ -220,6 +222,7 @@
       "l"(tmap), "r"(bar), "r"(c0), "r"(c1), "r"(c2), "h"(mask)
       : "memory");
 }
+__device__ __forceinline__ void fence_proxy_async_smem() { asm volatile("fence.proxy.async.shared::cta;" ::: "memory"); }
 __device__ __forceinline__ void named_bar_sync(int id, int threads) { asm volatile("bar.sync %0, %1;" ::"r"(id), "r"(threads) : "memory"); }
 template <int R>
 __device__ __forceinline__ void setmaxnreg_dec() { asm volatile("setmaxnreg.dec.sync.aligned.u32 %0;" ::"n"(R)); }
diff --git a/ddnm_b200/csrc/engine.cu b/ddnm_b200/csrc/engine.cu
--- a/ddnm_b200/csrc/engine.cu
+++ b/ddnm_b200/csrc/engine.cu
@@ -159,9 +159,29 @@
   }
 }
 
+SplitView UNetEngine::raw_operand(const SplitView& planes, const View& x, int mode) const {
+  SplitView s = planes;
+  s.C = x.C;
+  if (mode == TAPS_3X3_S2) { s.N = 4 * x.N; s.H = x.H / 2; s.W = x.W / 2; }
+  else { s.N = x.N; s.H = x.H; s.W = x.W; }
+  s.f32 = x.p;
+  s.ld = x.ld;
+  return s;
+}
+
 void UNetEngine::emit_tc(const std::string& name, const SplitView& a, int mode, const SplitView* side, const TcWeights& w,
                          int Cout, const View& out, const float* chanadd, int ca_ld, const float* residual, int ldr, int res_mode) {
   TcConvPlan P = tc_plan_conv(a, mode, side, w.hi, w.lo, Cout, out, chanadd, ca_ld, residual, ldr, res_mode, num_sms_, invariant_);
+  auto split_pass = [&](const SplitView& s, int smode, const std::string& what) {
+    View x;
+    x.p = const_cast<float*>(s.f32); x.C = s.C; x.ld = s.ld;
+    if (smode == SPLIT_S2D) { x.N = s.N / 4; x.H = 2 * s.H; x.W = 2 * s.W; }
+    else { x.N = s.N; x.H = s.H; x.W = s.W; }
+    SplitView planes = s;
+    emit_gn_split(name + what, x, "", false, smode, planes);
+  };
+  if (a.f32 && !(P.L.p.a32 & 1)) split_pass(a, mode == TAPS_3X3_S2 ? SPLIT_S2D : SPLIT_SAME, ".split");
+  if (side && side->f32 && !(P.L.p.a32 & 2)) split_pass(*side, SPLIT_SAME, ".side_split");
   const TcLaunch& L = P.L;
   const double bytes = (double)a.N * a.H * a.W * a.C * 4 + (side ? (double)side->N * side->H * side->W * side->C * 4 : 0) +
                        (double)Cout * w.ktot * 4 + (double)out.pixels() * Cout * 4 * (residual ? 2 : 1);
diff --git a/ddnm_b200/csrc/engine.cuh b/ddnm_b200/csrc/engine.cuh
--- a/ddnm_b200/csrc/engine.cuh
+++ b/ddnm_b200/csrc/engine.cuh
@@ -102,6 +102,7 @@
                      const float* ss = nullptr, int ss_ld = 0, SplitView* raw = nullptr);
   void emit_tc(const std::string& name, const SplitView& a, int mode, const SplitView* side, const TcWeights& w, int Cout,
                const View& out, const float* chanadd, int ca_ld, const float* residual, int ldr, int res_mode = 0);
+  SplitView raw_operand(const SplitView& planes, const View& x, int mode) const;
   void emit_attention_core(const std::string& name, float* qkv, int T, int heads, int ch, int qkv_ld, int head_stride, int q_off,
                            int k_off, int v_off, float alpha);
   void alloc_attention(size_t qkv_elems, size_t s_elems, size_t o_elems);
diff --git a/ddnm_b200/csrc/tc_gemm.cu b/ddnm_b200/csrc/tc_gemm.cu
--- a/ddnm_b200/csrc/tc_gemm.cu
+++ b/ddnm_b200/csrc/tc_gemm.cu
@@ -58,7 +58,9 @@
   __device__ uint32_t a_full(int u) const { return base + 8u * (2 * STAGES + u); }
   __device__ uint32_t a_empty(int u) const { return base + 8u * (2 * STAGES + HALO_UNITS + u); }
   __device__ uint32_t turn(int w) const { return base + 8u * (2 * STAGES + 2 * HALO_UNITS + w); }
+  __device__ uint32_t split(int s) const { return base + 8u * (2 * STAGES + 2 * HALO_UNITS + 2 + s); }
 };
+static_assert(8 * (3 * 4 + 2 * HALO_UNITS + 2) <= 256, "barrier block");
 
 struct TcRing {
   uint32_t stage = 0, phase = 0;
@@ -117,16 +119,23 @@
         cx += tap % 2 + p.up_px - 1;
       } else if (p.mode0 == TAPS_3X3_S2) {
         const int dy = tap / 3, dx = tap % 3;
-        cy += dy >> 1;
-        cx += dx >> 1;
-        cn += ((dy & 1) * 2 + (dx & 1)) * p.phase_stride;
+        if (p.a32 & 1) {
+          cy = 2 * cy + dy;
+          cx = 2 * cx + dx;
+        } else {
+          cy += dy >> 1;
+          cx += dx >> 1;
+          cn += ((dy & 1) * 2 + (dx & 1)) * p.phase_stride;
+        }
       }
       tma_load_4d(sa, tm_a0h, fb, c, cx, cy, cn);
-      if (lo) tma_load_4d(sa + A_PLANE_BYTES, tm_a0l, fb, c, cx, cy, cn);
+      if (p.a32 & 1) tma_load_4d(sa + A_PLANE_BYTES, tm_a0h, fb, c + 32, cx, cy, cn);
+      else if (lo) tma_load_4d(sa + A_PLANE_BYTES, tm_a0l, fb, c, cx, cy, cn);
     } else {
       const int c = (kb - p.kb0) * BK;
       tma_load_4d(sa, tm_a1h, fb, c, x0, y0, n0);
-      if (lo) tma_load_4d(sa + A_PLANE_BYTES, tm_a1l, fb, c, x0, y0, n0);
+      if (p.a32 & 2) tma_load_4d(sa + A_PLANE_BYTES, tm_a1h, fb, c + 32, x0, y0, n0);
+      else if (lo) tma_load_4d(sa + A_PLANE_BYTES, tm_a1l, fb, c, x0, y0, n0);
     }
     if (PAIR) {
       constexpr int BN = Cfg::B_PLANE_BYTES / (BK * 2);
@@ -423,6 +432,37 @@
 
 static constexpr int kPpThreads = 384;
 
+__device__ __forceinline__ void pp_split_kblock(uint32_t sa, int cw, int lane) {
+  const int s = lane & 15;
+  const int first = 2 * cw + (lane >> 4);
+  constexpr int kRows = 2;
+#pragma unroll 1
+  for (int q0 = 0; q0 < BM; q0 += 6 * kRows) {
+    float4 v[kRows];
+#pragma unroll
+    for (int i = 0; i < kRows; ++i) {
+      const int q = q0 + 6 * i + first;
+      if (q < BM) {
+        const uint32_t a = sa + (s >> 3) * A_PLANE_BYTES + q * 128 + (((s & 7) ^ (q & 7)) << 4);
+        asm volatile("ld.shared.v4.f32 {%0, %1, %2, %3}, [%4];" : "=f"(v[i].x), "=f"(v[i].y), "=f"(v[i].z), "=f"(v[i].w) : "r"(a) : "memory");
+      }
+    }
+    __syncwarp();
+#pragma unroll
+    for (int i = 0; i < kRows; ++i) {
+      const int q = q0 + 6 * i + first;
+      if (q < BM) {
+        uint32_t h0, h1, l0, l1;
+        split2_f16(v[i].x, v[i].y, h0, l0);
+        split2_f16(v[i].z, v[i].w, h1, l1);
+        const uint32_t a = sa + q * 128 + ((((s >> 1) ^ (q & 7)) << 4) | ((s & 1) << 3));
+        asm volatile("st.shared.v2.b32 [%0], {%1, %2};" ::"r"(a), "r"(h0), "r"(h1) : "memory");
+        asm volatile("st.shared.v2.b32 [%0], {%1, %2};" ::"r"(a + A_PLANE_BYTES), "r"(l0), "r"(l1) : "memory");
+      }
+    }
+  }
+}
+
 __device__ __forceinline__ int pp_worker(int cta, int T) {
   const int k = cta >> 1;
   return (k / T) * 2 * T + k % T + (cta & 1) * T;
@@ -438,13 +478,13 @@
   static_assert(SMEM_BYTES <= 227 * 1024, "shared memory capacity");
 };
 
-template <int BN, int TERMS, bool HALO, bool NTAIL, bool PAIR>
-__global__ void __launch_bounds__(kPpThreads, 1)
-conv_tc_pingpong_kernel(const __grid_constant__ CUtensorMap tm_a0h, const __grid_constant__ CUtensorMap tm_a0l,
-                        const __grid_constant__ CUtensorMap tm_a1h, const __grid_constant__ CUtensorMap tm_a1l,
-                        const __grid_constant__ CUtensorMap tm_bh, const __grid_constant__ CUtensorMap tm_bl, const TcParams p) {
+template <int BN, int TERMS, bool HALO, bool NTAIL, bool PAIR, bool A32>
+__device__ __forceinline__ void pp_kernel_body(const CUtensorMap& tm_a0h, const CUtensorMap& tm_a0l, const CUtensorMap& tm_a1h,
+                                               const CUtensorMap& tm_a1l, const CUtensorMap& tm_bh, const CUtensorMap& tm_bl,
+                                               const TcParams& p) {
   static_assert(TERMS == 1 || TERMS == 3, "1 or 3 fp16 products per MAC");
   static_assert(!PAIR || !NTAIL, "CTA pairs share one weight matrix (no batched GEMMs)");
+  static_assert(!A32 || (TERMS == 3 && !HALO && !NTAIL), "fp32 sources: per-tap fp32-grade convolutions");
   using Cfg = PpCfg<BN, HALO>;
   using Ring = typename Cfg::Ring;
   constexpr int STAGES = Ring::STAGES;
@@ -490,6 +530,9 @@
     }
     mbar_init(bars.turn(0), 4);
     mbar_init(bars.turn(1), 4);
+    if (A32) {
+      for (int s = 0; s < STAGES; ++s) mbar_init(bars.split(s), 3);
+    }
     mbar_fence_init();
   }
   if (PAIR) cluster_sync_all();
@@ -529,6 +572,23 @@
           }
         }
       }
+    } else if (A32 && warp > 0) {
+      uint32_t stage = 0, phase = 0;
+      for (int u = unit_begin; u < unit_end; u += unit_step) {
+        for (int kb = k_lo(u); kb < k_hi(u); ++kb) {
+          mbar_wait(bars.full(stage), phase);
+          if (p.a32 & (kb < p.kb0 ? 1 : 2)) {
+            pp_split_kblock(smem_base + stage * Ring::STAGE_BYTES, warp - 1, lane);
+            fence_proxy_async_smem();
+          }
+          __syncwarp();
+          if (lane == 0) mbar_arrive(bars.split(stage));
+          if (++stage == STAGES) {
+            stage = 0;
+            phase ^= 1u;
+          }
+        }
+      }
     }
     return;
   }
@@ -586,7 +646,7 @@
         a_frag1 = halo_row_off[1] - halo_row_off[0];
         a_plane = HALO_PLANE_BYTES;
       }
-      mbar_wait(bars.full(stage), phase);
+      mbar_wait(A32 ? bars.split(stage) : bars.full(stage), phase);
       const uint32_t sbb = HALO ? sb : sb + 2 * A_PLANE_BYTES;
       const uint64_t ah0 = wgmma_desc_sw128(a_base), ah1 = wgmma_desc_sw128(a_base + a_frag1);
       const uint64_t al0 = wgmma_desc_sw128(a_base + a_plane), al1 = wgmma_desc_sw128(a_base + a_frag1 + a_plane);
@@ -664,6 +724,22 @@
   }
 }
 
+template <int BN, int TERMS, bool HALO, bool NTAIL, bool PAIR>
+__global__ void __launch_bounds__(kPpThreads, 1)
+conv_tc_pingpong_kernel(const __grid_constant__ CUtensorMap tm_a0h, const __grid_constant__ CUtensorMap tm_a0l,
+                        const __grid_constant__ CUtensorMap tm_a1h, const __grid_constant__ CUtensorMap tm_a1l,
+                        const __grid_constant__ CUtensorMap tm_bh, const __grid_constant__ CUtensorMap tm_bl, const TcParams p) {
+  pp_kernel_body<BN, TERMS, HALO, NTAIL, PAIR, false>(tm_a0h, tm_a0l, tm_a1h, tm_a1l, tm_bh, tm_bl, p);
+}
+
+template <int BN, bool PAIR>
+__global__ void __launch_bounds__(kPpThreads, 1)
+conv_tc_pingpong_a32_kernel(const __grid_constant__ CUtensorMap tm_a0h, const __grid_constant__ CUtensorMap tm_a0l,
+                            const __grid_constant__ CUtensorMap tm_a1h, const __grid_constant__ CUtensorMap tm_a1l,
+                            const __grid_constant__ CUtensorMap tm_bh, const __grid_constant__ CUtensorMap tm_bl, const TcParams p) {
+  pp_kernel_body<BN, 3, false, false, PAIR, true>(tm_a0h, tm_a0l, tm_a1h, tm_a1l, tm_bh, tm_bl, p);
+}
+
 typedef CUresult (*EncodeTiledFn)(CUtensorMap*, CUtensorMapDataType, cuuint32_t, void*, const cuuint64_t*, const cuuint64_t*,
                                   const cuuint32_t*, const cuuint32_t*, CUtensorMapInterleave, CUtensorMapSwizzle,
                                   CUtensorMapL2promotion, CUtensorMapFloatOOBfill);
@@ -700,6 +776,19 @@
   return m;
 }
 
+static CUtensorMap make_map_f32(const float* base, int N, int H, int W, int C, int ld, const uint32_t* box, uint32_t es) {
+  CUtensorMap m;
+  const cuuint64_t gdim[4] = {(cuuint64_t)C, (cuuint64_t)W, (cuuint64_t)H, (cuuint64_t)N};
+  const cuuint64_t gstr[3] = {(cuuint64_t)ld * 4, (cuuint64_t)W * ld * 4, (cuuint64_t)H * W * ld * 4};
+  const cuuint32_t b[4] = {32u, box[1] * es, box[2] * es, box[3]};
+  const cuuint32_t e[4] = {1u, es, es, 1u};
+  CUresult r = encode_fn()(&m, CU_TENSOR_MAP_DATA_TYPE_FLOAT32, 4, const_cast<float*>(base), gdim, gstr, b, e,
+                           CU_TENSOR_MAP_INTERLEAVE_NONE, CU_TENSOR_MAP_SWIZZLE_128B, CU_TENSOR_MAP_L2_PROMOTION_L2_256B,
+                           CU_TENSOR_MAP_FLOAT_OOB_FILL_NONE);
+  DDNM_CHECK(r == CUDA_SUCCESS, "cuTensorMapEncodeTiled (fp32) failed (" + std::to_string((int)r) + ")");
+  return m;
+}
+
 static int g_terms = 3;
 void tc_set_terms(int terms) {
   DDNM_CHECK(terms == 1 || terms == 3, "terms must be 1 or 3");
@@ -719,6 +808,10 @@
 void tc_debug_pingpong(int on) { g_pingpong_enable = on; }
 static int g_pp_pair_enable = [] { const char* v = std::getenv("DDNM_PP_PAIR"); return v && *v ? std::atoi(v) : 1; }();
 void tc_debug_pp_pair(int on) { g_pp_pair_enable = on; }
+static int g_a32_enable = [] { const char* v = std::getenv("DDNM_A32"); return v && *v ? std::atoi(v) : 1; }();
+void tc_debug_a32(int on) { g_a32_enable = on; }
+static long long g_a32_launches = 0;
+long long tc_a32_launches() { return g_a32_launches; }
 static int g_deal = -1;
 void tc_debug_deal(int mode) {
   DDNM_CHECK(mode >= -1 && mode <= 1, "deal mode must be -1 (default rule), 0 (round-robin) or 1 (contiguous ranges)");
@@ -810,6 +903,20 @@
   L.grid = std::min(total, num_sms);
   p.deal = g_deal >= 0 ? g_deal : (out.st != nullptr && p.n_tiles == 1 && total >= 2 * L.grid ? 1 : 0);
   if (p.n_tiles != 1) p.deal = 0;
+  const bool a32_ok = g_a32_enable != 0 && L.pingpong && total > L.grid && p.terms == 3 && !L.halo && w_batches == 1 && p.n_tiles == 1;
+  auto tma_ok = [](const SplitView& s) { return s.f32 && s.ld % 4 == 0 && ((uintptr_t)s.f32 & 15) == 0; };
+  if (a32_ok && tma_ok(src0)) {
+    const bool s2 = mode0 == TAPS_3X3_S2;
+    L.a0h = make_map_f32(src0.f32, s2 ? src0.N / 4 : src0.N, s2 ? 2 * src0.H : src0.H, s2 ? 2 * src0.W : src0.W, src0.C, src0.ld, abox,
+                         s2 ? 2u : 1u);
+    L.a0l = L.a0h;
+    p.a32 |= 1;
+  }
+  if (a32_ok && src1 && tma_ok(*src1)) {
+    L.a1h = make_map_f32(src1->f32, src1->N, src1->H, src1->W, src1->C, src1->ld, abox, 1u);
+    L.a1l = L.a1h;
+    p.a32 |= 2;
+  }
   L.flops = 2.0 * (double)out.pixels() * Cout * Ktot;
   return L;
 }
@@ -952,10 +1059,10 @@
   else launch_bn<BN, false>(L, stream);
 }
 
-template <int BN, int TERMS, bool HALO, bool NTAIL = false, bool PAIR = false>
+template <int BN, int TERMS, bool HALO, bool NTAIL = false, bool PAIR = false, bool A32 = false>
 static void launch_pingpong(const TcLaunch& L, cudaStream_t stream) {
   using Cfg = PpCfg<BN, HALO>;
-  const auto kernel = conv_tc_pingpong_kernel<BN, TERMS, HALO, NTAIL, PAIR>;
+  const auto kernel = A32 ? conv_tc_pingpong_a32_kernel<BN, PAIR> : conv_tc_pingpong_kernel<BN, TERMS, HALO, NTAIL, PAIR>;
   static bool attr_set[64] = {};
   static int max_clusters[64] = {};
   if (first_use_on_device(attr_set)) {
@@ -981,10 +1088,11 @@
     int dev = 0;
     CUDA_CHECK(cudaGetDevice(&dev));
     if (L.grid / 2 > max_clusters[dev & 63]) {
-      launch_pingpong<BN, TERMS, HALO, NTAIL, false>(L, stream);
+      launch_pingpong<BN, TERMS, HALO, NTAIL, false, A32>(L, stream);
       return;
     }
   }
+  if (A32) ++g_a32_launches;
   launch_pdl(kernel, dim3(L.grid), dim3(kPpThreads), (size_t)Cfg::SMEM_BYTES, stream, PAIR ? 2 : 1, HALO ? L.hh : L.a0h,
              HALO ? L.hl : L.a0l, L.a1h, L.a1l, PAIR ? L.bh2 : L.bh, PAIR ? L.bl2 : L.bl, L.p);
   CUDA_CHECK(cudaGetLastError());
@@ -997,6 +1105,7 @@
     else launch_pingpong<BN, 1, false, false, PAIR>(L, stream);
   } else {
     if (L.halo) launch_pingpong<BN, 3, true, false, PAIR>(L, stream);
+    else if (L.p.a32) launch_pingpong<BN, 3, false, false, PAIR, true>(L, stream);
     else launch_pingpong<BN, 3, false, false, PAIR>(L, stream);
   }
 }
@@ -1019,6 +1128,8 @@
 void tc_run(const TcLaunch& L, cudaStream_t stream) {
   DDNM_CHECK(!L.halo || (L.p.split_k == 1 && L.p.kb1 == 0), "the HALO form runs unsplit launches without a 1x1 side input");
   const int units = L.p.tiles_x * L.p.tiles_y * L.p.tiles_n * L.p.n_tiles * L.p.split_k;
+  DDNM_CHECK(!L.p.a32 || (L.pingpong && units > L.grid && L.p.split_k == 1 && !L.halo && L.p.terms == 3),
+             "fp32 sources need an unsplit per-tap ping-pong launch");
   if (L.pingpong && units > L.grid) {
     switch (L.BN) {
       case 128: launch_pingpong_forms<128>(L, stream); return;
diff --git a/ddnm_b200/csrc/tc_gemm.cuh b/ddnm_b200/csrc/tc_gemm.cuh
--- a/ddnm_b200/csrc/tc_gemm.cuh
+++ b/ddnm_b200/csrc/tc_gemm.cuh
@@ -37,6 +37,7 @@
   int deal = 0;
   int terms;
   int stat_per_tile = 0;
+  int a32 = 0;
 };
 
 struct TcLaunch {
@@ -93,6 +94,8 @@
 void tc_debug_halo(int on);
 void tc_debug_pingpong(int on);
 void tc_debug_pp_pair(int on);
+void tc_debug_a32(int on);
+long long tc_a32_launches();
 void tc_set_terms(int terms);
 int tc_get_terms();
 
diff --git a/ddnm_b200/csrc/unet_simple.cu b/ddnm_b200/csrc/unet_simple.cu
--- a/ddnm_b200/csrc/unet_simple.cu
+++ b/ddnm_b200/csrc/unet_simple.cu
@@ -15,16 +15,25 @@
   SplitView A{splitA_hi_, splitA_lo_}, Bs{splitB_hi_, splitB_lo_};
   View h = view_of(hbuf_, x.H, x.W, Cout);
   h.st = new_stats(Cout); h.st_ld = Cout;
-  emit_gn_split(p + ".norm1", x, p + ".norm1", true, SPLIT_SAME, A, nullptr, 0, Cin != Cout ? &Bs : nullptr);
+  TcWeights w2{};
+  bool side32 = false;
+  if (Cin != Cout) {
+    w2 = prep_weights(p + ".conv2.weight", Cout, Cout, 9, p + ".nin_shortcut.weight", Cin);
+    SplitView a2 = A;
+    a2.N = x.N; a2.H = x.H; a2.W = x.W; a2.C = Cout;
+    const SplitView s32 = raw_operand(Bs, x, TAPS_1X1);
+    side32 = tc_plan_conv(a2, TAPS_3X3, &s32, w2.hi, w2.lo, Cout, out, nullptr, 0, nullptr, 0, 0, num_sms_, invariant_).L.p.a32 & 2;
+    if (side32) Bs = s32;
+  }
+  emit_gn_split(p + ".norm1", x, p + ".norm1", true, SPLIT_SAME, A, nullptr, 0, Cin != Cout && !side32 ? &Bs : nullptr);
   TcWeights w1 = prep_weights(p + ".conv1.weight", Cout, Cin, 9, "", 0);
   emit_tc(p + ".conv1", A, TAPS_3X3, nullptr, w1, Cout, h, emb_rows(p), emb_ld_, nullptr, 0);
   emit_gn_split(p + ".norm2", h, p + ".norm2", true, SPLIT_SAME, A);
   if (Cin != Cout) {
-    TcWeights w2 = prep_weights(p + ".conv2.weight", Cout, Cout, 9, p + ".nin_shortcut.weight", Cin);
     emit_tc(p + ".conv2+nin", A, TAPS_3X3, &Bs, w2, Cout, out, bias_sum(p + ".conv2.bias", p + ".nin_shortcut.bias", Cout), 0,
             nullptr, 0);
   } else {
-    TcWeights w2 = prep_weights(p + ".conv2.weight", Cout, Cout, 9, "", 0);
+    w2 = prep_weights(p + ".conv2.weight", Cout, Cout, 9, "", 0);
     emit_tc(p + ".conv2", A, TAPS_3X3, nullptr, w2, Cout, out, P(p + ".conv2.bias", Cout), 0, x.p, x.ld);
   }
 }
@@ -52,8 +61,7 @@
 }
 
 void UNetSimple::emit_downsample(const std::string& p, const View& x, const View& out) {
-  SplitView A{splitA_hi_, splitA_lo_};
-  emit_gn_split(p + ".s2d", x, "", false, SPLIT_S2D, A);
+  const SplitView A = raw_operand(SplitView{splitA_hi_, splitA_lo_}, x, TAPS_3X3_S2);
   TcWeights w = prep_weights(p + ".conv.weight", x.C, x.C, 9, "", 0);
   emit_tc(p + ".conv", A, TAPS_3X3_S2, nullptr, w, x.C, out, P(p + ".conv.bias", x.C), 0, nullptr, 0);
 }
diff --git a/include/ddnm_b200.h b/include/ddnm_b200.h
--- a/include/ddnm_b200.h
+++ b/include/ddnm_b200.h
@@ -192,6 +192,8 @@
 int ddnm_tc_debug_halo(int on);
 int ddnm_tc_debug_pingpong(int on);
 int ddnm_tc_debug_pp_pair(int on);
+int ddnm_tc_debug_a32(int on);
+int ddnm_tc_a32_launches(long long* n);
 int ddnm_unet_set_batch_invariant(void* handle, int on);
 int ddnm_tc_debug_sm_count(int n);
 
```

Measured after the change: 3.229 (median of 6 runs). +1.4%, better.
